# anthonyhu/tumblr-emotions

Hardware: AMD Instinct MI355X
Metric: training samples/sec (224x224 img + 32-tok text, batch 256) (higher is better)
Workload: dtype f32; 1 GPU; joint train step (fwd+bwd+all-reduce+Adam): Inception-v1 224x224x3 + 300-d embedding + LSTM-512, T=32, V=10000, 15 classes, batch 256 per GPU, reference freeze (<=Mixed_5b conv weights frozen, all BN betas trainable), dropout 0.8, BN train mode; global_batch=256, per_gpu_batch=256, parallelism=dp1, launch=eager

## Files before the change

include/ds_kernels.h:

```cpp
#ifndef DS_KERNELS_H
#define DS_KERNELS_H

#include <stddef.h>
#include <stdint.h>

#ifdef __cplusplus
extern "C" {
#endif

#define DS_OK 0
#define DS_ERR_ARG (-1)
#define DS_ERR_LAUNCH (-2)
#define DS_ERR_WORKSPACE (-3)

#define DS_DTYPE_F32 0
#define DS_DTYPE_BF16 1

#define DS_EPI_BIAS 1
#define DS_EPI_RELU 2
#define DS_EPI_ACCUM 4
#define DS_EPI_STATS 8
#define DS_EPI_MASK 16
#define DS_EPI_BNSUMS 32
#define DS_EPI_BN_RELU 64

int ds_version(void);
const char *ds_last_error(void);

typedef struct ds_conv_desc {
    int32_t N, H, W;
    int32_t Cin;
    int32_t ldx;
    int32_t KH, KW, stride;
    int32_t pad_t, pad_l;
    int32_t OH, OW;
    int32_t Cout;
    int32_t ldz;
    int64_t w_tap_stride;
    int32_t w_n_stride;
    int32_t w_k_stride;
    int32_t flip;
    int32_t fold_cin;
    int32_t flags;
    int32_t ldmask;
    int32_t splits;
    int64_t z_split_stride;
    int32_t tile_nt;
    int32_t grid_x;
    int32_t dtype;
    int32_t x_dtype;
    int32_t partials;
    const float *norm_rstd;
    const float *norm_shift;
    const float *mask_rstd;
    const float *mask_shift;
    const struct ds_bn_bwd_on_load *bnb;
    int32_t mask_dtype;
    int32_t z_dtype;
    uint8_t *pool_argmax;
    const struct ds_bn_finalize_in_launch *fin;
} ds_conv_desc;

typedef struct ds_bn_finalize_in_launch {
    const float *beta;
    float *mean, *rstd, *shift;
    float *moving_mean, *moving_var;
    uint32_t *ticket;
    int64_t count;
    float eps, decay;
} ds_bn_finalize_in_launch;

typedef struct ds_bn_bwd_on_load {
    const float *mean, *rstd, *shift;
    const float *coef;
    int32_t nseg;
    int32_t c_end[3];
    int32_t ld[3];
    const float *dy[3];
} ds_bn_bwd_on_load;

#ifdef DS_TUNING
int ds_debug_conv_set_tile(int mt, int nt);
int ds_debug_conv_set_path(int path);
int ds_debug_conv_set_wide(int mode);
int ds_debug_conv_wino_allow_ablation(int on);
int ds_debug_conv_wino4_set_nb(int nb);
int ds_debug_conv_bf16_set_max_nb(int nb);
#endif
int ds_conv_igemm_partials(const ds_conv_desc *d);
int ds_conv_igemm_bnsums_supported(const ds_conv_desc *d);
int ds_conv_igemm_norm_supported(const ds_conv_desc *d);
int ds_conv_igemm_bnb_supported(const ds_conv_desc *d);
int ds_conv_igemm_pool3_supported(const ds_conv_desc *d);
int ds_conv_igemm_finalize_tickets(const ds_conv_desc *d);
int ds_conv_igemm(const ds_conv_desc *d, const float *x, const float *w, float *z, const float *bias,
                  const float *mask, float *stats, const float *pivot, void *stream);

size_t ds_weights_bf16_bytes(int32_t Cin, int32_t Cout, int32_t taps, int32_t dgrad);
int ds_weights_to_bf16(const float *w, void *wb, int32_t Cin, int32_t Cout, int32_t taps, int32_t dgrad, void *stream);
int ds_conv_bf16_supported(const ds_conv_desc *d);
int ds_conv_bf16_partials(const ds_conv_desc *d);
int ds_conv_bf16(const ds_conv_desc *d, const void *x, const void *wb, float *z, const void *mask, float *stats,
                 const float *pivot, void *stream);

size_t ds_weights_f32x3_bytes(int32_t Cin, int32_t Cout, int32_t taps, int32_t dgrad);
int ds_weights_to_f32x3(const float *w, void *wb, int32_t Cin, int32_t Cout, int32_t taps, int32_t dgrad, void *stream);
int ds_conv_f32x3_supported(const ds_conv_desc *d);
int ds_conv_f32x3_partials(const ds_conv_desc *d);
int ds_conv_f32x3(const ds_conv_desc *d, const float *x, const void *wb, float *z, const float *mask, float *stats,
                  const float *pivot, void *stream);

#define DS_FP8_E4M3 0
#define DS_FP8_E5M2 1
#define DS_AMAX_FLOATS 512
int ds_absmax(const void *x, int64_t n, int32_t x_dtype, float *amax, void *stream);
size_t ds_weights_fp8_bytes(int32_t Cin, int32_t Cout, int32_t taps, int32_t dgrad);
int ds_weights_to_fp8(const float *w, void *wq, float *wscale, int32_t Cin, int32_t Cout, int32_t taps, int32_t dgrad,
                      void *stream);
int ds_conv_fp8_supported(const ds_conv_desc *d);
int ds_conv_fp8_partials(const ds_conv_desc *d);
int ds_conv_fp8(const ds_conv_desc *d, const void *x, const float *x_amax, int32_t a_format, const void *wq,
                const float *wscale, float *z, const void *mask, float *stats, const float *pivot, void *stream);

int ds_conv_stem_partials(int32_t N, int32_t OH, int32_t OW);
int ds_conv_stem(const float *x, const float *w, float *z, float *stats, const float *pivot, int32_t N, int32_t H,
                 int32_t W, int32_t cin_store, int32_t Cout, int32_t ldz, void *stream);
int ds_conv_stem_pool_supported(int32_t H, int32_t W);
int ds_conv_stem_pool_partials(int32_t N, int32_t OH, int32_t OW);
int ds_conv_stem_pool(const float *x, const float *w, float *zmax, float *stats, const float *pivot, int32_t N, int32_t H,
                      int32_t W, int32_t cin_store, int32_t Cout, int32_t ldz, void *stream);
int ds_conv_stem_pool_bf16(const float *x, const float *w, float *zmax, float *stats, const float *pivot, int32_t N, int32_t H,
                           int32_t W, int32_t cin_store, int32_t Cout, int32_t ldz, void *stream);
int ds_conv_stem_dgrad_supported(int32_t H, int32_t W);
int ds_conv_stem_dgrad(const float *dz, const float *w, float *dx, int32_t N, int32_t H, int32_t W, int32_t cin_store,
                       int32_t ldx, void *stream);
int ds_conv_stem_bf16_partials(int32_t N, int32_t OH, int32_t OW);
int ds_conv_stem_bf16(const float *x, const float *w, float *z, float *stats, const float *pivot, int32_t N, int32_t H, int32_t W,
                      int32_t cin_store, int32_t Cout, int32_t ldz, void *stream);

int ds_wino_transform_weights(const float *w, float *u, int32_t Cin, int32_t Cout, int32_t dgrad, void *stream);
int ds_conv_wino_partials(int32_t N, int32_t H, int32_t W);
int ds_conv_wino(const float *x, const float *u, float *z, float *stats, const float *pivot, const float *ymask,
                 int32_t N, int32_t H, int32_t W, int32_t Cin, int32_t ldx, int32_t Cout, int32_t ldz, int32_t flags,
                 void *stream);

int ds_conv_wino4_supported(int32_t H, int32_t W, int32_t Cin, int32_t Cout);
int ds_conv_wino4_prefer(int32_t N, int32_t H, int32_t W, int32_t Cin, int32_t Cout);
int ds_wino4_transform_weights(const float *w, float *u, int32_t Cin, int32_t Cout, int32_t dgrad, void *stream);
int ds_conv_wino4_partials(int32_t N, int32_t H, int32_t W);
int ds_conv_wino4(const float *x, const float *u, float *z, float *stats, const float *pivot, const float *ymask,
                  int32_t N, int32_t H, int32_t W, int32_t Cin, int32_t ldx, int32_t Cout, int32_t ldz, int32_t flags,
                  void *stream);
int ds_conv_wino4_splitk_choose(int32_t N, int32_t H, int32_t W, int32_t Cin, int32_t Cout);
int ds_conv_wino4_splitk_partials(int32_t N, int32_t H, int32_t W);
size_t ds_conv_wino4_splitk_workspace(int32_t N, int32_t H, int32_t W, int32_t Cout, int32_t splits);
int ds_conv_wino4_splitk(const float *x, const float *u, float *z, float *stats, const float *pivot, const float *ymask,
                         int32_t y_dtype, int32_t N, int32_t H, int32_t W, int32_t Cin, int32_t ldx, int32_t Cout, int32_t ldz,
                         int32_t flags, int32_t splits, void *ws, size_t ws_bytes, void *stream);
int ds_wino4_transform_weights_bf16x2(const float *w, void *u2, int32_t Cin, int32_t Cout, int32_t dgrad, void *stream);
int ds_conv_wino4_bf16x2(const float *x, const void *u2, float *z, float *stats, const float *pivot, const void *ymask,
                         int32_t y_dtype , int32_t N,
                         int32_t H, int32_t W, int32_t Cin, int32_t ldx, int32_t Cout, int32_t ldz, int32_t flags, void *stream);
int ds_conv_wino4_bf16x2_x16(const void *x16, const void *u2, float *z, float *stats, const float *pivot, const void *ymask,
                             int32_t y_dtype, int32_t N, int32_t H, int32_t W, int32_t Cin, int32_t ldx, int32_t Cout, int32_t ldz,
                             int32_t flags, void *stream);

#define DS_CONV_FWD 0
#define DS_CONV_DGRAD 1
#define DS_ARITH_F32 0
#define DS_ARITH_BF16 1
#define DS_ARITH_FP8 2
#define DS_ARITH_F32X3 3
#define DS_FAM_IGEMM 0
#define DS_FAM_WINO2 1
#define DS_FAM_WINO4 2
#define DS_FAM_STEM 3
#define DS_FAM_BF16D 4
#define DS_FAM_FP8D 5
#define DS_FAM_F32X3 6
#define DS_FAM_WINO4H 7
#define DS_FAM_STEM_POOL 8
#define DS_FAM_STEM_DGRAD 9
#define DS_PLAN_NO_WINO 1u
#define DS_PLAN_NO_WINO4 2u
#define DS_PLAN_NO_STEM_DIRECT 4u
#define DS_PLAN_NO_BF16_DIRECT 8u
#define DS_PLAN_ACT16 16u
#define DS_PLAN_FP8_EVERYWHERE 64u
#define DS_PLAN_FP8_WIDE_RULE 128u
#define DS_PLAN_NO_WINO4H 256u
#define DS_PLAN_STEM_POOL 512u
#define DS_PLAN_NO_SPLITK 1024u
#define DS_PLAN_PACKED_RGB 32u
typedef struct ds_conv_layer_plan {
    ds_conv_desc d;
    int32_t family;
    int32_t role, arith;
    int32_t partials;
    int32_t w_cin, w_cout, k;
    int32_t a_format;
    int32_t x16_ok;
    int64_t w_bytes;
    int64_t wscale_floats;
    double alg_flops;
    int32_t splitk;
    int32_t reserved0;
    int64_t ws_bytes;
} ds_conv_layer_plan;
typedef struct ds_conv_io {
    const float *bias;
    const float *mask;
    float *stats;
    const float *pivot;
    const float *x_amax;
    const float *wscale;
    const ds_bn_finalize_in_launch *fin;
    void *ws;
    size_t ws_bytes;
    const float *scale;
    const float *shift;
} ds_conv_io;
int ds_conv_plan(ds_conv_layer_plan *plan, int32_t role, int32_t arith, uint32_t options, int32_t N, int32_t H, int32_t W,
                 int32_t w_cin, int32_t w_cout, int32_t k, int32_t stride, int32_t ldx, int32_t ldz, int32_t flags);
int ds_conv_plan_set_flags(ds_conv_layer_plan *plan, int32_t flags);
int ds_conv_plan_enable_bnsums(ds_conv_layer_plan *plan, int32_t ldy);
int ds_conv_plan_norm_supported(const ds_conv_layer_plan *plan);
int ds_conv_plan_bnb_supported(const ds_conv_layer_plan *plan);
int ds_conv_plan_enable_pool3(ds_conv_layer_plan *plan, uint8_t *argmax);
int ds_conv_plan_enable_bn_relu(ds_conv_layer_plan *plan);
int ds_conv_plan_finalize_tickets(const ds_conv_layer_plan *plan);
int ds_conv_prepare_weights(const ds_conv_layer_plan *plan, const float *w_hwio, void *w_prepared, float *wscale,
                            void *stream);
int ds_conv_run(const ds_conv_layer_plan *plan, const void *x, const void *w, float *z, const ds_conv_io *io, void *stream);

size_t ds_conv_wgrad_workspace(const ds_conv_desc *d);
int ds_conv_wgrad(const ds_conv_desc *d, const float *x, const float *dz, int32_t lddz, float *dw,
                  void *ws, size_t ws_bytes, void *stream);

int ds_bn_finalize(const float *stats, int32_t P, int64_t count, int32_t C, const float *beta, const float *pivot,
                   float eps, float decay, float *mean, float *rstd, float *shift, float *moving_mean,
                   float *moving_var, void *stream);

int ds_bn_finalize_centered(const float *stats, int32_t P, int64_t count, int32_t C, const float *beta, const float *pivot,
                            float eps, float decay, float *mean, float *rstd, float *shift, float *moving_mean,
                            float *moving_var, float *mean_c, float *shift_c, void *stream);
typedef struct ds_bn_finalize_job {
    const float *stats;
    int32_t P, C;
    int64_t count;
    const float *beta;
    const float *pivot;
    float *mean, *rstd, *shift;
    float *moving_mean, *moving_var;
} ds_bn_finalize_job;
int ds_bn_finalize_multi(const ds_bn_finalize_job *jobs, int32_t njobs, float eps, float decay, void *stream);

int ds_bn_finalize_apply_relu(const float *stats, int32_t P, int64_t count, int32_t C, const float *beta, const float *pivot,
                              float eps, float decay, float *mean, float *rstd, float *shift, float *moving_mean,
                              float *moving_var, const float *z, int64_t M, const struct ds_segments *dst, uint32_t *ticket,
                              void *stream);

typedef struct ds_segments {
    int32_t nseg;
    int32_t c_begin[4];
    int32_t c_end[4];
    int32_t ld[4];
    void *ptr[4];
    int32_t dtype[4];
    float *amax[4];
    const float *ptr2[4];
} ds_segments;
int ds_bn_apply_relu(const float *z, int64_t M, int32_t C, const float *rstd, const float *shift,
                     const ds_segments *dst, void *stream);
int ds_bn_apply_relu_z16(const void *z16, int64_t M, int32_t C, const float *rstd, const float *shift,
                         const ds_segments *dst, void *stream);
int ds_bn_infer_prepare(const float *beta, const float *moving_mean, const float *moving_var, float eps,
                        int32_t C, float *rstd, float *shift, void *stream);
typedef struct ds_bn_infer_job {
    const float *beta, *moving_mean, *moving_var;
    int32_t C;
    float *rstd, *shift;
} ds_bn_infer_job;
int ds_bn_infer_prepare_multi(const ds_bn_infer_job *jobs, int32_t njobs, float eps, void *stream);

int ds_bn_bwd_partials(int64_t M, int32_t C);
int ds_bn_bwd_reduce(const void *z, int32_t ldz, int32_t z_dtype, const ds_segments *dy, int64_t M, int32_t C,
                     const float *mean, const float *rstd, const float *shift, float *partials, void *stream);
int ds_bn_bwd_finalize(const float *partials, int32_t P, int64_t M, int32_t C, float *dbeta, float *coef,
                       void *stream);
typedef struct ds_bn_sum_segments {
    int32_t nseg;
    int32_t c_begin[4], c_end[4];
    int32_t P[4];
    int32_t kind[4];
    const float *s[4];
    const float *q[4];
    int32_t P2[4];
    const float *s2[4];
    const float *q2[4];
} ds_bn_sum_segments;
int ds_bn_bwd_finalize_segs(const ds_bn_sum_segments *sg, int64_t M, int32_t C, const float *beta, float *dbeta,
                            float *coef, void *stream);
int ds_bn_bwd_finalize_multi(const ds_bn_sum_segments *sg, int64_t M, int32_t C, const float *const *beta,
                             float *const *dbeta, float *coef, void *stream);
int ds_bn_bwd_finalize_apply(const ds_bn_sum_segments *sg, const float *beta, float *dbeta, const float *const *beta_v,
                             float *const *dbeta_v, float *coef, const float *z, int32_t ldz, const ds_segments *dy, int64_t M,
                             int32_t C, const float *mean, const float *rstd, const float *shift, void *dz, int32_t dz_dtype,
                             int32_t lddz, float *amax, uint32_t *ticket, void *stream);
int ds_bn_bwd_apply(const float *z, int32_t ldz, const ds_segments *dy, int64_t M, int32_t C, const float *mean,
                    const float *rstd, const float *shift, const float *coef, float *dz, float *amax, void *stream);
int ds_bn_bwd_apply_cols(const float *z, int32_t ldz, const ds_segments *dy, int64_t M, int32_t ncols, const float *mean,
                         const float *rstd, const float *shift, const float *coef_g, const float *coef_gx, float *dz,
                         void *stream);
int ds_bn_infer_bwd_apply(const float *z, int32_t ldz, const ds_segments *dy, int64_t M, int32_t C, const float *rstd,
                          const float *shift, float *dz, void *stream);
int ds_bn_infer_bwd_partials(int64_t M, int32_t C);
int ds_bn_infer_bwd_apply_sums(const float *z, int32_t ldz, const ds_segments *dy, int64_t M, int32_t C, const float *rstd,
                               const float *shift, float *dz, float *partials, void *stream);
typedef struct ds_bn_sum_job {
    const float *partials;
    int32_t P, C;
    float *dbeta;
} ds_bn_sum_job;
int ds_bn_dbeta_reduce_multi(const ds_bn_sum_job *jobs, int32_t njobs, void *stream);
int ds_bn_bwd_apply_bf16(const float *z, int32_t ldz, const ds_segments *dy, int64_t M, int32_t C, const float *mean,
                         const float *rstd, const float *shift, const float *coef, void *dz16, int32_t lddz, float *amax,
                         void *stream);

int ds_bn_bwd_apply_z16(const void *z16, int32_t ldz, const ds_segments *dy, int64_t M, int32_t C, const float *mean,
                        const float *rstd, const float *shift, const float *coef, void *dz16, int32_t lddz, float *amax,
                        void *stream);

int ds_maxpool_fwd(const void *x, void *y, uint8_t *argmax, int32_t N, int32_t H, int32_t W, int32_t C,
                   int32_t k, int32_t stride, int32_t pad_t, int32_t pad_l, int32_t OH, int32_t OW,
                   int32_t act_dtype, void *stream);
int ds_maxpool_bn_relu_fwd(const float *z, const float *rstd, const float *shift, void *y, uint8_t *argmax,
                           int32_t N, int32_t H, int32_t W, int32_t C, int32_t k, int32_t stride, int32_t pad_t,
                           int32_t pad_l, int32_t OH, int32_t OW, int32_t y_dtype, float *amax, void *stream);
int ds_bn_pool_bwd_partials(int32_t N, int32_t OH, int32_t OW, int32_t C);
int ds_bn_pool_bwd_reduce(const float *z, const float *dpool, const uint8_t *argmax, int32_t N, int32_t H, int32_t W,
                          int32_t C, int32_t pad_t, int32_t pad_l, int32_t OH, int32_t OW, const float *mean,
                          const float *rstd, const float *shift, float *partials, void *stream);
int ds_bn_pool_bwd_apply(const float *z, const float *dpool, const uint8_t *argmax, int32_t N, int32_t H, int32_t W,
                         int32_t C, int32_t pad_t, int32_t pad_l, int32_t OH, int32_t OW, const float *mean,
                         const float *rstd, const float *shift, const float *coef, float *dz, void *stream);
int ds_bn_pool_bwd_apply_cols(const float *z, int32_t ldz, float *dz, int32_t lddz, const float *dpool, const uint8_t *argmax,
                              int32_t Cp, int32_t c0, int32_t N, int32_t H, int32_t W, int32_t pad_t, int32_t pad_l, int32_t OH,
                              int32_t OW, int32_t ncols, const float *mean, const float *rstd, const float *shift,
                              const float *coef_g, const float *coef_gx, int32_t k, void *stream);
int ds_bn_pool_infer_bwd_apply(const float *z, const float *dpool, const uint8_t *argmax, int32_t N, int32_t H, int32_t W,
                               int32_t C, int32_t pad_t, int32_t pad_l, int32_t OH, int32_t OW, const float *rstd,
                               const float *shift, float *dz, void *stream);
int ds_bn_pool_infer_bwd_apply_sums(const float *z, const float *dpool, const uint8_t *argmax, int32_t N, int32_t H, int32_t W,
                                    int32_t C, int32_t pad_t, int32_t pad_l, int32_t OH, int32_t OW, const float *rstd,
                                    const float *shift, float *dz, float *partials, void *stream);
int ds_maxpool_bwd(const float *dy, const uint8_t *argmax, float *dx, int32_t accumulate, int32_t N,
                   int32_t H, int32_t W, int32_t C, int32_t k, int32_t stride, int32_t pad_t, int32_t pad_l,
                   int32_t OH, int32_t OW, void *stream);

int ds_maxpool3_bwd_sums_partials(int32_t N, int32_t W, int32_t C);
int ds_maxpool3_bwd_sums(const float *dy, const uint8_t *argmax, float *dx, int32_t accumulate, const void *y,
                         int32_t y_dtype, int32_t N, int32_t H, int32_t W, int32_t C, float *partials, void *stream);

int ds_maxpool3_bwd_dy16(const void *dy16, const uint8_t *argmax, float *dx, int32_t accumulate, const void *y, int32_t y_dtype,
                         int32_t N, int32_t H, int32_t W, int32_t C, float *partials, void *stream);

int ds_avgpool_dropout_fwd(const float *x, int32_t N, int32_t HW, int32_t C, float keep, uint64_t seed,
                           const uint64_t *seed_dev, const float *mask_in, float *mask_out, float *out,
                           void *stream);
int ds_avgpool_dropout_bwd(const float *dout, const float *mask, int32_t N, int32_t HW, int32_t C,
                           float keep, float *dx, void *stream);

int ds_gather_rows(const float *table, const int64_t *ids, float *out, int32_t B, int32_t T, int32_t D,
                   int64_t table_rows, int32_t time_major, void *stream);

int ds_token_dot(const float *dx, const float *x, const int64_t *seq_len, float *out, int32_t B, int32_t T, int32_t D,
                 void *stream);

int ds_embedding_grad(const float *dx, const int64_t *ids, float *dtable, int32_t B, int32_t T, int32_t D,
                      int64_t table_rows, int32_t time_major, void *stream);

int ds_lstm_cell_fwd(float *gates, const float *rec_slabs, int32_t nslabs, int64_t slab_stride,
                     const float *c_prev, const float *h_prev, const int64_t *seq_len, int32_t t, int32_t B,
                     int32_t H, float forget_bias, float *c_out, float *h_out, void *stream);
int ds_lstm_cell_bwd(const float *acts, const float *c_t, const float *c_prev, const float *dh,
                     const float *dh_slabs, int32_t nslabs, int64_t slab_stride, const float *dc,
                     const int64_t *seq_len, int32_t t, int32_t B, int32_t H, float *dgates, float *dc_prev,
                     float *dh_carry, void *stream);

int ds_seq_sort_desc(const int64_t *seq_len, int32_t B, int32_t T, int32_t *perm, int64_t *len_sorted, void *stream);
int ds_permute_rows(const void *src, int64_t lds, void *dst, int64_t ldd, const int32_t *perm, int32_t rows, int32_t cols,
                    int32_t elem_bytes, int32_t gather, void *stream);
#define DS_LSTM_SKIP_MASKED 256
int ds_lstm_seq_supported(int32_t B, int32_t H);
size_t ds_lstm_seq_workspace(int32_t B, int32_t H);
int ds_lstm_seq_fwd(float *gates, const float *wh, int32_t ldw, float *h, float *c, const int64_t *seq_len, int32_t T,
                    int32_t B, int32_t H, float forget_bias, int32_t rows, void *ws, size_t ws_bytes, void *stream);
int ds_lstm_seq_bwd(const float *acts, const float *wh, int32_t ldw, const float *c, const float *dh_last,
                    int32_t ld_dh, const int64_t *seq_len, int32_t T, int32_t B, int32_t H, float *dgates, int32_t rows,
                    void *ws, size_t ws_bytes, void *stream);
int ds_lstm_seq_status(void *ws, int32_t B);
#ifdef DS_TUNING
int ds_debug_lstm_seq_set_profile(void *buf);
int ds_debug_lstm_seq_set_profile_bwd(void *buf);
#endif

int ds_softmax_ce(const float *logits, const int64_t *labels, int32_t B, int32_t C, float grad_scale,
                  const float *grad_scale_dev, float *loss, float *dlogits, void *stream);

int ds_adam_tf(float *theta, const float *g, float *m, float *v, int64_t n, int64_t n_wd, float wd,
               float grad_scale, float lr_t, const float *lr_t_dev, float beta1, float beta2, float eps,
               void *stream);

int ds_grad_accumulate(float *acc, float *g, int64_t n, int32_t mode, void *stream);

int ds_sumsq(const float *x, int64_t n, float *scratch, float *out, void *stream);
int ds_colsum(const float *x, int64_t M, int32_t C, int32_t ld, float *scratch, float *out, void *stream);
int ds_slab_epilogue(const float *slabs, int32_t splits, int64_t slab_stride, int32_t lds, int64_t M, int32_t N, float *out,
                     int32_t ldo, const float *bias, const float *mask, int32_t ldmask, int32_t flags, void *stream);
int ds_copy2d(const float *src, int32_t lds, float *dst, int32_t ldd, int64_t rows, int32_t cols,
              void *stream);
int ds_pad_channels(const float *src, int32_t cs, float *dst, int32_t cd, int64_t pixels, void *stream);
int ds_fill(float *dst, int64_t n, float value, void *stream);

typedef struct ds_preprocess_desc {
    int64_t offset;
    int32_t height, width;
    float scale_y, scale_x;
} ds_preprocess_desc;
int ds_preprocess_eval(const uint8_t *bytes, int64_t nbytes, const ds_preprocess_desc *desc, int32_t batch, const float *lut,
                       float *out, int32_t out_h, int32_t out_w, void *stream);

#define DS_PREPROCESS_FLIP 1u
#define DS_PREPROCESS_SATURATION_FIRST 2u
typedef struct ds_preprocess_train_desc {
    int64_t offset;
    int32_t height, width;
    float scale_y, scale_x;
    float delta;
    float factor;
    uint32_t flags;
    uint32_t reserved;
} ds_preprocess_train_desc;
int ds_preprocess_train(const uint8_t *bytes, int64_t nbytes, const ds_preprocess_train_desc *desc, int32_t batch,
                        const float *lut, float *out, int32_t out_h, int32_t out_w, void *stream);

#define DS_JPEG_UNSUPPORTED 1
#define DS_JPEG_MORE 2
#define DS_JPEG_444 0
#define DS_JPEG_422 1
#define DS_JPEG_420 2
#define DS_JPEG_GREY 3
typedef struct ds_jpeg_info {
    int32_t width, height;
    int32_t components;
    int32_t sampling;
    int32_t restart_interval;
    int32_t supported;
    int64_t coef_count;
    int64_t coef_bytes;
    uint8_t quant[3][64];
} ds_jpeg_info;
int ds_jpeg_probe(const uint8_t *bytes, int64_t n, ds_jpeg_info *info);
int ds_jpeg_entropy_decode(const uint8_t *bytes, int64_t n, const ds_jpeg_info *info, int16_t *coef, int64_t capacity);

typedef struct ds_jpeg_desc {
    int64_t coef_offset;
    int64_t out_offset;
    int32_t width, height;
    int32_t sampling;
    int32_t y0, x0, crop_h, crop_w;
    int32_t reserved;
    uint8_t quant[3][64];
} ds_jpeg_desc;
int ds_jpeg_reconstruct_host(const int16_t *coef, int64_t ncoef, const ds_jpeg_desc *desc, int32_t batch,
                             uint8_t *out_bytes, int64_t nbytes);
int ds_jpeg_reconstruct(const int16_t *coef, int64_t ncoef, const ds_jpeg_desc *desc, int32_t batch, uint8_t *out_bytes,
                        int64_t nbytes, void *scratch, int64_t scratch_bytes, void *stream);

typedef struct ds_example_fields {
    int64_t image_offset, image_length;
    int64_t seq_len, label, post_id, day;
    int32_t text_len;
    int32_t reserved;
} ds_example_fields;
int ds_example_parse(const uint8_t *rec, int64_t n, int64_t *text, int32_t text_capacity, ds_example_fields *fields);
int ds_jpeg_record_decode(const uint8_t *rec, int64_t n, int64_t *text, int32_t text_capacity, ds_example_fields *fields,
                          ds_jpeg_info *info, int16_t *coef, int64_t capacity, int32_t *jpeg_status);

typedef struct ds_jpeg_huff {
    uint8_t counts[16];
    uint8_t values[256];
} ds_jpeg_huff;
typedef struct ds_jpeg_scan_info {
    int64_t scan_begin;
    int64_t cut_count;
    ds_jpeg_huff dc[3], ac[3];
} ds_jpeg_scan_info;
int ds_jpeg_scan(const uint8_t *bytes, int64_t n, ds_jpeg_info *info, ds_jpeg_scan_info *scan, int64_t *cuts, int64_t capacity);
int ds_jpeg_record_scan(const uint8_t *rec, int64_t n, int64_t *text, int32_t text_capacity, ds_example_fields *fields,
                        ds_jpeg_info *info, ds_jpeg_scan_info *scan, int64_t *cuts, int64_t capacity, int32_t *jpeg_status);
int ds_jpeg_restart_transcode(const uint8_t *bytes, int64_t n, int32_t interval_mcus, uint8_t *out, int64_t capacity,
                              int64_t *out_n);

typedef struct ds_jpeg_scan_desc {
    int64_t coef_offset;
    int32_t width, height;
    int32_t sampling;
    int32_t first_segment;
    int32_t segments;
    int32_t reserved;
    uint8_t quant[3][64];
    ds_jpeg_huff dc[3], ac[3];
} ds_jpeg_scan_desc;
typedef struct ds_jpeg_segment {
    int64_t begin, end;
    int32_t first_mcu, mcus;
} ds_jpeg_segment;
#define DS_JPEG_E_CODE 1
#define DS_JPEG_E_RUN 2
#define DS_JPEG_E_RANGE 4
#define DS_JPEG_E_COLUMN 8
#define DS_JPEG_E_SEGMENT 16
#define DS_JPEG_E_TABLE 32
int ds_jpeg_entropy_decode_segments_host(const uint8_t *scan, int64_t nscan, const ds_jpeg_scan_desc *images, int32_t nimages,
                                         const ds_jpeg_segment *segs, int64_t nsegs, int16_t *coef, int64_t ncoef,
                                         int32_t *status);
int ds_jpeg_entropy_decode_device(const uint8_t *scan, int64_t nscan, const ds_jpeg_scan_desc *images, int32_t nimages,
                                  const ds_jpeg_segment *segs, int64_t nsegs, int16_t *coef, int64_t ncoef, int32_t *status,
                                  void *stream);

typedef struct ds_gather_desc {
    int64_t src_offset;
    int64_t out_offset;
    int32_t src;
    int32_t pitch;
    int32_t y0, x0;
    int32_t height, width;
} ds_gather_desc;
int ds_ragged_gather(const uint8_t *arena, int64_t narena, const uint8_t *spill, int64_t nspill, const ds_gather_desc *desc,
                     int32_t batch, uint8_t *out, int64_t nout, void *stream);
int ds_ragged_gather_host(const uint8_t *arena, int64_t narena, const uint8_t *spill, int64_t nspill,
                          const ds_gather_desc *desc, int32_t batch, uint8_t *out, int64_t nout);

int ds_eval_metrics_workspace(int32_t B, int32_t C);
int ds_eval_metrics_update(const float *logits, int32_t ldl, const int64_t *labels, int32_t B, int32_t C, int64_t *counts,
                           double *loss_sum, void *scratch, void *stream);

#ifdef __cplusplus
}
#endif
#endif
```

tumblr_emotions_amd/_lib.py:

```python
import ctypes as C
import os

_HERE = os.path.dirname(os.path.abspath(__file__))
LIB_PATH = os.environ.get("DS_LIB") or os.path.join(_HERE, "libds_kernels.so")

def tuning_env(name, default=None):
    return os.environ.get(name, default) if os.environ.get("DS_LIB") else default


DS_EPI_BIAS, DS_EPI_RELU, DS_EPI_ACCUM, DS_EPI_STATS, DS_EPI_MASK, DS_EPI_BNSUMS = 1, 2, 4, 8, 16, 32
DS_EPI_BN_RELU = 64
DS_DTYPE_F32, DS_DTYPE_BF16 = 0, 1
DS_FP8_E4M3, DS_FP8_E5M2 = 0, 1
DS_CONV_FWD, DS_CONV_DGRAD = 0, 1
DS_LSTM_SKIP_MASKED = 256
DS_ARITH_F32, DS_ARITH_BF16, DS_ARITH_FP8, DS_ARITH_F32X3 = 0, 1, 2, 3
DS_FAM_IGEMM, DS_FAM_WINO2, DS_FAM_WINO4, DS_FAM_STEM, DS_FAM_BF16D, DS_FAM_FP8D, DS_FAM_F32X3, DS_FAM_WINO4H, DS_FAM_STEM_POOL = range(9)
DS_FAM_STEM_DGRAD = 9
DS_PLAN_NO_WINO, DS_PLAN_NO_WINO4, DS_PLAN_NO_STEM_DIRECT, DS_PLAN_NO_BF16_DIRECT, DS_PLAN_ACT16, DS_PLAN_PACKED_RGB = 1, 2, 4, 8, 16, 32
DS_PLAN_FP8_EVERYWHERE, DS_PLAN_FP8_WIDE_RULE, DS_PLAN_NO_WINO4H, DS_PLAN_STEM_POOL = 64, 128, 256, 512
DS_PLAN_NO_SPLITK = 1024
DS_PREPROCESS_FLIP, DS_PREPROCESS_SATURATION_FIRST = 1, 2
DS_JPEG_UNSUPPORTED, DS_JPEG_MORE = 1, 2
DS_JPEG_444, DS_JPEG_422, DS_JPEG_420, DS_JPEG_GREY = 0, 1, 2, 3
DS_JPEG_E_CODE, DS_JPEG_E_RUN, DS_JPEG_E_RANGE, DS_JPEG_E_COLUMN, DS_JPEG_E_SEGMENT, DS_JPEG_E_TABLE = 1, 2, 4, 8, 16, 32


class ConvDesc(C.Structure):
    _fields_ = [
        ("N", C.c_int32), ("H", C.c_int32), ("W", C.c_int32), ("Cin", C.c_int32), ("ldx", C.c_int32),
        ("KH", C.c_int32), ("KW", C.c_int32), ("stride", C.c_int32), ("pad_t", C.c_int32), ("pad_l", C.c_int32),
        ("OH", C.c_int32), ("OW", C.c_int32), ("Cout", C.c_int32), ("ldz", C.c_int32),
        ("w_tap_stride", C.c_int64), ("w_n_stride", C.c_int32), ("w_k_stride", C.c_int32),
        ("flip", C.c_int32), ("fold_cin", C.c_int32), ("flags", C.c_int32), ("ldmask", C.c_int32),
        ("splits", C.c_int32), ("z_split_stride", C.c_int64),
        ("tile_nt", C.c_int32), ("grid_x", C.c_int32), ("dtype", C.c_int32), ("x_dtype", C.c_int32),
        ("partials", C.c_int32),
        ("norm_rstd", C.c_void_p), ("norm_shift", C.c_void_p), ("mask_rstd", C.c_void_p), ("mask_shift", C.c_void_p),
        ("bnb", C.c_void_p), ("mask_dtype", C.c_int32), ("z_dtype", C.c_int32), ("pool_argmax", C.c_void_p), ("fin", C.c_void_p),
    ]


class BnBwdOnLoad(C.Structure):
    _fields_ = [("mean", C.c_void_p), ("rstd", C.c_void_p), ("shift", C.c_void_p), ("coef", C.c_void_p),
                ("nseg", C.c_int32), ("c_end", C.c_int32 * 3), ("ld", C.c_int32 * 3), ("dy", C.c_void_p * 3)]


class BnFinalizeInLaunch(C.Structure):
    _fields_ = [("beta", C.c_void_p), ("mean", C.c_void_p), ("rstd", C.c_void_p), ("shift", C.c_void_p),
                ("moving_mean", C.c_void_p), ("moving_var", C.c_void_p), ("ticket", C.c_void_p), ("count", C.c_int64),
                ("eps", C.c_float), ("decay", C.c_float)]


class LayerPlanStruct(C.Structure):
    _fields_ = [("d", ConvDesc), ("family", C.c_int32), ("role", C.c_int32), ("arith", C.c_int32), ("partials", C.c_int32),
                ("w_cin", C.c_int32), ("w_cout", C.c_int32), ("k", C.c_int32), ("a_format", C.c_int32), ("x16_ok", C.c_int32),
                ("w_bytes", C.c_int64), ("wscale_floats", C.c_int64), ("alg_flops", C.c_double), ("splitk", C.c_int32),
                ("reserved0", C.c_int32), ("ws_bytes", C.c_int64)]


class ConvIO(C.Structure):
    _fields_ = [("bias", C.c_void_p), ("mask", C.c_void_p), ("stats", C.c_void_p), ("pivot", C.c_void_p),
                ("x_amax", C.c_void_p), ("wscale", C.c_void_p), ("fin", C.c_void_p), ("ws", C.c_void_p), ("ws_bytes", C.c_size_t),
                ("scale", C.c_void_p), ("shift", C.c_void_p)]


class Segments(C.Structure):
    _fields_ = [("nseg", C.c_int32), ("c_begin", C.c_int32 * 4), ("c_end", C.c_int32 * 4),
                ("ld", C.c_int32 * 4), ("ptr", C.c_void_p * 4), ("dtype", C.c_int32 * 4),
                ("amax", C.c_void_p * 4), ("ptr2", C.c_void_p * 4)]


class BnFinalizeJob(C.Structure):
    _fields_ = [("stats", C.c_void_p), ("P", C.c_int32), ("C", C.c_int32), ("count", C.c_int64), ("beta", C.c_void_p),
                ("pivot", C.c_void_p), ("mean", C.c_void_p), ("rstd", C.c_void_p), ("shift", C.c_void_p),
                ("moving_mean", C.c_void_p), ("moving_var", C.c_void_p)]


class BnInferJob(C.Structure):
    _fields_ = [("beta", C.c_void_p), ("moving_mean", C.c_void_p), ("moving_var", C.c_void_p), ("C", C.c_int32),
                ("rstd", C.c_void_p), ("shift", C.c_void_p)]


class BnSumJob(C.Structure):
    _fields_ = [("partials", C.c_void_p), ("P", C.c_int32), ("C", C.c_int32), ("dbeta", C.c_void_p)]


class SumSegments(C.Structure):
    _fields_ = [("nseg", C.c_int32), ("c_begin", C.c_int32 * 4), ("c_end", C.c_int32 * 4), ("P", C.c_int32 * 4),
                ("kind", C.c_int32 * 4), ("s", C.c_void_p * 4), ("q", C.c_void_p * 4), ("P2", C.c_int32 * 4),
                ("s2", C.c_void_p * 4), ("q2", C.c_void_p * 4)]


class PreprocessDesc(C.Structure):
    _fields_ = [("offset", C.c_int64), ("height", C.c_int32), ("width", C.c_int32), ("scale_y", C.c_float), ("scale_x", C.c_float)]


class PreprocessTrainDesc(C.Structure):
    _fields_ = [("offset", C.c_int64), ("height", C.c_int32), ("width", C.c_int32), ("scale_y", C.c_float), ("scale_x", C.c_float),
                ("delta", C.c_float), ("factor", C.c_float), ("flags", C.c_uint32), ("reserved", C.c_uint32)]


class JpegInfo(C.Structure):
    _fields_ = [("width", C.c_int32), ("height", C.c_int32), ("components", C.c_int32), ("sampling", C.c_int32),
                ("restart_interval", C.c_int32), ("supported", C.c_int32), ("coef_count", C.c_int64), ("coef_bytes", C.c_int64),
                ("quant", C.c_uint8 * 192)]


class JpegDesc(C.Structure):
    _fields_ = [("coef_offset", C.c_int64), ("out_offset", C.c_int64), ("width", C.c_int32), ("height", C.c_int32),
                ("sampling", C.c_int32), ("y0", C.c_int32), ("x0", C.c_int32), ("crop_h", C.c_int32), ("crop_w", C.c_int32),
                ("reserved", C.c_int32), ("quant", C.c_uint8 * 192)]


class JpegHuff(C.Structure):
    _fields_ = [("counts", C.c_uint8 * 16), ("values", C.c_uint8 * 256)]


class JpegScanInfo(C.Structure):
    _fields_ = [("scan_begin", C.c_int64), ("cut_count", C.c_int64), ("dc", JpegHuff * 3), ("ac", JpegHuff * 3)]


class GatherDesc(C.Structure):
    _fields_ = [("src_offset", C.c_int64), ("out_offset", C.c_int64), ("src", C.c_int32), ("pitch", C.c_int32),
                ("y0", C.c_int32), ("x0", C.c_int32), ("height", C.c_int32), ("width", C.c_int32)]


class ExampleFields(C.Structure):
    _fields_ = [("image_offset", C.c_int64), ("image_length", C.c_int64), ("seq_len", C.c_int64), ("label", C.c_int64),
                ("post_id", C.c_int64), ("day", C.c_int64), ("text_len", C.c_int32), ("reserved", C.c_int32)]


_P = C.c_void_p
_i32, _i64, _f32, _u64 = C.c_int32, C.c_int64, C.c_float, C.c_uint64
_CD = C.POINTER(ConvDesc)
_SG = C.POINTER(Segments)
_SS = C.POINTER(SumSegments)
_LP = C.POINTER(LayerPlanStruct)
_IO = C.POINTER(ConvIO)

SIGNATURES = {
    "ds_version": (C.c_int, []),
    "ds_last_error": (C.c_char_p, []),
    "ds_conv_igemm_partials": (C.c_int, [_CD]),
    "ds_conv_igemm_bnsums_supported": (C.c_int, [_CD]),
    "ds_conv_igemm_norm_supported": (C.c_int, [_CD]),
    "ds_conv_igemm_bnb_supported": (C.c_int, [_CD]),
    "ds_conv_igemm_pool3_supported": (C.c_int, [_CD]),
    "ds_conv_igemm_finalize_tickets": (C.c_int, [_CD]),
    "ds_conv_igemm": (C.c_int, [_CD, _P, _P, _P, _P, _P, _P, _P, _P]),
    "ds_weights_bf16_bytes": (C.c_size_t, [_i32, _i32, _i32, _i32]),
    "ds_weights_to_bf16": (C.c_int, [_P, _P, _i32, _i32, _i32, _i32, _P]),
    "ds_conv_bf16_supported": (C.c_int, [_CD]),
    "ds_conv_bf16_partials": (C.c_int, [_CD]),
    "ds_conv_bf16": (C.c_int, [_CD, _P, _P, _P, _P, _P, _P, _P]),
    "ds_weights_f32x3_bytes": (C.c_size_t, [_i32, _i32, _i32, _i32]),
    "ds_weights_to_f32x3": (C.c_int, [_P, _P, _i32, _i32, _i32, _i32, _P]),
    "ds_conv_f32x3_supported": (C.c_int, [_CD]),
    "ds_conv_f32x3_partials": (C.c_int, [_CD]),
    "ds_conv_f32x3": (C.c_int, [_CD, _P, _P, _P, _P, _P, _P, _P]),
    "ds_absmax": (C.c_int, [_P, _i64, _i32, _P, _P]),
    "ds_weights_fp8_bytes": (C.c_size_t, [_i32, _i32, _i32, _i32]),
    "ds_weights_to_fp8": (C.c_int, [_P, _P, _P, _i32, _i32, _i32, _i32, _P]),
    "ds_conv_fp8_supported": (C.c_int, [_CD]),
    "ds_conv_fp8_partials": (C.c_int, [_CD]),
    "ds_conv_fp8": (C.c_int, [_CD, _P, _P, _i32, _P, _P, _P, _P, _P, _P, _P]),
    "ds_conv_stem_partials": (C.c_int, [_i32, _i32, _i32]),
    "ds_conv_stem_bf16_partials": (C.c_int, [_i32, _i32, _i32]),
    "ds_conv_stem": (C.c_int, [_P, _P, _P, _P, _P, _i32, _i32, _i32, _i32, _i32, _i32, _P]),
    "ds_conv_stem_bf16": (C.c_int, [_P, _P, _P, _P, _P, _i32, _i32, _i32, _i32, _i32, _i32, _P]),
    "ds_conv_stem_pool_supported": (C.c_int, [_i32, _i32]),
    "ds_conv_stem_pool_partials": (C.c_int, [_i32, _i32, _i32]),
    "ds_conv_stem_pool": (C.c_int, [_P, _P, _P, _P, _P, _i32, _i32, _i32, _i32, _i32, _i32, _P]),
    "ds_conv_stem_pool_bf16": (C.c_int, [_P, _P, _P, _P, _P, _i32, _i32, _i32, _i32, _i32, _i32, _P]),
    "ds_conv_stem_dgrad_supported": (C.c_int, [_i32, _i32]),
    "ds_conv_stem_dgrad": (C.c_int, [_P, _P, _P, _i32, _i32, _i32, _i32, _i32, _P]),
    "ds_wino_transform_weights": (C.c_int, [_P, _P, _i32, _i32, _i32, _P]),
    "ds_conv_wino_partials": (C.c_int, [_i32, _i32, _i32]),
    "ds_conv_wino": (C.c_int, [_P, _P, _P, _P, _P, _P, _i32, _i32, _i32, _i32, _i32, _i32, _i32, _i32, _P]),
    "ds_conv_wino4_supported": (C.c_int, [_i32, _i32, _i32, _i32]),
    "ds_conv_wino4_prefer": (C.c_int, [_i32, _i32, _i32, _i32, _i32]),
    "ds_wino4_transform_weights": (C.c_int, [_P, _P, _i32, _i32, _i32, _P]),
    "ds_conv_wino4_partials": (C.c_int, [_i32, _i32, _i32]),
    "ds_conv_wino4_splitk_choose": (C.c_int, [_i32, _i32, _i32, _i32, _i32]),
    "ds_conv_wino4_splitk_partials": (C.c_int, [_i32, _i32, _i32]),
    "ds_conv_wino4_splitk_workspace": (C.c_size_t, [_i32, _i32, _i32, _i32, _i32]),
    "ds_conv_wino4_splitk": (C.c_int, [_P, _P, _P, _P, _P, _P, _i32, _i32, _i32, _i32, _i32, _i32, _i32, _i32, _i32, _i32, _P, C.c_size_t, _P]),
    "ds_conv_wino4": (C.c_int, [_P, _P, _P, _P, _P, _P, _i32, _i32, _i32, _i32, _i32, _i32, _i32, _i32, _P]),
    "ds_conv_wino4_bf16x2": (C.c_int, [_P, _P, _P, _P, _P, _P, _i32, _i32, _i32, _i32, _i32, _i32, _i32, _i32, _i32, _P]),
    "ds_conv_wino4_bf16x2_x16": (C.c_int, [_P, _P, _P, _P, _P, _P, _i32, _i32, _i32, _i32, _i32, _i32, _i32, _i32, _i32, _P]),
    "ds_wino4_transform_weights_bf16x2": (C.c_int, [_P, _P, _i32, _i32, _i32, _P]),
    "ds_conv_plan": (C.c_int, [_LP, _i32, _i32, C.c_uint32] + [_i32] * 10),
    "ds_conv_plan_set_flags": (C.c_int, [_LP, _i32]),
    "ds_conv_plan_enable_bnsums": (C.c_int, [_LP, _i32]),
    "ds_conv_plan_norm_supported": (C.c_int, [_LP]),
    "ds_conv_plan_bnb_supported": (C.c_int, [_LP]),
    "ds_conv_plan_enable_pool3": (C.c_int, [_LP, C.c_void_p]),
    "ds_conv_plan_enable_bn_relu": (C.c_int, [_LP]),
    "ds_conv_plan_finalize_tickets": (C.c_int, [_LP]),
    "ds_conv_prepare_weights": (C.c_int, [_LP, _P, _P, _P, _P]),
    "ds_conv_run": (C.c_int, [_LP, _P, _P, _P, _IO, _P]),
    "ds_conv_wgrad_workspace": (C.c_size_t, [_CD]),
    "ds_conv_wgrad": (C.c_int, [_CD, _P, _P, _i32, _P, _P, C.c_size_t, _P]),
    "ds_bn_finalize": (C.c_int, [_P, _i32, _i64, _i32, _P, _P, _f32, _f32, _P, _P, _P, _P, _P, _P]),
    "ds_bn_finalize_centered": (C.c_int, [_P, _i32, _i64, _i32, _P, _P, _f32, _f32, _P, _P, _P, _P, _P, _P, _P, _P]),
    "ds_bn_apply_relu": (C.c_int, [_P, _i64, _i32, _P, _P, _SG, _P]),
    "ds_bn_apply_relu_z16": (C.c_int, [_P, _i64, _i32, _P, _P, _SG, _P]),
    "ds_bn_bwd_apply_z16": (C.c_int, [_P, _i32, _SG, _i64, _i32, _P, _P, _P, _P, _P, _i32, _P, _P]),
    "ds_bn_infer_prepare": (C.c_int, [_P, _P, _P, _f32, _i32, _P, _P, _P]),
    "ds_bn_infer_prepare_multi": (C.c_int, [_P, _i32, _f32, _P]),
    "ds_bn_bwd_partials": (C.c_int, [_i64, _i32]),
    "ds_bn_bwd_reduce": (C.c_int, [_P, _i32, _i32, _SG, _i64, _i32, _P, _P, _P, _P, _P]),
    "ds_bn_bwd_finalize_segs": (C.c_int, [_SS, _i64, _i32, _P, _P, _P, _P]),
    "ds_bn_bwd_finalize": (C.c_int, [_P, _i32, _i64, _i32, _P, _P, _P]),
    "ds_bn_bwd_finalize_multi": (C.c_int, [_SS, _i64, _i32, _P, _P, _P, _P]),
    "ds_bn_finalize_multi": (C.c_int, [_P, _i32, _f32, _f32, _P]),
    "ds_bn_finalize_apply_relu": (C.c_int, [_P, _i32, _i64, _i32, _P, _P, _f32, _f32, _P, _P, _P, _P, _P, _P, _i64, _SG, _P, _P]),
    "ds_bn_bwd_finalize_apply": (C.c_int, [_SS, _P, _P, _P, _P, _P, _P, _i32, _SG, _i64, _i32, _P, _P, _P, _P, _i32, _i32, _P, _P, _P]),
    "ds_bn_bwd_apply": (C.c_int, [_P, _i32, _SG, _i64, _i32, _P, _P, _P, _P, _P, _P, _P]),
    "ds_bn_bwd_apply_cols": (C.c_int, [_P, _i32, _SG, _i64, _i32, _P, _P, _P, _P, _P, _P, _P]),
    "ds_bn_infer_bwd_apply": (C.c_int, [_P, _i32, _SG, _i64, _i32, _P, _P, _P, _P]),
    "ds_bn_infer_bwd_partials": (C.c_int, [_i64, _i32]),
    "ds_bn_infer_bwd_apply_sums": (C.c_int, [_P, _i32, _SG, _i64, _i32, _P, _P, _P, _P, _P]),
    "ds_bn_dbeta_reduce_multi": (C.c_int, [_P, _i32, _P]),
    "ds_bn_bwd_apply_bf16": (C.c_int, [_P, _i32, _SG, _i64, _i32, _P, _P, _P, _P, _P, _i32, _P, _P]),
    "ds_maxpool_fwd": (C.c_int, [_P, _P, _P] + [_i32] * 11 + [_P]),
    "ds_maxpool_bn_relu_fwd": (C.c_int, [_P, _P, _P, _P, _P] + [_i32] * 11 + [_P, _P]),
    "ds_bn_pool_bwd_partials": (C.c_int, [_i32, _i32, _i32, _i32]),
    "ds_bn_pool_bwd_reduce": (C.c_int, [_P, _P, _P] + [_i32] * 8 + [_P, _P, _P, _P, _P]),
    "ds_bn_pool_bwd_apply": (C.c_int, [_P, _P, _P] + [_i32] * 8 + [_P, _P, _P, _P, _P, _P]),
    "ds_bn_pool_bwd_apply_cols": (C.c_int, [_P, _i32, _P, _i32, _P, _P] + [_i32] * 10 + [_P, _P, _P, _P, _P, _i32, _P]),
    "ds_bn_pool_infer_bwd_apply": (C.c_int, [_P, _P, _P] + [_i32] * 8 + [_P, _P, _P, _P]),
    "ds_bn_pool_infer_bwd_apply_sums": (C.c_int, [_P, _P, _P] + [_i32] * 8 + [_P, _P, _P, _P, _P]),
    "ds_maxpool_bwd": (C.c_int, [_P, _P, _P] + [_i32] * 11 + [_P]),
    "ds_maxpool3_bwd_sums_partials": (C.c_int, [_i32, _i32, _i32]),
    "ds_maxpool3_bwd_sums": (C.c_int, [_P, _P, _P, _i32, _P, _i32, _i32, _i32, _i32, _i32, _P, _P]),
    "ds_maxpool3_bwd_dy16": (C.c_int, [_P, _P, _P, _i32, _P, _i32, _i32, _i32, _i32, _i32, _P, _P]),
    "ds_avgpool_dropout_fwd": (C.c_int, [_P, _i32, _i32, _i32, _f32, _u64, _P, _P, _P, _P, _P]),
    "ds_avgpool_dropout_bwd": (C.c_int, [_P, _P, _i32, _i32, _i32, _f32, _P, _P]),
    "ds_gather_rows": (C.c_int, [_P, _P, _P, _i32, _i32, _i32, _i64, _i32, _P]),
    "ds_token_dot": (C.c_int, [_P, _P, _P, _P, _i32, _i32, _i32, _P]),
    "ds_embedding_grad": (C.c_int, [_P, _P, _P, _i32, _i32, _i32, _i64, _i32, _P]),
    "ds_lstm_cell_fwd": (C.c_int, [_P, _P, _i32, _i64, _P, _P, _P, _i32, _i32, _i32, _f32, _P, _P, _P]),
    "ds_lstm_cell_bwd": (C.c_int, [_P, _P, _P, _P, _P, _i32, _i64, _P, _P, _i32, _i32, _i32, _P, _P, _P, _P]),
    "ds_seq_sort_desc": (C.c_int, [_P, _i32, _i32, _P, _P, _P]),
    "ds_permute_rows": (C.c_int, [_P, _i64, _P, _i64, _P, _i32, _i32, _i32, _i32, _P]),
    "ds_lstm_seq_supported": (C.c_int, [_i32, _i32]),
    "ds_lstm_seq_workspace": (C.c_size_t, [_i32, _i32]),
    "ds_lstm_seq_fwd": (C.c_int, [_P, _P, _i32, _P, _P, _P, _i32, _i32, _i32, _f32, _i32, _P, C.c_size_t, _P]),
    "ds_lstm_seq_bwd": (C.c_int, [_P, _P, _i32, _P, _P, _i32, _P, _i32, _i32, _i32, _P, _i32, _P, C.c_size_t, _P]),
    "ds_lstm_seq_status": (C.c_int, [_P, _i32]),
    "ds_softmax_ce": (C.c_int, [_P, _P, _i32, _i32, _f32, _P, _P, _P, _P]),
    "ds_adam_tf": (C.c_int, [_P, _P, _P, _P, _i64, _i64, _f32, _f32, _f32, _P, _f32, _f32, _f32, _P]),
    "ds_grad_accumulate": (C.c_int, [_P, _P, _i64, _i32, _P]),
    "ds_sumsq": (C.c_int, [_P, _i64, _P, _P, _P]),
    "ds_colsum": (C.c_int, [_P, _i64, _i32, _i32, _P, _P, _P]),
    "ds_slab_epilogue": (C.c_int, [_P, _i32, _i64, _i32, _i64, _i32, _P, _i32, _P, _P, _i32, _i32, _P]),
    "ds_copy2d": (C.c_int, [_P, _i32, _P, _i32, _i64, _i32, _P]),
    "ds_pad_channels": (C.c_int, [_P, _i32, _P, _i32, _i64, _P]),
    "ds_fill": (C.c_int, [_P, _i64, _f32, _P]),
    "ds_preprocess_eval": (C.c_int, [_P, _i64, _P, _i32, _P, _P, _i32, _i32, _P]),
    "ds_preprocess_train": (C.c_int, [_P, _i64, _P, _i32, _P, _P, _i32, _i32, _P]),
    "ds_jpeg_probe": (C.c_int, [_P, _i64, C.POINTER(JpegInfo)]),
    "ds_jpeg_entropy_decode": (C.c_int, [_P, _i64, C.POINTER(JpegInfo), _P, _i64]),
    "ds_jpeg_reconstruct_host": (C.c_int, [_P, _i64, _P, _i32, _P, _i64]),
    "ds_jpeg_reconstruct": (C.c_int, [_P, _i64, _P, _i32, _P, _i64, _P, _i64, _P]),
    "ds_example_parse": (C.c_int, [_P, _i64, _P, _i32, C.POINTER(ExampleFields)]),
    "ds_jpeg_record_decode": (C.c_int, [_P, _i64, _P, _i32, C.POINTER(ExampleFields), C.POINTER(JpegInfo), _P, _i64,
                                        C.POINTER(_i32)]),
    "ds_jpeg_scan": (C.c_int, [_P, _i64, C.POINTER(JpegInfo), C.POINTER(JpegScanInfo), _P, _i64]),
    "ds_jpeg_record_scan": (C.c_int, [_P, _i64, _P, _i32, C.POINTER(ExampleFields), C.POINTER(JpegInfo), C.POINTER(JpegScanInfo),
                                      _P, _i64, C.POINTER(_i32)]),
    "ds_jpeg_restart_transcode": (C.c_int, [_P, _i64, _i32, _P, _i64, C.POINTER(_i64)]),
    "ds_jpeg_entropy_decode_segments_host": (C.c_int, [_P, _i64, _P, _i32, _P, _i64, _P, _i64, _P]),
    "ds_jpeg_entropy_decode_device": (C.c_int, [_P, _i64, _P, _i32, _P, _i64, _P, _i64, _P, _P]),
    "ds_ragged_gather": (C.c_int, [_P, _i64, _P, _i64, _P, _i32, _P, _i64, _P]),
    "ds_ragged_gather_host": (C.c_int, [_P, _i64, _P, _i64, _P, _i32, _P, _i64]),
    "ds_eval_metrics_workspace": (C.c_int, [_i32, _i32]),
    "ds_eval_metrics_update": (C.c_int, [_P, _i32, _P, _i32, _i32, _P, _P, _P, _P]),
}

_lib = None


DEBUG_SIGNATURES = {
    "ds_debug_conv_set_tile": (C.c_int, [C.c_int, C.c_int]),
    "ds_debug_conv_set_path": (C.c_int, [C.c_int]),
    "ds_debug_conv_set_wide": (C.c_int, [C.c_int]),
    "ds_debug_conv_wino_allow_ablation": (C.c_int, [C.c_int]),
    "ds_debug_conv_wino4_set_nb": (C.c_int, [C.c_int]),
    "ds_debug_conv_bf16_set_max_nb": (C.c_int, [C.c_int]),
    "ds_debug_lstm_seq_set_profile": (C.c_int, [_P]),
    "ds_debug_lstm_seq_set_profile_bwd": (C.c_int, [_P]),
}
TUNING_LIB_PATH = os.path.join(_HERE, "libds_kernels_tuning.so")
_tuning = None


def _bind(lib, table):
    for name, (res, args) in table.items():
        fn = getattr(lib, name)
        fn.restype = res
        fn.argtypes = args


def load_tuning():
    global _tuning
    if _tuning is None:
        if not os.path.exists(TUNING_LIB_PATH):
            raise RuntimeError("tumblr_emotions_amd: %s not found -- `make -C tumblr_emotions_amd/csrc` builds it" % TUNING_LIB_PATH)
        lib = C.CDLL(TUNING_LIB_PATH)
        _bind(lib, SIGNATURES)
        _bind(lib, DEBUG_SIGNATURES)
        _tuning = lib
    return _tuning


class tuning_library:

    def __enter__(self):
        global _lib
        self._saved = load()
        _lib = load_tuning()
        return _lib

    def __exit__(self, *exc):
        global _lib
        _lib = self._saved
        return False


def load():
    global _lib
    if _lib is not None:
        return _lib
    if not os.path.exists(LIB_PATH):
        raise RuntimeError(
            "tumblr_emotions_amd: %s not found -- build it with `python -c 'import __graft_entry__ as g; "
            "g.build()'` or `make -C tumblr_emotions_amd/csrc`.  There is no CPU fallback." % LIB_PATH)
    if os.environ.get("DS_LIB"):
        import sys
        sys.stderr.write("tumblr_emotions_amd: DS_LIB overrides the kernel library: %s\n" % LIB_PATH)
    lib = C.CDLL(LIB_PATH)
    _bind(lib, SIGNATURES)
    if hasattr(lib, "ds_debug_conv_set_tile"):
        _bind(lib, DEBUG_SIGNATURES)
    _lib = lib
    return lib


def check(rc, what):
    if rc != 0:
        raise RuntimeError("%s failed (%d): %s" % (what, rc, load().ds_last_error().decode()))
```

tumblr_emotions_amd/csrc/conv_wgrad.hip:

```cpp
#include <stdio.h>
#include <stdlib.h>
#include "ds_common.h"

typedef float f32x16 __attribute__((ext_vector_type(16)));
typedef float f32x4 __attribute__((ext_vector_type(4)));
typedef unsigned int u32x4 __attribute__((ext_vector_type(4)));

namespace {

constexpr int TJ = 128;
constexpr int TP = 16;

struct WgradParams {
    ds_conv_desc d;
    const float *x;
    const float *dz;
    float *out;
    int lddz;
    int M;
    int ci_tiles;
    int pix_per_split;
    int x_vec, z_vec;
    unsigned x_bytes, z_bytes;
    float inv_ohw, inv_ow;
    int slabs;
};

constexpr unsigned kOOB = 0x80000000u;

__device__ __forceinline__ __amdgpu_buffer_rsrc_t make_srd(const void *p, unsigned bytes) {
    return __builtin_amdgcn_make_buffer_rsrc(const_cast<void *>(p), 0, (int)bytes, 0x00020000);
}

__device__ __forceinline__ f32x4 load4(__amdgpu_buffer_rsrc_t r, unsigned off, bool ok, bool vec, int valid) {
    if (vec) return __builtin_bit_cast(f32x4, __builtin_amdgcn_raw_buffer_load_b128(r, ok ? off : kOOB, 0, 0));
    f32x4 v;
#pragma unroll
    for (int j = 0; j < 4; ++j)
        v[j] = __builtin_bit_cast(float, __builtin_amdgcn_raw_buffer_load_b32(r, (ok && j < valid) ? off + 4 * j : kOOB, 0, 0));
    return v;
}

__device__ __forceinline__ int fdiv(int a, int b, float inv) {
    int q = (int)((float)a * inv);
    int r = a - q * b;
    if (r < 0) --q;
    if (r >= b) ++q;
    return q;
}

template <int TIT>
__global__ __launch_bounds__(256) void conv_wgrad_kernel(const WgradParams p) {
    constexpr int LDX = TIT + 4, LDZ = TJ + 4;
    constexpr int WNW = TIT == 128 ? 2 : 4;
    constexpr int CW = TJ / WNW;
    constexpr int BS = CW / 32;
    constexpr int XQ = TIT / 4;
    constexpr int XROWS = 256 / XQ;
    constexpr int XP = TP / XROWS;
    __shared__ __attribute__((aligned(16))) float smem[2 * TP * LDX + 2 * TP * LDZ];
    float *Xs = smem;
    float *Zs = smem + 2 * TP * LDX;
    const ds_conv_desc &d = p.d;
    const int tid = threadIdx.x, lane = tid & 63;
    const int wave = __builtin_amdgcn_readfirstlane(tid >> 6);
    const int wm = TIT == 128 ? wave >> 1 : 0, wn = TIT == 128 ? wave & 1 : wave;
    const int li = lane & 31, lk = lane >> 5;
    const int tap = blockIdx.x / p.ci_tiles;
    const int i0 = (blockIdx.x % p.ci_tiles) * TIT;
    const int j0 = blockIdx.y * TJ;
    const int split = blockIdx.z;
    const int dh = tap / d.KW, dw = tap % d.KW;
    const int ohw = d.OH * d.OW;
    const int m_begin = split * p.pix_per_split;
    int m_end = m_begin + p.pix_per_split;
    if (m_end > p.M) m_end = p.M;

    int it_valid = (d.Cin - (i0 + wm * 64) + 31) / 32;
    it_valid = it_valid < 0 ? 0 : (it_valid > 2 ? 2 : it_valid);
    int jt_valid = (d.Cout - (j0 + wn * CW) + 31) / 32;
    jt_valid = jt_valid < 0 ? 0 : (jt_valid > BS ? BS : jt_valid);

    f32x16 acc[2][BS];
#pragma unroll
    for (int a = 0; a < 2; ++a)
#pragma unroll
        for (int b = 0; b < BS; ++b)
#pragma unroll
            for (int r = 0; r < 16; ++r) acc[a][b][r] = 0.f;

    const int xrow = tid / XQ, xc4 = (tid % XQ) * 4;
    const int zrow = tid >> 5, zc4 = (tid & 31) * 4;
    f32x4 rx[XP], rz[2];
    const __amdgpu_buffer_rsrc_t srd_x = make_srd(p.x, p.x_bytes);
    const __amdgpu_buffer_rsrc_t srd_z = make_srd(p.dz, p.z_bytes);
    const int cx = i0 + xc4, cz = j0 + zc4;
    const bool small = p.M < (1 << 24);

    auto load_tile = [&](int mt0) {
#pragma unroll
        for (int i = 0; i < XP; ++i) {
            const int m = mt0 + xrow + XROWS * i;
            const bool rv = m < m_end;
            const int mm = rv ? m : 0;
            const int n = small ? fdiv(mm, ohw, p.inv_ohw) : mm / ohw;
            const int r = mm - n * ohw;
            const int oh = small ? fdiv(r, d.OW, p.inv_ow) : r / d.OW;
            const int ow = r - oh * d.OW;
            const int ih = oh * d.stride - d.pad_t + dh, iw = ow * d.stride - d.pad_l + dw;
            const int iwc = d.fold_cin > 0 ? iw + cx / d.fold_cin : iw;
            const bool okx = rv && (unsigned)ih < (unsigned)d.H && (unsigned)iwc < (unsigned)d.W && cx < d.Cin;
            const unsigned offx = (unsigned)(((n * d.H + ih) * d.W + iw) * d.ldx + cx);
            rx[i] = load4(srd_x, offx * 4u, okx, p.x_vec, d.Cin - cx);
        }
#pragma unroll
        for (int i = 0; i < 2; ++i) {
            const int m = mt0 + zrow + 8 * i;
            const bool okz = m < m_end && cz < d.Cout;
            const unsigned offz = (unsigned)(m < m_end ? m : 0) * (unsigned)p.lddz + (unsigned)cz;
            rz[i] = load4(srd_z, offz * 4u, okz, p.z_vec, d.Cout - cz);
        }
    };
    auto store_tile = [&](int buf) {
#pragma unroll
        for (int i = 0; i < XP; ++i)
            *reinterpret_cast<f32x4 *>(Xs + (buf * TP + xrow + XROWS * i) * LDX + xc4) = rx[i];
#pragma unroll
        for (int i = 0; i < 2; ++i)
            *reinterpret_cast<f32x4 *>(Zs + (buf * TP + zrow + 8 * i) * LDZ + zc4) = rz[i];
    };
    auto compute = [&](int buf) {
        const float *xs = Xs + buf * TP * LDX + wm * 64 + li;
        const float *zs = Zs + buf * TP * LDZ + wn * CW + li;
#pragma unroll
        for (int s = 0; s < TP / 2; ++s) {
            const int row = 2 * s + lk;
            float af[2], bf[BS];
            af[0] = xs[row * LDX];
            af[1] = xs[row * LDX + 32];
#pragma unroll
            for (int b = 0; b < BS; ++b) bf[b] = zs[row * LDZ + 32 * b];
#pragma unroll
            for (int a = 0; a < 2; ++a)
#pragma unroll
                for (int b = 0; b < BS; ++b)
                    if (a < it_valid && b < jt_valid)
                        acc[a][b] = __builtin_amdgcn_mfma_f32_32x32x2f32(af[a], bf[b], acc[a][b], 0, 0, 0);
        }
    };

    const int KT = (m_end - m_begin + TP - 1) / TP;
    if (KT > 0) {
        load_tile(m_begin);
        store_tile(0);
        __syncthreads();
        for (int kt = 0; kt < KT; ++kt) {
            const int cur = kt & 1;
            if (kt + 1 < KT) load_tile(m_begin + (kt + 1) * TP);
            compute(cur);
            if (kt + 1 < KT) store_tile(cur ^ 1);
            __syncthreads();
        }
    }

    float *out = p.out + (int64_t)split * (d.KH * d.KW) * d.Cin * d.Cout + (int64_t)tap * d.Cin * d.Cout;
#pragma unroll
    for (int a = 0; a < 2; ++a)
#pragma unroll
        for (int b = 0; b < BS; ++b) {
            const int col = j0 + wn * CW + b * 32 + li;
#pragma unroll
            for (int r = 0; r < 16; ++r) {
                const int row = i0 + wm * 64 + a * 32 + (r & 3) + 8 * (r >> 2) + 4 * lk;
                if (row < d.Cin && col < d.Cout) out[(int64_t)row * d.Cout + col] = acc[a][b][r];
            }
        }
}


#ifndef DS_WG_U
#define DS_WG_U 4
#endif
template <int W>
__device__ __forceinline__ f32x4 loadw(__amdgpu_buffer_rsrc_t r, unsigned off) {
    f32x4 v = {0.f, 0.f, 0.f, 0.f};
    if constexpr (W == 4) {
        v = __builtin_bit_cast(f32x4, __builtin_amdgcn_raw_buffer_load_b128(r, off, 0, 0));
    } else if constexpr (W == 2) {
        typedef unsigned int u32x2 __attribute__((ext_vector_type(2)));
        typedef float f32x2 __attribute__((ext_vector_type(2)));
        const f32x2 t = __builtin_bit_cast(f32x2, __builtin_amdgcn_raw_buffer_load_b64(r, off, 0, 0));
        v[0] = t[0]; v[1] = t[1];
    } else {
        v[0] = __builtin_bit_cast(float, __builtin_amdgcn_raw_buffer_load_b32(r, off, 0, 0));
    }
    return v;
}

template <int AI, int BJ>
__global__ __launch_bounds__(256, (AI * BJ > 8) ? 1 : 2) void wgrad_direct_kernel(const WgradParams p) {
    constexpr int NACC = AI * BJ, U = DS_WG_U;
    __shared__ __attribute__((aligned(16))) float red[2 * NACC * 16 * 64];
    const ds_conv_desc &d = p.d;
    const int tid = threadIdx.x, lane = tid & 63;
    const int wave = __builtin_amdgcn_readfirstlane(tid >> 6);
    const int li = lane & 31, lk = lane >> 5;
    const int co_tiles = (d.Cout + 32 * BJ - 1) / (32 * BJ);
    const int split = (int)(blockIdx.x % (unsigned)p.slabs);
    int bid = (int)(blockIdx.x / (unsigned)p.slabs);
    const int jt = bid % co_tiles; bid /= co_tiles;
    const int itile = bid % p.ci_tiles;
    const int tap = bid / p.ci_tiles;
    const int dh = tap / d.KW, dw = tap % d.KW;
    const int ci0 = itile * 32 * AI, co0 = jt * 32 * BJ;
    const int ci = ci0 + AI * li, co = co0 + BJ * li;
    const bool ci_ok = ci < d.Cin, co_ok = co < d.Cout;
    const __amdgpu_buffer_rsrc_t srd_x = make_srd(p.x, p.x_bytes);
    const __amdgpu_buffer_rsrc_t srd_z = make_srd(p.dz, p.z_bytes);

    const int m_begin = split * p.pix_per_split;
    int m_end = m_begin + p.pix_per_split;
    if (m_end > p.M) m_end = p.M;
    int q = (m_end - m_begin + 3) / 4;
    q = (q + 1) & ~1;
    const int wb = m_begin + wave * q;
    int we = wb + q;
    if (we > m_end) we = m_end;
    const int steps = we > wb ? (we - wb + 1) / 2 : 0;

    int m = wb + lk;
    const int ohw = d.OH * d.OW;
    int oh = 0, ow = 0;
    unsigned offx, offz;
    {
        const int mm = m < p.M ? m : 0;
        const int n = mm / ohw;
        const int r = mm - n * ohw;
        oh = r / d.OW;
        ow = r - oh * d.OW;
        const int ih = oh * d.stride - d.pad_t + dh, iw = ow * d.stride - d.pad_l + dw;
        offx = ((unsigned)((n * d.H + ih) * d.W + iw) * (unsigned)d.ldx + (unsigned)ci) * 4u;
        offz = ((unsigned)mm * (unsigned)p.lddz + (unsigned)co) * 4u;
    }
    const unsigned ldx4 = (unsigned)d.ldx * 4u;
    const unsigned step_x = 2u * (unsigned)d.stride * ldx4;
    const unsigned row_x = (unsigned)((d.W - d.OW) * d.stride) * ldx4;
    const unsigned img_x = (unsigned)((d.H - d.OH * d.stride) * d.W) * ldx4;
    const unsigned step_z = 2u * (unsigned)p.lddz * 4u;
    auto lo_of = [](int pad, int tap, int stride) { const int v = pad - tap; return v <= 0 ? 0 : (v + stride - 1) / stride; };
    auto hi_of = [](int pad, int tap, int stride, int ext, int oext) {
        const int v = ext - 1 + pad - tap;
        const int h = v < 0 ? -1 : v / stride;
        return h > oext - 1 ? oext - 1 : h;
    };
    const int lo_h = lo_of(d.pad_t, dh, d.stride), lo_w = lo_of(d.pad_l, dw, d.stride);
    const unsigned span_h = (unsigned)(hi_of(d.pad_t, dh, d.stride, d.H, d.OH) - lo_h);
    const unsigned span_w = (unsigned)(hi_of(d.pad_l, dw, d.stride, d.W, d.OW) - lo_w);
    const int OWc = d.OW, OHc = d.OH;
    auto offsets = [&](unsigned &ox, unsigned &oz) {
        const bool mv = m < we;
        const bool in = (unsigned)(oh - lo_h) <= span_h && (unsigned)(ow - lo_w) <= span_w;
        oz = (mv && co_ok) ? offz : kOOB;
        ox = (mv && ci_ok && in) ? offx : kOOB;
        m += 2;
        offz += step_z;
        offx += step_x;
        ow += 2;
#pragma unroll
        for (int rep = 0; rep < 2; ++rep) {
            if (rep == 1 && OWc > 1) break;
            const bool wrap = ow >= OWc;
            ow = wrap ? ow - OWc : ow;
            oh += wrap ? 1 : 0;
            offx += wrap ? row_x : 0u;
            const bool wrap2 = oh >= OHc;
            oh = wrap2 ? oh - OHc : oh;
            offx += wrap2 ? img_x : 0u;
        }
    };

    f32x16 acc[AI][BJ];
#pragma unroll
    for (int a = 0; a < AI; ++a)
#pragma unroll
        for (int b = 0; b < BJ; ++b)
#pragma unroll
            for (int r = 0; r < 16; ++r) acc[a][b][r] = 0.f;

    f32x4 xa[U], zb[U];
#pragma unroll
    for (int u = 0; u < U; ++u) {
        unsigned ox, oz;
        offsets(ox, oz);
        xa[u] = loadw<AI>(srd_x, ox);
        zb[u] = loadw<BJ>(srd_z, oz);
    }
    for (int s = 0; s < steps; s += U) {
#pragma unroll
        for (int u = 0; u < U; ++u) {
            const f32x4 a4 = xa[u], b4 = zb[u];
            unsigned ox, oz;
            offsets(ox, oz);
            xa[u] = loadw<AI>(srd_x, ox);
            zb[u] = loadw<BJ>(srd_z, oz);
#pragma unroll
            for (int a = 0; a < AI; ++a)
#pragma unroll
                for (int b = 0; b < BJ; ++b)
                    acc[a][b] = __builtin_amdgcn_mfma_f32_32x32x2f32(a4[a], b4[b], acc[a][b], 0, 0, 0);
        }
    }

    auto put = [&](int slot) {
#pragma unroll
        for (int a = 0; a < AI; ++a)
#pragma unroll
            for (int b = 0; b < BJ; ++b)
#pragma unroll
                for (int r4 = 0; r4 < 4; ++r4) {
                    f32x4 v = {acc[a][b][4 * r4], acc[a][b][4 * r4 + 1], acc[a][b][4 * r4 + 2], acc[a][b][4 * r4 + 3]};
                    *reinterpret_cast<f32x4 *>(red + ((slot * NACC + a * BJ + b) * 4 + r4) * 256 + lane * 4) = v;
                }
    };
    auto get = [&](int slot) {
#pragma unroll
        for (int a = 0; a < AI; ++a)
#pragma unroll
            for (int b = 0; b < BJ; ++b)
#pragma unroll
                for (int r4 = 0; r4 < 4; ++r4) {
                    const f32x4 v = *reinterpret_cast<const f32x4 *>(red + ((slot * NACC + a * BJ + b) * 4 + r4) * 256 + lane * 4);
#pragma unroll
                    for (int e = 0; e < 4; ++e) acc[a][b][4 * r4 + e] += v[e];
                }
    };
    if (wave >= 2) put(wave - 2);
    __syncthreads();
    if (wave < 2) get(wave);
    __syncthreads();
    if (wave == 1) put(0);
    __syncthreads();
    if (wave != 0) return;
    get(0);

    float *out = p.out + (int64_t)split * (d.KH * d.KW) * d.Cin * d.Cout + (int64_t)tap * d.Cin * d.Cout;
    if (!co_ok) return;
#pragma unroll
    for (int a = 0; a < AI; ++a)
#pragma unroll
        for (int r = 0; r < 16; ++r) {
            const int row = ci0 + AI * ((r & 3) + 8 * (r >> 2) + 4 * lk) + a;
            if (row < d.Cin) {
                float *o = out + (int64_t)row * d.Cout + co;
                if constexpr (BJ == 4) {
                    *reinterpret_cast<f32x4 *>(o) = f32x4{acc[a][0][r], acc[a][1][r], acc[a][2][r], acc[a][3][r]};
                } else if constexpr (BJ == 2) {
                    typedef float f32x2 __attribute__((ext_vector_type(2)));
                    *reinterpret_cast<f32x2 *>(o) = f32x2{acc[a][0][r], acc[a][1][r]};
                } else {
                    *o = acc[a][0][r];
                }
            }
        }
}

__global__ __launch_bounds__(256) void splitk_reduce_kernel(const float *ws, float *dw, int64_t n, int splits) {
    for (int64_t i = (int64_t)blockIdx.x * 256 + threadIdx.x; i < n; i += (int64_t)gridDim.x * 256) {
        float s = 0.f;
        for (int k = 0; k < splits; ++k) s += ws[(int64_t)k * n + i];
        dw[i] = s;
    }
}

int pick_ti(const ds_conv_desc *d) {
    const int p128 = (d->Cin + 127) / 128 * 128, p64 = (d->Cin + 63) / 64 * 64;
    return (p128 - p64) * 5 >= p128 ? 64 : 128;
}

int pick_splits(const ds_conv_desc *d, int64_t M) {
    const int ti = pick_ti(d);
    const int tiles = d->KH * d->KW * ((d->Cin + ti - 1) / ti) * ((d->Cout + TJ - 1) / TJ);
    static int occ = 0, minpix = 0;
    if (!occ) {
        const char *e = ds::tune_env("DS_WGRAD_OCC");
        occ = e ? atoi(e) : 3;
        e = ds::tune_env("DS_WGRAD_MINPIX");
        minpix = e ? atoi(e) : 64;
    }
    int splits = (occ * ds::kCUs + tiles - 1) / tiles;
    const int max_splits = (int)((M + minpix - 1) / minpix);
    if (splits > max_splits) splits = max_splits;
    if (splits < 1) splits = 1;
    return splits;
}

struct WgradPlan {
    int direct;
    int ai, bj;
    int splits;
};

int max_width(int C, int ld, uintptr_t ptr) {
    for (int w = 4; w > 1; w >>= 1)
        if (C % w == 0 && ld % w == 0 && (ptr & (4 * w - 1)) == 0) return w;
    return 1;
}

bool direct_ok(const ds_conv_desc *d, int64_t M) {
    static int mode = -1;
    if (mode < 0) {
        const char *e = ds::tune_env("DS_WGRAD_DIRECT");
        mode = e ? atoi(e) : 1;
    }
    return mode && d->fold_cin == 0 && M >= 512;
}

WgradPlan plan_direct(const ds_conv_desc *d, int64_t M, int wx, int wz, int only_ai = 0, int only_bj = 0) {
    WgradPlan best = {};
    double best_cost = 1e30;
    static const int kSlabs[] = {1, 2, 4, 8, 16, 24, 32, 40, 48, 56, 64};
    const double wbytes = (double)d->KH * d->KW * d->Cin * d->Cout * 4.0;
    for (int ai = 1; ai <= wx; ai *= 2)
        for (int bj = 1; bj <= wz; bj *= 2) {
            if ((only_ai && ai != only_ai) || (only_bj && bj != only_bj)) continue;
            const int nacc = ai * bj;
            const int occ = nacc > 8 ? 1 : (nacc > 4 ? 2 : 3);
            const int tiles = d->KH * d->KW * ((d->Cin + 32 * ai - 1) / (32 * ai)) * ((d->Cout + 32 * bj - 1) / (32 * bj));
            for (int slabs : kSlabs) {
                if (slabs > 1 && M / slabs < 256) break;
                const int xcds = slabs >= 8 ? 8 : slabs;
                const double per_xcd = (double)tiles * slabs / 8.0;
                const double slots = 32.0 * occ;
                double rounds = (double)(int64_t)(per_xcd / slots);
                if (rounds * slots < per_xcd) rounds += 1.0;
                const double steps = (double)M / slabs / 8.0;
                const double step_cycles = nacc * 64.0 > 160.0 ? nacc * 64.0 : 160.0;
                const double t_wg = steps * step_cycles + 1500.0 + nacc * 350.0;
                const double t_red = slabs > 1 ? 6000.0 + slabs * wbytes / 1500.0 : 0.0;
                const double cost = rounds * t_wg + t_red;
                (void)xcds;
                if (cost < best_cost) {
                    best_cost = cost;
                    best.direct = 1; best.ai = ai; best.bj = bj; best.splits = slabs;
                }
            }
        }
    return best;
}

WgradPlan plan_wgrad(const ds_conv_desc *d, int64_t M, const float *x, const float *dz, int lddz, const float *dw,
                     const void *ws) {
    if (direct_ok(d, M)) {
        const uintptr_t zalign = (uintptr_t)dz | (uintptr_t)dw | (uintptr_t)ws;
        const int wx = max_width(d->Cin, d->ldx, (uintptr_t)x), wz = max_width(d->Cout, lddz, zalign);
        WgradPlan pl = plan_direct(d, M, wx, wz);
        if (const char *e = ds::tune_env("DS_WGRAD_FORCE")) {
            int a = 0, b = 0, sl = 0;
            if (sscanf(e, "%d,%d,%d", &a, &b, &sl) == 3) {
                if ((a && a <= wx) || (b && b <= wz)) {
                    const WgradPlan f = plan_direct(d, M, wx, wz, a <= wx ? a : 0, b <= wz ? b : 0);
                    if (f.direct) pl = f;
                }
                if (sl) pl.splits = sl;
            }
        }
        return pl;
    }
    WgradPlan pl = {};
    pl.splits = pick_splits(d, M);
    return pl;
}

}

extern "C" size_t ds_conv_wgrad_workspace(const ds_conv_desc *d) {
    const int64_t M = (int64_t)d->N * d->OH * d->OW;
    int splits = pick_splits(d, M);
    if (direct_ok(d, M)) {
        splits = 1;
        for (int wx = 1; wx <= 4; wx *= 2)
            for (int wz = 1; wz <= 4; wz *= 2) {
                const int sp = plan_direct(d, M, wx, wz).splits;
                splits = sp > splits ? sp : splits;
            }
    }
    if (splits == 1) return 0;
    return (size_t)splits * d->KH * d->KW * d->Cin * d->Cout * sizeof(float);
}

extern "C" int ds_conv_wgrad(const ds_conv_desc *d, const float *x, const float *dz, int32_t lddz, float *dw,
                             void *ws, size_t ws_bytes, void *stream) {
    DS_REQUIRE(d && x && dz && dw, "ds_conv_wgrad: null argument");
    const int64_t M = (int64_t)d->N * d->OH * d->OW;
    DS_REQUIRE(M < (1ll << 31), "ds_conv_wgrad: M too large");
    DS_REQUIRE(d->fold_cin == 0 || (d->KW == 1 && d->ldx == d->fold_cin && d->fold_cin % 4 == 0 && d->Cin % d->fold_cin == 0),
               "ds_conv_wgrad: fold_cin needs KW=1, ldx==fold_cin, fold_cin %% 4 == 0");
    const WgradPlan pl = plan_wgrad(d, M, x, dz, lddz, dw, ws);
    if (ds::tune_env("DS_WGRAD_DEBUG"))
        fprintf(stderr, "wgrad M=%lld Cin=%d Cout=%d k=%d: direct=%d ai=%d bj=%d slabs=%d\n", (long long)M, d->Cin, d->Cout, d->KH,
                pl.direct, pl.ai, pl.bj, pl.splits);
    const int splits = pl.splits;
    const size_t need = splits == 1 ? 0 : (size_t)splits * d->KH * d->KW * d->Cin * d->Cout * sizeof(float);
    if (need > 0 && (ws == nullptr || ws_bytes < need)) {
        ds::set_error("ds_conv_wgrad: workspace %zu bytes < required %zu", ws_bytes, need);
        return DS_ERR_WORKSPACE;
    }
    WgradParams p;
    p.d = *d;
    p.x = x; p.dz = dz; p.lddz = lddz;
    p.out = splits == 1 ? dw : (float *)ws;
    p.M = (int)M;
    const int64_t x_elems = ((int64_t)d->N * d->H * d->W - 1) * d->ldx + d->Cin;
    const int64_t z_elems = (M - 1) * lddz + d->Cout;
    DS_REQUIRE(x_elems * 4 < (1ll << 31) && z_elems * 4 < (1ll << 31), "ds_conv_wgrad: operand larger than 2 GiB (split the batch)");
    p.x_bytes = (unsigned)(x_elems * 4);
    p.z_bytes = (unsigned)(z_elems * 4);
    p.inv_ohw = 1.0f / (float)(d->OH * d->OW);
    p.inv_ow = 1.0f / (float)d->OW;
    p.x_vec = (d->ldx % 4 == 0) && (d->Cin % 4 == 0) && (((uintptr_t)x & 15) == 0);
    p.z_vec = (lddz % 4 == 0) && (d->Cout % 4 == 0) && (((uintptr_t)dz & 15) == 0);
    hipStream_t s = (hipStream_t)stream;
    int pps = (int)((M + splits - 1) / splits);
    if (pl.direct) {
        p.ci_tiles = (d->Cin + 32 * pl.ai - 1) / (32 * pl.ai);
        p.pix_per_split = (pps + 7) / 8 * 8;
        const int co_tiles = (d->Cout + 32 * pl.bj - 1) / (32 * pl.bj);
        p.slabs = splits;
        const dim3 grid((unsigned)(d->KH * d->KW * p.ci_tiles * co_tiles * splits));
#define DS_WG(A, B) if (pl.ai == A && pl.bj == B) hipLaunchKernelGGL((wgrad_direct_kernel<A, B>), grid, dim3(256), 0, s, p);
        DS_WG(4, 4) DS_WG(4, 2) DS_WG(4, 1) DS_WG(2, 4) DS_WG(2, 2) DS_WG(2, 1) DS_WG(1, 4) DS_WG(1, 2) DS_WG(1, 1)
#undef DS_WG
    } else {
        const int ti = pick_ti(d);
        p.ci_tiles = (d->Cin + ti - 1) / ti;
        p.pix_per_split = ((pps + TP - 1) / TP) * TP;
        dim3 grid(d->KH * d->KW * p.ci_tiles, (d->Cout + TJ - 1) / TJ, splits);
        if (ti == 64) hipLaunchKernelGGL(conv_wgrad_kernel<64>, grid, dim3(256), 0, s, p);
        else hipLaunchKernelGGL(conv_wgrad_kernel<128>, grid, dim3(256), 0, s, p);
    }
    if (splits > 1) {
        const int64_t n = (int64_t)d->KH * d->KW * d->Cin * d->Cout;
        hipLaunchKernelGGL(splitk_reduce_kernel, dim3(ds::stream_grid(n, 256)), dim3(256), 0, s,
                           (const float *)ws, dw, n, splits);
    }
    return ds::check_launch("ds_conv_wgrad");
}
```

tumblr_emotions_amd/csrc/text_misc.hip:

```cpp
#include <stdlib.h>
#include "ds_common.h"

namespace {

template <int VEC, bool NT = true, bool OUTORDER = false>
__global__ __launch_bounds__(256) void gather_rows_kernel(const float *table, const int64_t *ids, float *out, int B,
                                                          int T, int D, int64_t rows, int time_major, int rpw) {
    typedef float vec_t __attribute__((ext_vector_type(VEC)));
    const int lane = threadIdx.x & 63;
    const int64_t wave = ((int64_t)blockIdx.x * 256 + threadIdx.x) >> 6;
    const int64_t total = (int64_t)B * T;
    int64_t r = wave * rpw;
    const int64_t r1 = r + rpw < total ? r + rpw : total;
    if (r >= r1) return;
    const int DV = D / VEC;
    int b, t;
    if (OUTORDER) { t = (int)(r / B); b = (int)(r - (int64_t)t * B); }
    else { b = (int)(r / T); t = (int)(r - (int64_t)b * T); }
    constexpr int U = 4;
    if (VEC == 4 && DV <= 128) {
        const float *srcA[U], *srcB[U];
        float *dstA[U], *dstB[U];
        bool okA[U], okB[U];
        vec_t a0[U], a1[U], b0[U], b1[U];
// ... 10 lines not shown
            }
#pragma unroll
            for (int u = 0; u < U; ++u) {
                v0[u] = vec_t(0.f);
                v1[u] = vec_t(0.f);
                if (lane < DV && ok[u]) v0[u] = *reinterpret_cast<const vec_t *>(src[u] + lane * VEC);
                if (64 + lane < DV && ok[u]) v1[u] = *reinterpret_cast<const vec_t *>(src[u] + (64 + lane) * VEC);
            }
        };
        auto put = [&](float *(&dst)[U], vec_t (&v0)[U], vec_t (&v1)[U]) {
#pragma unroll
            for (int u = 0; u < U; ++u) {
                if (!dst[u]) continue;
                if (lane < DV) {
                    if (NT) __builtin_nontemporal_store(v0[u], reinterpret_cast<vec_t *>(dst[u] + lane * VEC));
                    else *reinterpret_cast<vec_t *>(dst[u] + lane * VEC) = v0[u];
                }
                if (64 + lane < DV) {
                    if (NT) __builtin_nontemporal_store(v1[u], reinterpret_cast<vec_t *>(dst[u] + (64 + lane) * VEC));
                    else *reinterpret_cast<vec_t *>(dst[u] + (64 + lane) * VEC) = v1[u];
                }
            }
        };
        fetch(r, srcA, dstA, okA, a0, a1);
        for (; r < r1; r += 2 * U) {
            if (r + U < r1) fetch(r + U, srcB, dstB, okB, b0, b1);
            put(dstA, a0, a1);
            if (r + U >= r1) break;
            if (r + 2 * U < r1) fetch(r + 2 * U, srcA, dstA, okA, a0, a1);
            put(dstB, b0, b1);
        }
        return;
    }
    for (; r < r1; r += U) {
        const float *src[U];
        float *dst[U];
        bool ok[U];
#pragma unroll
        for (int u = 0; u < U; ++u) {
            const bool in = r + u < r1;
            const int64_t id = in ? ids[OUTORDER ? (int64_t)b * T + t : r + u] : -1;
            ok[u] = id >= 0 && id < rows;
            src[u] = table + (ok[u] ? id : 0) * D;
            dst[u] = in ? out + (OUTORDER ? r + u : (time_major ? (int64_t)t * B + b : r + u)) * D : nullptr;
            if (OUTORDER) { if (++b == B) { b = 0; ++t; } }
            else if (++t == T) { t = 0; ++b; }
        }
        for (int v0 = 0; v0 < DV; v0 += 64) {
            const int v = v0 + lane;
            vec_t val[U];
#pragma unroll
            for (int u = 0; u < U; ++u) {
                val[u] = vec_t(0.f);
                if (v < DV && ok[u]) val[u] = *reinterpret_cast<const vec_t *>(src[u] + v * VEC);
            }
#pragma unroll
            for (int u = 0; u < U; ++u)
                if (v < DV && dst[u]) {
                    if (NT) __builtin_nontemporal_store(val[u], reinterpret_cast<vec_t *>(dst[u] + v * VEC));
                    else *reinterpret_cast<vec_t *>(dst[u] + v * VEC) = val[u];
                }
        }
    }
}

template <int NQ>
__global__ __launch_bounds__(256) void embedding_grad_kernel(const float *dx, const int64_t *ids, float *dtable, int B,
                                                             int T, int D, int64_t rows, int time_major) {
    const int lane = threadIdx.x & 63;
    const int64_t v = (int64_t)blockIdx.x * 4 + (threadIdx.x >> 6);
    if (v >= rows) return;
    float acc[NQ];
#pragma unroll
    for (int q = 0; q < NQ; ++q) acc[q] = 0.f;
    const int BT = B * T;
    for (int base = 0; base < BT; base += 64) {
        const int pos = base + lane;
        const int64_t id = pos < BT ? ids[pos] : -1;
        unsigned long long mask = __ballot(id == v);
        while (mask) {
            const int j = __ffsll((long long)mask) - 1;
            mask &= mask - 1;
            const int p = base + j;
            const int b = p / T, t = p - b * T;
            const float *src = dx + (time_major ? (int64_t)t * B + b : (int64_t)p) * D;
#pragma unroll
            for (int q = 0; q < NQ; ++q) {
                const int c = lane + 64 * q;
                if (c < D) acc[q] += src[c];
            }
        }
    }
#pragma unroll
    for (int q = 0; q < NQ; ++q) {
        const int c = lane + 64 * q;
        if (c < D) dtable[v * D + c] = acc[q];
    }
}

__device__ __forceinline__ float sigmoidf_(float x) { return 1.f / (1.f + __expf(-x)); }

__global__ __launch_bounds__(256) void lstm_cell_fwd_kernel(float *gates, const float *rec, int nslabs,
                                                            int64_t slab_stride, const float *c_prev,
                                                            const float *h_prev, const int64_t *seq_len, int t, int B,
                                                            int H, float forget_bias, float *c_out, float *h_out) {
    const int64_t total = (int64_t)B * H;
    for (int64_t i = (int64_t)blockIdx.x * 256 + threadIdx.x; i < total; i += (int64_t)gridDim.x * 256) {
        const int b = (int)(i / H), h = (int)(i - (int64_t)b * H);
        float *g = gates + (int64_t)b * 4 * H + h;
        float pi = g[0], pj = g[H], pf = g[2 * H], po = g[3 * H];
        for (int s = 0; s < nslabs; ++s) {
            const float *r = rec + s * slab_stride + (int64_t)b * 4 * H + h;
            pi += r[0]; pj += r[H]; pf += r[2 * H]; po += r[3 * H];
        }
        const float si = sigmoidf_(pi);
        const float tj = tanhf(pj);
        const float sf = sigmoidf_(pf + forget_bias);
        const float so = sigmoidf_(po);
        const float cp = c_prev[i], hp = h_prev[i];
        const float cn = cp * sf + si * tj;
        const float hn = tanhf(cn) * so;
        const bool live = (int64_t)t < seq_len[b];
        g[0] = si;
        g[H] = tj;
        g[2 * H] = sf;
        g[3 * H] = so;
        c_out[i] = live ? cn : cp;
        h_out[i] = live ? hn : hp;
    }
}

__global__ __launch_bounds__(256) void lstm_cell_bwd_kernel(const float *acts, const float *c_t, const float *c_prev,
                                                            const float *dh, const float *dh_slabs, int nslabs,
                                                            int64_t slab_stride, const float *dc,
                                                            const int64_t *seq_len, int t, int B, int H,
                                                            float *dgates, float *dc_prev, float *dh_carry) {
    const int64_t total = (int64_t)B * H;
    for (int64_t i = (int64_t)blockIdx.x * 256 + threadIdx.x; i < total; i += (int64_t)gridDim.x * 256) {
        const int b = (int)(i / H), h = (int)(i - (int64_t)b * H);
        const float *a = acts + (int64_t)b * 4 * H + h;
        float *dg = dgates + (int64_t)b * 4 * H + h;
        const bool live = (int64_t)t < seq_len[b];
        float dhv = dh[i];
        for (int s = 0; s < nslabs; ++s) dhv += dh_slabs[s * slab_stride + i];
        const float dcv = dc[i];
        if (live) {
            const float si = a[0], tj = a[H], sf = a[2 * H], so = a[3 * H];
            const float tc = tanhf(c_t[i]);
            const float dct = dcv + dhv * so * (1.f - tc * tc);
            dg[0] = dct * tj * si * (1.f - si);
            dg[H] = dct * si * (1.f - tj * tj);
            dg[2 * H] = dct * c_prev[i] * sf * (1.f - sf);
            dg[3 * H] = dhv * tc * so * (1.f - so);
            dc_prev[i] = dct * sf;
            dh_carry[i] = 0.f;
        } else {
            dg[0] = 0.f;
            dg[H] = 0.f;
            dg[2 * H] = 0.f;
            dg[3 * H] = 0.f;
            dc_prev[i] = dcv;
            dh_carry[i] = dhv;
        }
    }
}

__global__ __launch_bounds__(256) void softmax_ce_kernel(const float *logits, const int64_t *labels, int B, int C,
                                                         float grad_scale, const float *grad_scale_dev,
                                                         float *loss, float *dlogits) {
    __shared__ float red[256];
    if (grad_scale_dev) grad_scale *= grad_scale_dev[0];
    float acc = 0.f;
    for (int b = threadIdx.x; b < B; b += 256) {
        const float *z = logits + (int64_t)b * C;
        float m = -INFINITY;
        for (int c = 0; c < C; ++c) m = fmaxf(m, z[c]);
        float s = 0.f;
        for (int c = 0; c < C; ++c) s += expf(z[c] - m);
        const int64_t yl = labels[b];
        const bool yok = yl >= 0 && yl < C;
        const int y = yok ? (int)yl : -1;
        acc += yok ? (m + logf(s)) - z[y] : NAN;
        if (dlogits) {
            const float k = grad_scale / (float)B, inv = 1.f / s;
            for (int c = 0; c < C; ++c)
                dlogits[(int64_t)b * C + c] = (expf(z[c] - m) * inv - (c == y ? 1.f : 0.f)) * k;
        }
    }
    red[threadIdx.x] = acc;
    __syncthreads();
    for (int o = 128; o > 0; o >>= 1) {
        if (threadIdx.x < o) red[threadIdx.x] += red[threadIdx.x + o];
        __syncthreads();
    }
    if (threadIdx.x == 0 && loss) loss[0] = red[0] / (float)B;
}

__global__ __launch_bounds__(256) void adam_tf_kernel(float *theta, const float *g, float *m, float *v, int64_t n,
                                                      int64_t n_wd, float wd, float grad_scale, float lr_t,
                                                      const float *lr_t_dev, float b1, float b2, float eps) {
    if (lr_t_dev) lr_t = lr_t_dev[0];
    for (int64_t i = (int64_t)blockIdx.x * 256 + threadIdx.x; i < n; i += (int64_t)gridDim.x * 256) {
        const float w = theta[i];
        float gi = g[i] * grad_scale;
        if (i < n_wd) gi += wd * w;
        const float mi = b1 * m[i] + (1.f - b1) * gi;
        const float vi = b2 * v[i] + (1.f - b2) * gi * gi;
        m[i] = mi;
        v[i] = vi;
        theta[i] = w - lr_t * mi / (sqrtf(vi) + eps);
    }
}

constexpr int kAccumVecPerBlock = 256 * 4;

template <int MODE>
__global__ __launch_bounds__(256) void grad_accumulate_kernel(float4 *acc, float4 *g, int64_t n4) {
    for (int64_t i = (int64_t)blockIdx.x * 256 + threadIdx.x; i < n4; i += (int64_t)gridDim.x * 256) {
        const float4 b = g[i];
        if (MODE == 0) {
            acc[i] = b;
        } else {
            const float4 a = acc[i];
            const float4 s = make_float4(a.x + b.x, a.y + b.y, a.z + b.z, a.w + b.w);
            if (MODE == 1) acc[i] = s;
            else g[i] = s;
        }
    }
}

constexpr int kSumsqBlocks = 256;

__global__ __launch_bounds__(256) void sumsq_stage1(const float *x, int64_t n, float *partials) {
    __shared__ float red[256];
    float acc = 0.f;
    for (int64_t i = (int64_t)blockIdx.x * 256 + threadIdx.x; i < n; i += (int64_t)gridDim.x * 256) acc += x[i] * x[i];
    red[threadIdx.x] = acc;
    __syncthreads();
    for (int o = 128; o > 0; o >>= 1) {
        if (threadIdx.x < o) red[threadIdx.x] += red[threadIdx.x + o];
        __syncthreads();
    }
    if (threadIdx.x == 0) partials[blockIdx.x] = red[0];
}

__global__ __launch_bounds__(256) void sum_stage2(const float *partials, int n, float *out) {
    __shared__ double red[256];
    double acc = 0.0;
    for (int i = threadIdx.x; i < n; i += 256) acc += (double)partials[i];
    red[threadIdx.x] = acc;
    __syncthreads();
    for (int o = 128; o > 0; o >>= 1) {
        if (threadIdx.x < o) red[threadIdx.x] += red[threadIdx.x + o];
        __syncthreads();
    }
    if (threadIdx.x == 0) out[0] = (float)red[0];
}

__global__ __launch_bounds__(256) void colsum_stage1(const float *x, int64_t M, int C, int ld, int rows_per_split,
                                                     float *partials) {
    __shared__ float red[4][64];
    const int cl = threadIdx.x & 63, rl = threadIdx.x >> 6;
    const int c = blockIdx.x * 64 + cl;
    const int64_t r0 = (int64_t)blockIdx.y * rows_per_split;
    int64_t r1 = r0 + rows_per_split;
    if (r1 > M) r1 = M;
    float acc = 0.f;
    if (c < C)
        for (int64_t r = r0 + rl; r < r1; r += 4) acc += x[r * ld + c];
    red[rl][cl] = acc;
    __syncthreads();
    if (rl == 0 && c < C) partials[(int64_t)blockIdx.y * C + c] = red[0][cl] + red[1][cl] + red[2][cl] + red[3][cl];
}

__global__ __launch_bounds__(256) void colsum_small_kernel(const float *x, int64_t M, int C, int ld, int rows_per_split,
                                                           int RS, float *out) {
    __shared__ float red[4][64];
    const int cl = threadIdx.x & 63, rl = threadIdx.x >> 6;
    const int c = blockIdx.x * 64 + cl;
    double total = 0.0;
    for (int s = 0; s < RS; ++s) {
        const int64_t r0 = (int64_t)s * rows_per_split;
        int64_t r1 = r0 + rows_per_split;
        if (r1 > M) r1 = M;
        float acc = 0.f;
        if (c < C)
            for (int64_t r = r0 + rl; r < r1; r += 4) acc += x[r * ld + c];
        __syncthreads();
        red[rl][cl] = acc;
        __syncthreads();
        if (rl == 0) total += (double)(red[0][cl] + red[1][cl] + red[2][cl] + red[3][cl]);
    }
    if (rl == 0 && c < C) out[c] = (float)total;
}

__global__ __launch_bounds__(256) void colsum_stage2(const float *partials, int RS, int C, float *out) {
    const int c = blockIdx.x * 256 + threadIdx.x;
    if (c >= C) return;
    double acc = 0.0;
    for (int s = 0; s < RS; ++s) acc += (double)partials[(int64_t)s * C + c];
    out[c] = (float)acc;
}

__global__ __launch_bounds__(256) void copy2d_kernel(const float *src, int lds, float *dst, int ldd, int64_t rows,
                                                     int cols) {
    const int64_t total = rows * cols;
    for (int64_t i = (int64_t)blockIdx.x * 256 + threadIdx.x; i < total; i += (int64_t)gridDim.x * 256) {
        const int64_t r = i / cols;
        const int c = (int)(i - r * cols);
        dst[r * ldd + c] = src[r * lds + c];
    }
}

__global__ __launch_bounds__(256) void pad_channels_kernel(const float *src, int cs, float *dst, int cd,
                                                           int64_t pixels) {
    const int64_t total = pixels * cd;
    for (int64_t i = (int64_t)blockIdx.x * 256 + threadIdx.x; i < total; i += (int64_t)gridDim.x * 256) {
        const int64_t p = i / cd;
        const int c = (int)(i - p * cd);
        dst[i] = c < cs ? src[p * cs + c] : 0.f;
    }
}

__global__ __launch_bounds__(256) void fill_kernel(float *dst, int64_t n, float value) {
    for (int64_t i = (int64_t)blockIdx.x * 256 + threadIdx.x; i < n; i += (int64_t)gridDim.x * 256) dst[i] = value;
}

template <int VEC>
__global__ __launch_bounds__(256) void token_dot_kernel(const float *dx, const float *x, const int64_t *seq_len, float *out,
                                                        int B, int T, int D) {
    const int lane = threadIdx.x & 63;
    const int64_t row = (int64_t)blockIdx.x * 4 + (threadIdx.x >> 6);
    if (row >= (int64_t)T * B) return;
    const int t = (int)(row / B), b = (int)(row - (int64_t)t * B);
    float acc = 0.f;
    if ((int64_t)t < seq_len[b]) {
        const float *a = dx + row * D, *e = x + row * D;
        if (VEC == 4) {
            for (int d = lane * 4; d < D; d += 256) {
                const float4 u = *reinterpret_cast<const float4 *>(a + d), v = *reinterpret_cast<const float4 *>(e + d);
                acc = __builtin_fmaf(u.x, v.x, acc);
                acc = __builtin_fmaf(u.y, v.y, acc);
                acc = __builtin_fmaf(u.z, v.z, acc);
                acc = __builtin_fmaf(u.w, v.w, acc);
            }
        } else {
            for (int d = lane; d < D; d += 64) acc = __builtin_fmaf(a[d], e[d], acc);
        }
        acc = ds::wave_sum(acc);
    }
    if (lane == 0) out[(int64_t)b * T + t] = acc;
}

}

extern "C" int ds_gather_rows(const float *table, const int64_t *ids, float *out, int32_t B, int32_t T, int32_t D,
                              int64_t table_rows, int32_t time_major, void *stream) {
    DS_REQUIRE(table && ids && out && B > 0 && T > 0 && D > 0 && table_rows > 0, "ds_gather_rows: bad argument");
    hipStream_t s = (hipStream_t)stream;
    const bool a16 = (((uintptr_t)table | (uintptr_t)out) & 15) == 0, a8 = (((uintptr_t)table | (uintptr_t)out) & 7) == 0;
    const int64_t total = (int64_t)B * T;
    int rpw = (int)((total + (int64_t)ds::kCUs * 32 * 4 - 1) / ((int64_t)ds::kCUs * 32 * 4));
    rpw = rpw < 4 ? 4 : (rpw > 16 ? 16 : rpw);
    const int64_t waves = (total + rpw - 1) / rpw;
    const dim3 grid((unsigned)((waves + 3) / 4));
    static int plain = -1;
    if (plain < 0) {
        const char *e = ds::tune_env("DS_GATHER_PLAIN_STORES");
        plain = e ? atoi(e) : 0;
    }
    static int outorder = -1;
    if (outorder < 0) {
        const char *e = ds::tune_env("DS_GATHER_OUTORDER");
        outorder = e ? atoi(e) : 1;
    }
    if (D % 4 == 0 && a16 && !plain && time_major && outorder == 1) {
        hipLaunchKernelGGL((gather_rows_kernel<4, true, true>), grid, dim3(256), 0, s, table, ids, out, B, T, D, table_rows, time_major, rpw);
    } else if (D % 4 == 0 && a16 && time_major && outorder == 2) {
        hipLaunchKernelGGL((gather_rows_kernel<4, false, true>), grid, dim3(256), 0, s, table, ids, out, B, T, D, table_rows, time_major, rpw);
    } else if (D % 4 == 0 && a16 && plain) {
        hipLaunchKernelGGL((gather_rows_kernel<4, false>), grid, dim3(256), 0, s, table, ids, out, B, T, D, table_rows, time_major, rpw);
    } else if (D % 4 == 0 && a16) {
        hipLaunchKernelGGL(gather_rows_kernel<4>, grid, dim3(256), 0, s, table, ids, out, B, T, D, table_rows, time_major, rpw);
    } else if (D % 2 == 0 && a8) {
        hipLaunchKernelGGL(gather_rows_kernel<2>, grid, dim3(256), 0, s, table, ids, out, B, T, D, table_rows, time_major, rpw);
    } else {
        hipLaunchKernelGGL(gather_rows_kernel<1>, grid, dim3(256), 0, s, table, ids, out, B, T, D, table_rows, time_major, rpw);
    }
    return ds::check_launch("ds_gather_rows");
}

extern "C" int ds_token_dot(const float *dx, const float *x, const int64_t *seq_len, float *out, int32_t B, int32_t T,
                            int32_t D, void *stream) {
    DS_REQUIRE(dx && x && seq_len && out && B > 0 && T > 0 && D > 0, "ds_token_dot: bad argument");
    const int64_t rows = (int64_t)B * T;
    const dim3 grid((unsigned)((rows + 3) / 4));
    if (D % 4 == 0 && ((((uintptr_t)dx) | ((uintptr_t)x)) & 15) == 0)
        hipLaunchKernelGGL(token_dot_kernel<4>, grid, dim3(256), 0, (hipStream_t)stream, dx, x, seq_len, out, B, T, D);
    else
        hipLaunchKernelGGL(token_dot_kernel<1>, grid, dim3(256), 0, (hipStream_t)stream, dx, x, seq_len, out, B, T, D);
    return ds::check_launch("ds_token_dot");
}

extern "C" int ds_embedding_grad(const float *dx, const int64_t *ids, float *dtable, int32_t B, int32_t T, int32_t D,
                                 int64_t table_rows, int32_t time_major, void *stream) {
    DS_REQUIRE(dx && ids && dtable && B > 0 && T > 0 && D > 0 && D <= 512 && table_rows > 0,
               "ds_embedding_grad: bad argument (D <= 512)");
    const dim3 grid((unsigned)((table_rows + 3) / 4)), block(256);
    hipStream_t s = (hipStream_t)stream;
    if (D <= 64) hipLaunchKernelGGL(embedding_grad_kernel<1>, grid, block, 0, s, dx, ids, dtable, B, T, D, table_rows, time_major);
    else if (D <= 128) hipLaunchKernelGGL(embedding_grad_kernel<2>, grid, block, 0, s, dx, ids, dtable, B, T, D, table_rows, time_major);
    else if (D <= 320) hipLaunchKernelGGL(embedding_grad_kernel<5>, grid, block, 0, s, dx, ids, dtable, B, T, D, table_rows, time_major);
    else hipLaunchKernelGGL(embedding_grad_kernel<8>, grid, block, 0, s, dx, ids, dtable, B, T, D, table_rows, time_major);
    return ds::check_launch("ds_embedding_grad");
}

extern "C" int ds_lstm_cell_fwd(float *gates, const float *rec_slabs, int32_t nslabs, int64_t slab_stride,
                                const float *c_prev, const float *h_prev, const int64_t *seq_len, int32_t t, int32_t B,
                                int32_t H, float forget_bias, float *c_out, float *h_out, void *stream) {
    DS_REQUIRE(gates && c_prev && h_prev && seq_len && c_out && h_out && B > 0 && H > 0 && nslabs >= 0 &&
                   (nslabs == 0 || rec_slabs),
               "ds_lstm_cell_fwd: bad argument");
    hipLaunchKernelGGL(lstm_cell_fwd_kernel, dim3(ds::stream_grid((int64_t)B * H, 256)), dim3(256), 0,
                       (hipStream_t)stream, gates, rec_slabs, nslabs, slab_stride, c_prev, h_prev, seq_len, t, B, H,
                       forget_bias, c_out, h_out);
    return ds::check_launch("ds_lstm_cell_fwd");
}

extern "C" int ds_lstm_cell_bwd(const float *acts, const float *c_t, const float *c_prev, const float *dh,
                                const float *dh_slabs, int32_t nslabs, int64_t slab_stride, const float *dc,
                                const int64_t *seq_len, int32_t t, int32_t B, int32_t H, float *dgates,
                                float *dc_prev, float *dh_carry, void *stream) {
    DS_REQUIRE(acts && c_t && c_prev && dh && dc && seq_len && dgates && dc_prev && dh_carry && nslabs >= 0 &&
                   (nslabs == 0 || dh_slabs),
               "ds_lstm_cell_bwd: bad argument");
    hipLaunchKernelGGL(lstm_cell_bwd_kernel, dim3(ds::stream_grid((int64_t)B * H, 256)), dim3(256), 0,
                       (hipStream_t)stream, acts, c_t, c_prev, dh, dh_slabs, nslabs, slab_stride, dc, seq_len, t, B,
                       H, dgates, dc_prev, dh_carry);
    return ds::check_launch("ds_lstm_cell_bwd");
}

extern "C" int ds_softmax_ce(const float *logits, const int64_t *labels, int32_t B, int32_t C, float grad_scale,
                             const float *grad_scale_dev, float *loss, float *dlogits, void *stream) {
    DS_REQUIRE(logits && labels && B > 0 && C > 0, "ds_softmax_ce: bad argument");
    hipLaunchKernelGGL(softmax_ce_kernel, dim3(1), dim3(256), 0, (hipStream_t)stream, logits, labels, B, C, grad_scale,
                       grad_scale_dev, loss, dlogits);
    return ds::check_launch("ds_softmax_ce");
}

extern "C" int ds_adam_tf(float *theta, const float *g, float *m, float *v, int64_t n, int64_t n_wd, float wd,
                          float grad_scale, float lr_t, const float *lr_t_dev, float beta1, float beta2, float eps,
                          void *stream) {
    DS_REQUIRE(theta && g && m && v && n > 0 && n_wd >= 0 && n_wd <= n, "ds_adam_tf: bad argument");
    hipLaunchKernelGGL(adam_tf_kernel, dim3(ds::stream_grid(n, 256)), dim3(256), 0, (hipStream_t)stream, theta, g, m, v,
                       n, n_wd, wd, grad_scale, lr_t, lr_t_dev, beta1, beta2, eps);
    return ds::check_launch("ds_adam_tf");
}

extern "C" int ds_grad_accumulate(float *acc, float *g, int64_t n, int32_t mode, void *stream) {
    DS_REQUIRE(acc && g, "ds_grad_accumulate: null pointer");
    DS_REQUIRE(n > 0 && n % 4 == 0, "ds_grad_accumulate: n must be a positive multiple of 4 (got %lld)", (long long)n);
    DS_REQUIRE(mode >= 0 && mode <= 2, "ds_grad_accumulate: mode must be 0 (first), 1 (middle) or 2 (last), not %d", (int)mode);
    DS_REQUIRE(((uintptr_t)acc | (uintptr_t)g) % 16 == 0, "ds_grad_accumulate: acc and g must be 16-byte aligned");
    const int64_t n4 = n / 4;
    const dim3 grid(ds::stream_grid(n4, kAccumVecPerBlock)), block(256);
    float4 *a4 = reinterpret_cast<float4 *>(acc), *g4 = reinterpret_cast<float4 *>(g);
    if (mode == 0) hipLaunchKernelGGL(grad_accumulate_kernel<0>, grid, block, 0, (hipStream_t)stream, a4, g4, n4);
    else if (mode == 1) hipLaunchKernelGGL(grad_accumulate_kernel<1>, grid, block, 0, (hipStream_t)stream, a4, g4, n4);
    else hipLaunchKernelGGL(grad_accumulate_kernel<2>, grid, block, 0, (hipStream_t)stream, a4, g4, n4);
    return ds::check_launch("ds_grad_accumulate");
}

extern "C" int ds_sumsq(const float *x, int64_t n, float *scratch, float *out, void *stream) {
    DS_REQUIRE(x && scratch && out && n > 0, "ds_sumsq: bad argument");
    int blocks = ds::stream_grid(n, 256 * 8);
    if (blocks > kSumsqBlocks) blocks = kSumsqBlocks;
    hipLaunchKernelGGL(sumsq_stage1, dim3(blocks), dim3(256), 0, (hipStream_t)stream, x, n, scratch);
    hipLaunchKernelGGL(sum_stage2, dim3(1), dim3(256), 0, (hipStream_t)stream, scratch, blocks, out);
    return ds::check_launch("ds_sumsq");
}

__global__ __launch_bounds__(256) void seq_sort_desc_kernel(const int64_t *seq_len, int B, int T, int *perm, int64_t *len_sorted) {
    extern __shared__ int lens[];
    for (int i = threadIdx.x; i < B; i += 256) {
        const int64_t l = seq_len[i];
        lens[i] = (int)(l < 0 ? 0 : (l > T ? T : l));
    }
    __syncthreads();
    for (int i = threadIdx.x; i < B; i += 256) {
        const int li = lens[i];
        int rank = 0;
        for (int j = 0; j < B; ++j) {
            const int lj = lens[j];
            rank += (lj > li || (lj == li && j < i)) ? 1 : 0;
        }
        perm[rank] = i;
        len_sorted[rank] = li;
    }
}

template <typename E>
__global__ __launch_bounds__(256) void permute_rows_kernel(const E *src, int64_t lds, E *dst, int64_t ldd, const int *perm,
                                                           int rows, int cols, int gather) {
    const int64_t total = (int64_t)rows * cols;
    for (int64_t i = (int64_t)blockIdx.x * 256 + threadIdx.x; i < total; i += (int64_t)gridDim.x * 256) {
        const int r = (int)(i / cols), c = (int)(i - (int64_t)r * cols);
        const int pr = perm[r];
        if (gather) dst[(int64_t)r * ldd + c] = src[(int64_t)pr * lds + c];
        else dst[(int64_t)pr * ldd + c] = src[(int64_t)r * lds + c];
    }
}

extern "C" int ds_seq_sort_desc(const int64_t *seq_len, int32_t B, int32_t T, int32_t *perm, int64_t *len_sorted, void *stream) {
    DS_REQUIRE(seq_len && perm && len_sorted && B > 0 && B <= 4096 && T > 0, "ds_seq_sort_desc: bad argument (1 <= B <= 4096)");
    hipLaunchKernelGGL(seq_sort_desc_kernel, dim3(1), dim3(256), (size_t)B * sizeof(int), (hipStream_t)stream, seq_len, B, T, perm,
                       len_sorted);
    return ds::check_launch("ds_seq_sort_desc");
}

extern "C" int ds_permute_rows(const void *src, int64_t lds, void *dst, int64_t ldd, const int32_t *perm, int32_t rows, int32_t cols,
                               int32_t elem_bytes, int32_t gather, void *stream) {
    DS_REQUIRE(src && dst && perm && rows > 0 && cols > 0 && lds >= cols && ldd >= cols && (elem_bytes == 4 || elem_bytes == 8),
               "ds_permute_rows: bad argument (elem_bytes 4 or 8)");
    const int grid = ds::stream_grid((int64_t)rows * cols, 256);
    if (elem_bytes == 4)
        hipLaunchKernelGGL(permute_rows_kernel<float>, dim3(grid), dim3(256), 0, (hipStream_t)stream, (const float *)src, lds,
                           (float *)dst, ldd, perm, rows, cols, gather);
    else
        hipLaunchKernelGGL(permute_rows_kernel<int64_t>, dim3(grid), dim3(256), 0, (hipStream_t)stream, (const int64_t *)src, lds,
                           (int64_t *)dst, ldd, perm, rows, cols, gather);
    return ds::check_launch("ds_permute_rows");
}

extern "C" int ds_colsum(const float *x, int64_t M, int32_t C, int32_t ld, float *scratch, float *out, void *stream) {
    DS_REQUIRE(x && scratch && out && M > 0 && C > 0 && ld >= C, "ds_colsum: bad argument");
    int RS = (int)((M + 63) / 64);
    if (RS > 64) RS = 64;
    const int rps = (int)((M + RS - 1) / RS);
    if (RS <= 8) {
        hipLaunchKernelGGL(colsum_small_kernel, dim3((C + 63) / 64), dim3(256), 0, (hipStream_t)stream, x, M, C, ld, rps, RS, out);
        return ds::check_launch("ds_colsum");
    }
    hipLaunchKernelGGL(colsum_stage1, dim3((C + 63) / 64, RS), dim3(256), 0, (hipStream_t)stream, x, M, C, ld, rps,
                       scratch);
    hipLaunchKernelGGL(colsum_stage2, dim3((C + 255) / 256), dim3(256), 0, (hipStream_t)stream, scratch, RS, C, out);
    return ds::check_launch("ds_colsum");
}

__global__ __launch_bounds__(256) void slab_epilogue_kernel(const float *slabs, int splits, int64_t slab_stride, int lds,
                                                            int64_t M, int N, float *out, int ldo, const float *bias,
                                                            const float *mask, int ldmask, int flags) {
    const int64_t total = M * N;
    for (int64_t i = (int64_t)blockIdx.x * 256 + threadIdx.x; i < total; i += (int64_t)gridDim.x * 256) {
        const int64_t m = i / N;
        const int n = (int)(i - m * N);
        float v = 0.f;
        for (int k = 0; k < splits; ++k) v += slabs[(int64_t)k * slab_stride + m * lds + n];
        if (flags & DS_EPI_BIAS) v += bias[n];
        const int64_t o = m * ldo + n;
        if (flags & DS_EPI_ACCUM) v += out[o];
        if (flags & DS_EPI_MASK) v = mask[m * ldmask + n] > 0.f ? v : 0.f;
        if (flags & DS_EPI_RELU) v = fmaxf(v, 0.f);
        out[o] = v;
    }
}

extern "C" int ds_slab_epilogue(const float *slabs, int32_t splits, int64_t slab_stride, int32_t lds, int64_t M, int32_t N,
                                float *out, int32_t ldo, const float *bias, const float *mask, int32_t ldmask, int32_t flags,
                                void *stream) {
    DS_REQUIRE(slabs && out && splits >= 1 && M > 0 && N > 0 && lds >= N && ldo >= N, "ds_slab_epilogue: bad argument");
    DS_REQUIRE((flags & ~(DS_EPI_BIAS | DS_EPI_ACCUM | DS_EPI_MASK | DS_EPI_RELU)) == 0 && (!(flags & DS_EPI_BIAS) || bias) &&
                   (!(flags & DS_EPI_MASK) || (mask && ldmask >= N)),
               "ds_slab_epilogue: flags are BIAS / ACCUM / MASK / RELU (with their operands)");
    hipLaunchKernelGGL(slab_epilogue_kernel, dim3(ds::stream_grid(M * N, 256)), dim3(256), 0, (hipStream_t)stream, slabs, splits,
                       slab_stride, lds, M, N, out, ldo, bias, mask, ldmask, flags);
    return ds::check_launch("ds_slab_epilogue");
}

extern "C" int ds_copy2d(const float *src, int32_t lds, float *dst, int32_t ldd, int64_t rows, int32_t cols,
                         void *stream) {
    DS_REQUIRE(src && dst && rows > 0 && cols > 0, "ds_copy2d: bad argument");
    hipLaunchKernelGGL(copy2d_kernel, dim3(ds::stream_grid(rows * cols, 256)), dim3(256), 0, (hipStream_t)stream, src,
                       lds, dst, ldd, rows, cols);
    return ds::check_launch("ds_copy2d");
}

extern "C" int ds_pad_channels(const float *src, int32_t cs, float *dst, int32_t cd, int64_t pixels, void *stream) {
    DS_REQUIRE(src && dst && cs > 0 && cd >= cs && pixels > 0, "ds_pad_channels: bad argument");
    hipLaunchKernelGGL(pad_channels_kernel, dim3(ds::stream_grid(pixels * cd, 256)), dim3(256), 0, (hipStream_t)stream,
                       src, cs, dst, cd, pixels);
    return ds::check_launch("ds_pad_channels");
}

extern "C" int ds_fill(float *dst, int64_t n, float value, void *stream) {
    DS_REQUIRE(dst && n > 0, "ds_fill: bad argument");
    hipLaunchKernelGGL(fill_kernel, dim3(ds::stream_grid(n, 256)), dim3(256), 0, (hipStream_t)stream, dst, n, value);
    return ds::check_launch("ds_fill");
}
```

tumblr_emotions_amd/engine_text.py:

```python
import ctypes as C

import torch

from . import _lib, ops
from .ops import WgradPlan, gemm_plan, head_gemm_plan, DS_EPI_ACCUM, DS_EPI_BIAS, DS_EPI_MASK, DS_EPI_RELU

FORGET_BIAS = 1.0


def _vp(addr):
    return C.c_void_p(addr)


def _gemm_wgrad(M, K, N, lda, lddz):
    return WgradPlan(M, 1, 1, K, lda, 1, 1, 1, N, lddz, pad_t=0, pad_l=0, OH=1, OW=1)


class TextTowerEngine:
    KERNEL = "Text/rnn/basic_lstm_cell/kernel"
    BIAS = "Text/rnn/basic_lstm_cell/bias"
    EMB = "Text/W_embedding"

    def __init__(self, store, vocab_rows, embed_dim, rnn_size, post_size, device="cuda", trainable_embedding=False):
        self.store, self.V, self.D, self.H, self.T = store, vocab_rows, embed_dim, rnn_size, post_size
        self.device = torch.device(device)
        self.trainable_embedding = trainable_embedding
        store.declare(self.EMB, (vocab_rows, embed_dim), trainable_embedding, bucket=1)
        store.declare(self.KERNEL, (embed_dim + rnn_size, 4 * rnn_size), True, bucket=1)
        store.declare(self.BIAS, (4 * rnn_size,), True, bucket=1)
        self.B = None
        self.reducer = None
        self.persistent = True
        self.seq_rows = 1
        self.sort_by_length = _lib.tuning_env("DS_LSTM_SORT", "1") != "0" 

    def alloc(self, B):
        if self.B == B:
            return
        dev, T, D, H = self.device, self.T, self.D, self.H
        self.B = B
        self.alloc_gen = getattr(self, "alloc_gen", 0) + 1
        self.use_seq = self.persistent and ops.lstm_seq_supported(B, H)
        self.sorted = bool(self.use_seq and self.sort_by_length)
        if self.sorted:
            self.perm = torch.empty(B, dtype=torch.int32, device=dev)
            self.len_sorted = torch.empty(B, dtype=torch.int64, device=dev)
            self.texts_sorted = torch.empty(B, T, dtype=torch.int64, device=dev)
            self.h_last = torch.empty(B, H, device=dev)
            self.dh_sorted = torch.empty(B, H, device=dev)
        self.seq_ws = torch.zeros(max(ops.lstm_seq_workspace(B, H) // 4, 4), dtype=torch.int32, device=dev)
        self.x = torch.empty(T * B, D, device=dev)
        self.gates = torch.empty(T, B, 4 * H, device=dev)
        self.dgates = torch.empty(T, B, 4 * H, device=dev)
        self.h = torch.zeros(T + 1, B, H, device=dev)
        self.c = torch.zeros(T + 1, B, H, device=dev)
        self.dh = [torch.empty(B, H, device=dev), torch.empty(B, H, device=dev)]
        self.dc = torch.empty(B, H, device=dev)
        st = self.store
        self.table = st.view(self.EMB)
        kptr = st.ptr(self.KERNEL)
        self.wx, self.wh = _vp(kptr), _vp(kptr + 4 * D * 4 * H)
        self.bias = _vp(st.ptr(self.BIAS))
        gk = st.grad_ptr(self.KERNEL)
        self.gwx, self.gwh = _vp(gk), _vp(gk + 4 * D * 4 * H)
        self.gbias = st.grad_view(self.BIAS)
        self.xproj = gemm_plan(T * B, D, 4 * H, D, 4 * H, 4 * H, flags=DS_EPI_BIAS)
        def nsplit(m, n, k):
            blocks = -(-m // 128) * -(-n // 32)
            return int(max(1, min(512 // max(blocks, 1), (k // 16) // 4)))
        self.sf, self.sb = nsplit(B, 4 * H, H), nsplit(B, H, 4 * H)
        self.rec_slabs = torch.empty(self.sf, B, 4 * H, device=dev)
        self.dh_slabs = torch.empty(self.sb, B, H, device=dev)
        self.rec = gemm_plan(B, H, 4 * H, H, 4 * H, 4 * H, splits=self.sf, z_split_stride=B * 4 * H)
        self.rec_dgrad = gemm_plan(B, 4 * H, H, 4 * H, H, 4 * H, transposed_w=True, splits=self.sb,
                                   z_split_stride=B * H)
        self.wgrad_x = _gemm_wgrad(T * B, D, 4 * H, D, 4 * H)
        self.wgrad_h = _gemm_wgrad(T * B, H, 4 * H, H, 4 * H)
        self.ws_bytes = max(self.wgrad_x.ws_bytes, self.wgrad_h.ws_bytes)
        self.ws = torch.empty(max(self.ws_bytes // 4, 4), device=dev)
        self.colsum_scratch = torch.empty(64 * 4 * H, device=dev)
        self.dx = None
        if self.trainable_embedding:
            self._ensure_dx()
            self.gtable = st.grad_view(self.EMB)

    def _ensure_dx(self):
        if self.dx is None:
            B, T, D, H = self.B, self.T, self.D, self.H
            self.dx = torch.empty(T * B, D, device=self.device)
            self.x_dgrad = gemm_plan(T * B, 4 * H, D, 4 * H, D, 4 * H, transposed_w=True)
            self.tok = torch.empty(B, T, device=self.device)

    def forward(self, texts, seq_lens, scale=None):
        B, T, H = texts.shape[0], self.T, self.H
        assert texts.shape[1] == T and texts.dtype == torch.int64 and seq_lens.dtype == torch.int64
        self.alloc(B)
        if self.sorted:
            if not seq_lens.is_contiguous() or not texts.is_contiguous():
                seq_lens, texts = seq_lens.contiguous(), texts.contiguous()
            ops.seq_sort_desc(seq_lens, B, T, self.perm, self.len_sorted)
            ops.permute_rows(texts, self.texts_sorted, self.perm, B, T, gather=True)
            seq_lens, texts = self.len_sorted, self.texts_sorted
        self.seq_lens, self.texts = seq_lens, texts
        ops.gather_rows(self.table, texts, self.x, B, T, self.D, time_major=True)
        if scale is not None:
            if tuple(scale.shape) != (B,) or scale.dtype != torch.float32:
                raise ValueError("scale must be a float32 [%d] tensor" % B)
            if self.sorted:
                scale = scale[self.perm.long()]
            self.x.view(T, B, self.D).mul_(scale.view(1, B, 1))
        self.xproj.run(ops._p(self.x), self.wx, ops._p(self.gates), bias=self.bias)
        if self.use_seq:
            rows = self.seq_rows | (_lib.DS_LSTM_SKIP_MASKED if self.sorted else 0)
            ops.lstm_seq_fwd(self.gates, self.wh, 4 * H, self.h, self.c, seq_lens, T, B, H, FORGET_BIAS, self.seq_ws, rows=rows)
            if self.sorted:
                ops.permute_rows(self.h[T], self.h_last, self.perm, B, H, gather=False)
                return self.h_last
            return self.h[T]
        slab = B * 4 * H
        for t in range(T):
            ns = 0
            if t > 0:
                self.rec.run(ops._p(self.h[t]), self.wh, ops._p(self.rec_slabs))
                ns = self.sf
            ops.lstm_cell_fwd(self.gates[t], self.c[t], self.h[t], seq_lens, t, B, H, FORGET_BIAS, self.c[t + 1],
                              self.h[t + 1], self.rec_slabs, ns, slab)
        return self.h[T]

    def check_status(self):
        if self.B is not None and self.use_seq:
            ops.lstm_seq_status(self.seq_ws, self.B)

    def backward(self, dh_last):
        self._bptt(dh_last)
        self._weight_grads()

    def input_backward(self, dh_last):
        B, T, D, H = self.B, self.T, self.D, self.H
        self._bptt(dh_last)
        self._ensure_dx()
        self.x_dgrad.run(ops._p(self.dgates), self.wx, ops._p(self.dx))
        ops.token_dot(self.dx, self.x, self.seq_lens, self.tok, B, T, D)
        live = torch.arange(T, device=self.device).view(1, T) < self.seq_lens.view(B, 1)
        dwords = torch.where(live.unsqueeze(-1), self.dx.view(T, B, D).permute(1, 0, 2), self.dx.new_zeros(()))
        scores = self.tok
        if self.sorted:
            order = torch.empty_like(self.perm, dtype=torch.int64)
            order[self.perm.long()] = torch.arange(B, device=self.device)
            dwords, scores = dwords[order], scores[order]
        return dwords.contiguous(), scores.clone()

    def _bptt(self, dh_last):
        B, T, H = self.B, self.T, self.H
        if self.use_seq:
            rows = self.seq_rows
            if self.sorted:
                ops.permute_rows(dh_last, self.dh_sorted, self.perm, B, H, gather=True)
                dh_last, rows = self.dh_sorted, rows | _lib.DS_LSTM_SKIP_MASKED
            ops.lstm_seq_bwd(self.gates, self.wh, 4 * H, self.c, dh_last, dh_last.stride(0), self.seq_lens, T, B, H,
                             self.dgates, self.seq_ws, rows=rows)
            return
        dh, dh2 = self.dh
        ops.copy2d(dh_last, dh_last.stride(0), dh, H, B, H)
        ops.fill(self.dc, B * H, 0.0)
        ns = 0
        for t in range(T - 1, -1, -1):
            ops.lstm_cell_bwd(self.gates[t], self.c[t + 1], self.c[t], dh, self.dc, self.seq_lens, t, B, H,
                              self.dgates[t], self.dc, dh2, self.dh_slabs, ns, B * H)
            if t > 0:
                self.rec_dgrad.run(ops._p(self.dgates[t]), self.wh, ops._p(self.dh_slabs))
                ns = self.sb
            dh, dh2 = dh2, dh

    def _weight_grads(self):
        B, T, H = self.B, self.T, self.H
        dg = ops._p(self.dgates)
        self.wgrad_x.run(ops._p(self.x), dg, self.gwx, ops._p(self.ws), self.ws_bytes)
        self.wgrad_h.run(ops._p(self.h), dg, self.gwh, ops._p(self.ws), self.ws_bytes)
        ops.colsum(self.dgates, T * B, 4 * H, 4 * H, self.colsum_scratch, self.gbias)
        if self.trainable_embedding:
            self.x_dgrad.run(dg, self.wx, ops._p(self.dx))
            ops.embedding_grad(self.dx, self.texts, self.gtable, B, T, self.D, time_major=True)
        if self.reducer is not None:
            self.reducer.stage_done("text")


class JointHeadEngine:

    def __init__(self, store, im_size, tx_size, fc_size, nb_emotions, device="cuda"):
        self.store, self.im, self.tx, self.fc, self.nc = store, im_size, tx_size, fc_size, nb_emotions
        self.device = torch.device(device)
        store.declare("W_fc", (im_size + tx_size, fc_size), True, bucket=1)
        store.declare("b_fc", (fc_size,), True, bucket=1)
        store.declare("W_softmax", (fc_size, nb_emotions), True, bucket=1)
        store.declare("b_softmax", (nb_emotions,), True, bucket=1)
        self.B = None
        self.reducer = None

    def alloc(self, B):
        if self.B == B:
            return
        dev, im, tx, fc, nc = self.device, self.im, self.tx, self.fc, self.nc
        self.B = B
        self.alloc_gen = getattr(self, "alloc_gen", 0) + 1
        self.dense = torch.empty(B, fc, device=dev)
        self.ddense = torch.empty(B, fc, device=dev)
        self.logits = torch.empty(B, nc, device=dev)
        self.d_im = torch.empty(B, im, device=dev)
        self.d_tx = torch.empty(B, tx, device=dev)
        st = self.store
        w = st.ptr("W_fc")
        self.w_im, self.w_tx = _vp(w), _vp(w + 4 * im * fc)
        gw = st.grad_ptr("W_fc")
        self.gw_im, self.gw_tx = _vp(gw), _vp(gw + 4 * im * fc)
        self.b_fc, self.gb_fc = _vp(st.ptr("b_fc")), st.grad_view("b_fc")
        self.w_sm, self.gw_sm = _vp(st.ptr("W_softmax")), _vp(st.grad_ptr("W_softmax"))
        self.b_sm, self.gb_sm = _vp(st.ptr("b_softmax")), st.grad_view("b_softmax")
        self.fc_im = None
        self.ws_bytes = 0
        self.colsum_scratch = torch.empty(64 * max(fc, nc), device=dev)

    def _plans(self, ld_im, ld_tx):
        B, im, tx, fc, nc = self.B, self.im, self.tx, self.fc, self.nc
        self.fc_im = head_gemm_plan(B, im, fc, ld_im, fc, fc, device=self.device)
        self.fc_tx = head_gemm_plan(B, tx, fc, ld_tx, fc, fc, flags=DS_EPI_ACCUM | DS_EPI_BIAS | DS_EPI_RELU, device=self.device)
        self.sm = head_gemm_plan(B, fc, nc, fc, nc, nc, flags=DS_EPI_BIAS, device=self.device)
        self.sm_dgrad = head_gemm_plan(B, nc, fc, nc, fc, nc, transposed_w=True, flags=DS_EPI_MASK, ldmask=fc, device=self.device)
        self.sm_wgrad = _gemm_wgrad(B, fc, nc, fc, nc)
        self.im_dgrad = head_gemm_plan(B, fc, im, fc, im, fc, transposed_w=True, device=self.device)
        self.tx_dgrad = head_gemm_plan(B, fc, tx, fc, tx, fc, transposed_w=True, device=self.device)
        self.im_wgrad = _gemm_wgrad(B, im, fc, ld_im, fc)
        self.tx_wgrad = _gemm_wgrad(B, tx, fc, ld_tx, fc)
        self.ws_bytes = max(p.ws_bytes for p in (self.sm_wgrad, self.im_wgrad, self.tx_wgrad))
        self.ws = torch.empty(max(self.ws_bytes // 4, 4), device=self.device)
        self._lds = (ld_im, ld_tx)

    def forward(self, im_feat, tx_feat):
        B = im_feat.shape[0]
        self.alloc(B)
        lds = (im_feat.stride(0), tx_feat.stride(0))
        if self.fc_im is None or self._lds != lds:
            self._plans(*lds)
        self.im_feat, self.tx_feat = im_feat, tx_feat
        self.fc_im.run(ops._p(im_feat), self.w_im, ops._p(self.dense))
        self.fc_tx.run(ops._p(tx_feat), self.w_tx, ops._p(self.dense), bias=self.b_fc)
        self.sm.run(ops._p(self.dense), self.w_sm, ops._p(self.logits), bias=self.b_sm)
        return self.logits

    def backward(self, dlogits):
        B, fc, nc = self.B, self.fc, self.nc
        dl, ws = ops._p(dlogits), ops._p(self.ws)
        self.sm_wgrad.run(ops._p(self.dense), dl, self.gw_sm, ws, self.ws_bytes)
        ops.colsum(dlogits, B, nc, nc, self.colsum_scratch, self.gb_sm)
        self.sm_dgrad.run(dl, self.w_sm, ops._p(self.ddense), mask=ops._p(self.dense))
        dd = ops._p(self.ddense)
        self.im_wgrad.run(ops._p(self.im_feat), dd, self.gw_im, ws, self.ws_bytes)
        self.tx_wgrad.run(ops._p(self.tx_feat), dd, self.gw_tx, ws, self.ws_bytes)
        ops.colsum(self.ddense, B, fc, fc, self.colsum_scratch, self.gb_fc)
        self.im_dgrad.run(dd, self.w_im, ops._p(self.d_im))
        self.tx_dgrad.run(dd, self.w_tx, ops._p(self.d_tx))
        if self.reducer is not None:
            self.reducer.stage_done("head")
        return self.d_im, self.d_tx

    def input_backward(self, dlogits, with_text=False):
        self.sm_dgrad.run(ops._p(dlogits), self.w_sm, ops._p(self.ddense), mask=ops._p(self.dense))
        self.im_dgrad.run(ops._p(self.ddense), self.w_im, ops._p(self.d_im))
        if with_text:
            self.tx_dgrad.run(ops._p(self.ddense), self.w_tx, ops._p(self.d_tx))
            return self.d_im, self.d_tx
        return self.d_im


class TextHeadEngine:

    def __init__(self, store, rnn_size, nb_emotions, device="cuda"):
        self.store, self.H, self.nc = store, rnn_size, nb_emotions
        self.device = torch.device(device)
        store.declare("W_softmax", (rnn_size, nb_emotions), True, bucket=1)
        store.declare("b_softmax", (nb_emotions,), True, bucket=1)
        self.B = None
        self.reducer = None

    def alloc(self, B):
        if self.B == B:
            return
        dev, H, nc = self.device, self.H, self.nc
        self.B = B
        self.alloc_gen = getattr(self, "alloc_gen", 0) + 1
        self.logits = torch.empty(B, nc, device=dev)
        self.d_tx = torch.empty(B, H, device=dev)
        st = self.store
        self.w_sm, self.gw_sm = _vp(st.ptr("W_softmax")), _vp(st.grad_ptr("W_softmax"))
        self.b_sm, self.gb_sm = _vp(st.ptr("b_softmax")), st.grad_view("b_softmax")
        self.sm = head_gemm_plan(B, H, nc, H, nc, nc, flags=DS_EPI_BIAS, device=self.device)
        self.sm_dgrad = head_gemm_plan(B, nc, H, nc, H, nc, transposed_w=True, device=self.device)
        self.sm_wgrad = _gemm_wgrad(B, H, nc, H, nc)
        self.ws_bytes = self.sm_wgrad.ws_bytes
        self.ws = torch.empty(max(self.ws_bytes // 4, 4), device=dev)
        self.colsum_scratch = torch.empty(64 * max(nc, 4), device=dev)

    def forward(self, tx_feat):
        self.alloc(tx_feat.shape[0])
        assert tx_feat.stride(0) == self.H
        self.tx_feat = tx_feat
        self.sm.run(ops._p(tx_feat), self.w_sm, ops._p(self.logits), bias=self.b_sm)
        return self.logits

    def backward(self, dlogits):
        dl = ops._p(dlogits)
        self.sm_wgrad.run(ops._p(self.tx_feat), dl, self.gw_sm, ops._p(self.ws), self.ws_bytes)
        ops.colsum(dlogits, self.B, self.nc, self.nc, self.colsum_scratch, self.gb_sm)
        self.sm_dgrad.run(dl, self.w_sm, ops._p(self.d_tx))
        if self.reducer is not None:
            self.reducer.stage_done("head")
        return self.d_tx

    def input_backward(self, dlogits):
        self.sm_dgrad.run(ops._p(dlogits), self.w_sm, ops._p(self.d_tx))
        return self.d_tx
```

tumblr_emotions_amd/ops.py:

```python
import ctypes as C
import os

import torch

from . import _lib
from ._lib import (ConvDesc, Segments, SumSegments, DS_EPI_ACCUM, DS_EPI_BIAS, DS_EPI_BNSUMS, DS_EPI_MASK, DS_EPI_RELU,
                   DS_EPI_STATS, DS_EPI_BN_RELU,
                   DS_DTYPE_BF16, DS_DTYPE_F32, DS_FP8_E4M3, DS_FP8_E5M2, DS_CONV_FWD, DS_CONV_DGRAD, DS_ARITH_F32, DS_ARITH_BF16,
                   DS_ARITH_FP8, DS_ARITH_F32X3, DS_FAM_IGEMM, DS_FAM_WINO2, DS_FAM_WINO4, DS_FAM_STEM, DS_FAM_BF16D, DS_FAM_FP8D,
                   DS_FAM_F32X3, DS_FAM_WINO4H, DS_FAM_STEM_POOL, DS_FAM_STEM_DGRAD, DS_PLAN_STEM_POOL, DS_PLAN_NO_SPLITK, DS_PLAN_NO_WINO4H, DS_PLAN_NO_WINO, DS_PLAN_NO_WINO4, DS_PLAN_NO_STEM_DIRECT, DS_PLAN_NO_BF16_DIRECT, DS_PLAN_ACT16,
                   DS_PLAN_PACKED_RGB, DS_PLAN_FP8_EVERYWHERE, DS_PLAN_FP8_WIDE_RULE)


_raw_stream = getattr(torch._C, "_cuda_getCurrentRawStream", None)


def _stream():
    if _raw_stream is not None:
        return C.c_void_p(_raw_stream(torch.cuda.current_device()))
    return C.c_void_p(torch.cuda.current_stream().cuda_stream)


def _p(t):
    if t is None:
# ... 204 lines not shown
            self.u = torch.empty(self.p.w_bytes, dtype=torch.uint8, device=device)
        if self.p.wscale_floats:
            self.wscale = torch.zeros(self.p.wscale_floats, device=device)
            self.io.wscale = self.wscale.data_ptr()

    def set_workspace(self, t):
        assert t.numel() * t.element_size() >= self.ws_bytes
        self._ws = t
        self.io.ws, self.io.ws_bytes = t.data_ptr(), t.numel() * t.element_size()

    def prepare(self, w_hwio):
        if self.u is not None:
            _lib.check(_lib.load().ds_conv_prepare_weights(self._ref, w_hwio, _p(self.u), _p(self.wscale), _stream()),
                       "ds_conv_prepare_weights")

    def enable_bnsums(self, ldy):
        return int(_lib.load().ds_conv_plan_enable_bnsums(self._ref, ldy))

    def norm_supported(self):
        return bool(_lib.load().ds_conv_plan_norm_supported(self._ref))

    def enable_pool3(self, argmax):
        if not _lib.load().ds_conv_plan_enable_pool3(self._ref, _p(argmax)):
            return False
        self.pool_argmax = argmax
        return True

    def copy(self):
        q = object.__new__(LayerPlan)
        q.p = _lib.LayerPlanStruct()
        C.memmove(C.byref(q.p), self._ref, C.sizeof(q.p))
        q._ref = C.byref(q.p)
        q.d, q.family, q.M, q.alg_flops = q.p.d, q.p.family, self.M, self.alg_flops
        q.u, q.wscale, q._ws = self.u, self.wscale, self._ws
        q.io = _lib.ConvIO()
        q.io.ws, q.io.ws_bytes = self.io.ws, self.io.ws_bytes
        q.ws_bytes, q.splitk = self.ws_bytes, self.splitk
        q._run, q._io_ref = self._run, C.byref(q.io)
        q.pool_argmax = getattr(self, "pool_argmax", None)
        return q

    def bn_relu_variant(self, ldz=None):
        q = self.copy()
        q.p.d.flags, q.p.d.partials, q.p.partials = 0, 0, 0
        if ldz is not None:
            q.p.d.ldz = ldz
        if not _lib.load().ds_conv_plan_enable_bn_relu(q._ref):
            return None
        return q

    def run_bn_relu(self, x, w_hwio, y, scale, shift):
        t = CONV_TIMER
        if t is not None:
            t.begin()
        self.io.scale, self.io.shift = scale, shift
        _lib.check(self._run(self._ref, x, w_hwio if self.u is None else self.u.data_ptr(), y, self._io_ref, _stream()),
                   "ds_conv_run")
        if t is not None:
            t.end(self)

    def finalize_tickets(self):
        return int(_lib.load().ds_conv_plan_finalize_tickets(self._ref))

    def enable_bn_backward_on_load(self, mean, rstd, shift, coef, parts):
        if not _lib.load().ds_conv_plan_bnb_supported(self._ref) or len(parts) > 3:
            return False
        if any(c0 % 16 for (c0, _, _, _) in parts):
            return False
        b = _lib.BnBwdOnLoad()
        b.mean, b.rstd, b.shift, b.coef = mean.data_ptr(), rstd.data_ptr(), shift.data_ptr(), coef.data_ptr()
        b.nseg = len(parts)
        for i, (c0, c1, ptr, ld) in enumerate(parts):
            assert c0 == (parts[i - 1][1] if i else 0)
            b.c_end[i], b.ld[i], b.dy[i] = c1, ld, ptr
        self.bnb = b
        self.d.bnb = C.addressof(b)
        return True

    def run(self, x, w_hwio, z, stats=None, pivot=None, mask=None, bias=None, x_amax=None, fin=None):
        t = CONV_TIMER
        if t is not None:
            t.begin()
        io = self.io
        io.stats, io.pivot, io.mask, io.bias, io.x_amax, io.fin = stats, pivot, mask, bias, x_amax, fin
        _lib.check(self._run(self._ref, x, w_hwio if self.u is None else self.u.data_ptr(), z, self._io_ref, _stream()),
                   "ds_conv_run")
        if t is not None:
            t.end(self)


def conv_norm_supported(plan):
    return bool(_lib.load().ds_conv_igemm_norm_supported(C.byref(plan.d)))


def wino4_supported(H, W, Cin, Cout):
    return bool(_lib.load().ds_conv_wino4_supported(H, W, Cin, Cout))


def wino4_prefer(N, H, W, Cin, Cout):
    return bool(_lib.load().ds_conv_wino4_prefer(N, H, W, Cin, Cout))


def wino_transform_weights(w_ptr, u, Cin, Cout, dgrad, f4=False):
    lib = _lib.load()
    if f4:
        _lib.check(lib.ds_wino4_transform_weights(w_ptr, _p(u), Cin, Cout, int(dgrad), _stream()), "ds_wino4_transform_weights")
    else:
        _lib.check(lib.ds_wino_transform_weights(w_ptr, _p(u), Cin, Cout, int(dgrad), _stream()), "ds_wino_transform_weights")


class StemPlan:

    def __init__(self, N, H, W, cin_store, Cout, ldz, bf16=False):
        self.args = (N, H, W, cin_store, Cout, ldz)
        self.bf16 = bf16
        self.flags = DS_EPI_STATS
        OH, OW = (H + 1) // 2, (W + 1) // 2
        self.M = N * OH * OW
        self.partials = (_lib.load().ds_conv_stem_bf16_partials if bf16 else _lib.load().ds_conv_stem_partials)(N, OH, OW)
        self.alg_flops = 2.0 * self.M * Cout * 147

    def run(self, x, w, z, stats=None, pivot=None):
        t = CONV_TIMER
        if t is not None:
            t.begin()
        N, H, W, cs, Cout, ldz = self.args
        f = _lib.load().ds_conv_stem_bf16 if self.bf16 else _lib.load().ds_conv_stem
        _lib.check(f(x, w, z, stats, pivot, N, H, W, cs, Cout, ldz, _stream()), "ds_conv_stem")
        if t is not None:
            t.end(self)


class Bf16Plan:

    def __init__(self, N, H, W, Cin, ldx, k, stride, Cout, ldz, flags=0, pad_t=None, pad_l=None, OH=None, OW=None):
        d = ConvDesc()
        d.dtype = DS_DTYPE_BF16
        d.N, d.H, d.W, d.Cin, d.ldx = N, H, W, Cin, ldx
        d.KH, d.KW, d.stride = k, k, stride
        if OH is None:
            OH, pt = same_pad(H, k, stride)
            OW, pl = same_pad(W, k, stride)
            pad_t = pt if pad_t is None else pad_t
            pad_l = pl if pad_l is None else pad_l
        d.pad_t, d.pad_l, d.OH, d.OW = pad_t, pad_l, OH, OW
        d.Cout, d.ldz, d.flags, d.splits = Cout, ldz, flags, 1
        self.d = d
        lib = _lib.load()
        if not lib.ds_conv_bf16_supported(C.byref(d)):
            raise ValueError("ds_conv_bf16 does not take this geometry")
        self.M = N * OH * OW
        self.partials = lib.ds_conv_bf16_partials(C.byref(d)) if flags & DS_EPI_STATS else 0
        self.alg_flops = 2.0 * self.M * Cout * k * k * Cin

    def set_ldx(self, ldx):
        self.d.ldx = ldx

    @property
    def flags(self):
        return self.d.flags

    @flags.setter
    def flags(self, v):
        self.d.flags = v

    def run(self, x, wb, z, stats=None, pivot=None, mask=None):
        t = CONV_TIMER
        if t is not None:
            t.begin()
        _lib.check(_lib.load().ds_conv_bf16(C.byref(self.d), x, wb, z, mask, stats, pivot, _stream()), "ds_conv_bf16")
        if t is not None:
            t.end(self)


class Fp8Plan(Bf16Plan):

    def __init__(self, N, H, W, Cin, ldx, k, stride, Cout, ldz, flags=0, a_format=DS_FP8_E4M3, **kw):
        super().__init__(N, H, W, Cin, ldx, k, stride, Cout, ldz, flags=flags, **kw)
        lib = _lib.load()
        if not lib.ds_conv_fp8_supported(C.byref(self.d)):
            raise ValueError("ds_conv_fp8 does not take this geometry")
        self.a_format = a_format
        self.partials = lib.ds_conv_fp8_partials(C.byref(self.d)) if flags & DS_EPI_STATS else 0

    def run(self, x, wq, z, stats=None, pivot=None, x_amax=None, wscale=None, mask=None):
        t = CONV_TIMER
        if t is not None:
            t.begin()
        _lib.check(_lib.load().ds_conv_fp8(C.byref(self.d), x, x_amax, self.a_format, wq, wscale, z, mask, stats, pivot,
                                           _stream()), "ds_conv_fp8")
        if t is not None:
            t.end(self)


AMAX_FLOATS = 512
WSCALE_FLOATS = 4 + AMAX_FLOATS


def amax_value(record):
    return float(record.view(-1)[:AMAX_FLOATS:32].max().item())


def absmax(x, n, out, x_dtype=DS_DTYPE_F32):
    if not isinstance(x, C.c_void_p):
        x_dtype = act_dtype(x)
        x = _p(x)
    _lib.check(_lib.load().ds_absmax(x, n, x_dtype, _p(out), _stream()), "ds_absmax")


def weights_fp8_bytes(Cin, Cout, taps, dgrad):
    return int(_lib.load().ds_weights_fp8_bytes(Cin, Cout, taps, int(dgrad)))


def weights_to_fp8(w_ptr, wq, wscale, Cin, Cout, taps, dgrad):
    _lib.check(_lib.load().ds_weights_to_fp8(w_ptr, _p(wq), _p(wscale), Cin, Cout, taps, int(dgrad), _stream()),
               "ds_weights_to_fp8")


def weights_bf16_bytes(Cin, Cout, taps, dgrad):
    return int(_lib.load().ds_weights_bf16_bytes(Cin, Cout, taps, int(dgrad)))


def weights_to_bf16(w_ptr, wb, Cin, Cout, taps, dgrad):
    _lib.check(_lib.load().ds_weights_to_bf16(w_ptr, _p(wb), Cin, Cout, taps, int(dgrad), _stream()),
               "ds_weights_to_bf16")


class F32x3Plan:
    f4 = False

    def __init__(self, N, H, W, Cin, ldx, k, stride, Cout, ldz, flags=0, pad_t=None, pad_l=None, OH=None, OW=None):
        d = ConvDesc()
        d.dtype = DS_DTYPE_F32
        d.N, d.H, d.W, d.Cin, d.ldx = N, H, W, Cin, ldx
        d.KH, d.KW, d.stride = k, k, stride
        if OH is None:
            OH, pt = same_pad(H, k, stride)
            OW, pl = same_pad(W, k, stride)
            pad_t = pt if pad_t is None else pad_t
            pad_l = pl if pad_l is None else pad_l
        d.pad_t, d.pad_l, d.OH, d.OW = pad_t, pad_l, OH, OW
        d.Cout, d.ldz, d.flags, d.splits = Cout, ldz, flags, 1
        self.d = d
        lib = _lib.load()
        if not lib.ds_conv_f32x3_supported(C.byref(d)):
            raise ValueError("ds_conv_f32x3 does not take this geometry")
        self.M = N * OH * OW
        self.partials = lib.ds_conv_f32x3_partials(C.byref(d)) if flags & DS_EPI_STATS else 0
        self.partials_for_sums = lib.ds_conv_f32x3_partials(C.byref(d))
        self.alg_flops = 2.0 * self.M * Cout * k * k * Cin

    def set_ldx(self, ldx):
        self.d.ldx = ldx

    def set_ldz(self, ldz):
        self.d.ldz = ldz

    @property
    def flags(self):
        return self.d.flags

    @flags.setter
    def flags(self, v):
        self.d.flags = v

    def run(self, x, wb, z, stats=None, pivot=None, mask=None):
        t = CONV_TIMER
        if t is not None:
            t.begin()
        _lib.check(_lib.load().ds_conv_f32x3(C.byref(self.d), x, wb, z, mask, stats, pivot, _stream()), "ds_conv_f32x3")
        if t is not None:
            t.end(self)


def weights_f32x3_bytes(Cin, Cout, taps, dgrad):
    return int(_lib.load().ds_weights_f32x3_bytes(Cin, Cout, taps, int(dgrad)))


def weights_to_f32x3(w_ptr, wb, Cin, Cout, taps, dgrad):
    _lib.check(_lib.load().ds_weights_to_f32x3(w_ptr, _p(wb), Cin, Cout, taps, int(dgrad), _stream()), "ds_weights_to_f32x3")


class WgradPlan:

    def __init__(self, N, H, W, Cin, ldx, KH, KW, stride, Cout, lddz, pad_t=None, pad_l=None, OH=None, OW=None,
                 fold_cin=0):
        d = ConvDesc()
        d.fold_cin = fold_cin
        d.N, d.H, d.W, d.Cin, d.ldx = N, H, W, Cin, ldx
        d.KH, d.KW, d.stride = KH, KW, stride
        if OH is None:
            OH, pad_t = same_pad(H, KH, stride)
            OW, pad_l = same_pad(W, KW if not fold_cin else Cin // fold_cin, stride)
        d.pad_t, d.pad_l, d.OH, d.OW = pad_t, pad_l, OH, OW
        d.Cout, d.ldz = Cout, Cout
        self.d = d
        self.lddz = lddz
        self.ws_bytes = int(_lib.load().ds_conv_wgrad_workspace(C.byref(d)))

    def run(self, x, dz, dw, ws, ws_bytes):
        _lib.check(_lib.load().ds_conv_wgrad(C.byref(self.d), x, dz, self.lddz, dw, ws, ws_bytes, _stream()),
                   "ds_conv_wgrad")


def bn_finalize(stats, P, count, C_, beta, eps, decay, mean, rstd, shift, mm, mv, pivot=None):
    _lib.check(_lib.load().ds_bn_finalize(_p(stats), P, count, C_, _p(beta), _p(pivot), eps, decay, _p(mean),
                                          _p(rstd), _p(shift), _p(mm), _p(mv), _stream()), "ds_bn_finalize")


def bn_finalize_centered(stats, P, count, C_, beta, eps, decay, mean, rstd, shift, mm, mv, pivot, mean_c, shift_c):
    _lib.check(_lib.load().ds_bn_finalize_centered(_p(stats), P, count, C_, _p(beta), _p(pivot), eps, decay, _p(mean), _p(rstd),
                                                   _p(shift), _p(mm), _p(mv), _p(mean_c), _p(shift_c), _stream()),
               "ds_bn_finalize_centered")


def bn_apply_relu(z, M, C_, rstd, shift, segs):
    if z.dtype == torch.bfloat16:
        _lib.check(_lib.load().ds_bn_apply_relu_z16(_p(z), M, C_, _p(rstd), _p(shift), C.byref(segs), _stream()),
                   "ds_bn_apply_relu_z16")
        return
    _lib.check(_lib.load().ds_bn_apply_relu(_p(z), M, C_, _p(rstd), _p(shift), C.byref(segs), _stream()),
               "ds_bn_apply_relu")


def bn_infer_prepare(beta, mm, mv, eps, C_, rstd, shift):
    _lib.check(_lib.load().ds_bn_infer_prepare(_p(beta), _p(mm), _p(mv), eps, C_, _p(rstd), _p(shift), _stream()),
               "ds_bn_infer_prepare")


class BnInferJobs:

    def __init__(self, jobs):
        self.n = len(jobs)
        self.arr = (_lib.BnInferJob * self.n)()
        self._keep = jobs
        for a, (beta, mm, mv, C_, rstd, shift) in zip(self.arr, jobs):
            a.beta, a.moving_mean, a.moving_var, a.C = _p(beta), _p(mm), _p(mv), C_
            a.rstd, a.shift = _p(rstd), _p(shift)

    def run(self, eps):
        _lib.check(_lib.load().ds_bn_infer_prepare_multi(C.cast(self.arr, C.c_void_p), self.n, eps, _stream()),
                   "ds_bn_infer_prepare_multi")


def bn_bwd_partials(M, C_):
    return _lib.load().ds_bn_bwd_partials(M, C_)


def bn_bwd_reduce(z, segs, M, C_, mean, rstd, shift, partials, ldz=None, z_dtype=DS_DTYPE_F32):
    ptr = lambda t: t if isinstance(t, C.c_void_p) else _p(t)
    if not isinstance(z, C.c_void_p):
        z_dtype = act_dtype(z)
    _lib.check(_lib.load().ds_bn_bwd_reduce(ptr(z), C_ if ldz is None else ldz, z_dtype, C.byref(segs), M, C_, ptr(mean),
                                            ptr(rstd), ptr(shift), ptr(partials), _stream()), "ds_bn_bwd_reduce")


def bn_bwd_finalize_segs(sum_segs, M, C_, beta, dbeta, coef):
    _lib.check(_lib.load().ds_bn_bwd_finalize_segs(C.byref(sum_segs), M, C_, _p(beta), _p(dbeta), _p(coef), _stream()),
               "ds_bn_bwd_finalize_segs")


class BnFinalizeJobs:

    def __init__(self, jobs):
        self.n = len(jobs)
        self.arr = (_lib.BnFinalizeJob * self.n)()
        self._keep = jobs
        for a, (stats, P, count, C_, beta, pivot, mean, rstd, shift, mm, mv) in zip(self.arr, jobs):
            a.stats, a.P, a.C, a.count = stats.data_ptr(), P, C_, count
            a.beta, a.pivot = beta.data_ptr(), (pivot.data_ptr() if pivot is not None else None)
            a.mean, a.rstd, a.shift = mean.data_ptr(), rstd.data_ptr(), shift.data_ptr()
            a.moving_mean = mm.data_ptr() if mm is not None else None
            a.moving_var = mv.data_ptr() if mv is not None else None

    def run(self, eps, decay):
        _lib.check(_lib.load().ds_bn_finalize_multi(C.cast(self.arr, C.c_void_p), self.n, eps, decay, _stream()),
                   "ds_bn_finalize_multi")


def bn_bwd_finalize_multi(sum_segs, M, C_, betas, dbetas, coef):
    n = sum_segs.nseg
    b = (C.c_void_p * 4)(*[t.data_ptr() for t in betas[:n]])
    d = (C.c_void_p * 4)(*[(t.data_ptr() if t is not None else None) for t in dbetas[:n]])
    _lib.check(_lib.load().ds_bn_bwd_finalize_multi(C.byref(sum_segs), M, C_, C.cast(b, C.c_void_p), C.cast(d, C.c_void_p),
                                                    _p(coef), _stream()), "ds_bn_bwd_finalize_multi")


def bn_finalize_apply_relu(stats, P, count, C_, beta, eps, decay, mean, rstd, shift, mm, mv, pivot, z, M, segs, ticket):
    _lib.check(_lib.load().ds_bn_finalize_apply_relu(_p(stats), P, count, C_, _p(beta), _p(pivot), eps, decay, _p(mean), _p(rstd),
                                                     _p(shift), _p(mm), _p(mv), _p(z), M, C.byref(segs), _p(ticket), _stream()),
               "ds_bn_finalize_apply_relu")


def bn_bwd_finalize_apply(sum_segs, M, C_, beta, dbeta, coef, z, segs, mean, rstd, shift, dz, ticket, amax=None, ldz=0,
                          betas=None, dbetas=None):
    bv = dv = None
    if betas is not None:
        n = sum_segs.nseg
        bv = C.cast((C.c_void_p * 4)(*[t.data_ptr() for t in betas[:n]]), C.c_void_p)
        dv = C.cast((C.c_void_p * 4)(*[(t.data_ptr() if t is not None else None) for t in dbetas[:n]]), C.c_void_p)
    out16 = dz.dtype == torch.bfloat16
    _lib.check(_lib.load().ds_bn_bwd_finalize_apply(C.byref(sum_segs), _p(beta), _p(dbeta), bv, dv, _p(coef), _p(z), ldz or C_,
                                                    C.byref(segs), M, C_, _p(mean), _p(rstd), _p(shift), _p(dz),
                                                    DS_DTYPE_BF16 if out16 else DS_DTYPE_F32, dz.stride(0) if out16 else 0,
                                                    _p(amax), _p(ticket), _stream()), "ds_bn_bwd_finalize_apply")


def bn_bwd_finalize(partials, P, M, C_, dbeta, coef):
    _lib.check(_lib.load().ds_bn_bwd_finalize(_p(partials), P, M, C_, _p(dbeta), _p(coef), _stream()),
               "ds_bn_bwd_finalize")


def bn_bwd_apply(z, segs, M, C_, mean, rstd, shift, coef, dz, amax=None, ldz=0):
    if z.dtype == torch.bfloat16:
        assert dz.dtype == torch.bfloat16
        _lib.check(_lib.load().ds_bn_bwd_apply_z16(_p(z), ldz or C_, C.byref(segs), M, C_, _p(mean), _p(rstd), _p(shift),
                                                   _p(coef), _p(dz), dz.stride(0), _p(amax), _stream()), "ds_bn_bwd_apply_z16")
        return
    if dz.dtype == torch.bfloat16:
        _lib.check(_lib.load().ds_bn_bwd_apply_bf16(_p(z), ldz or C_, C.byref(segs), M, C_, _p(mean), _p(rstd), _p(shift),
                                                    _p(coef), _p(dz), dz.stride(0), _p(amax), _stream()), "ds_bn_bwd_apply_bf16")
        return
    _lib.check(_lib.load().ds_bn_bwd_apply(_p(z), ldz or C_, C.byref(segs), M, C_, _p(mean), _p(rstd), _p(shift), _p(coef),
                                           _p(dz), _p(amax), _stream()), "ds_bn_bwd_apply")


def bn_bwd_apply_cols(z, segs, M, ncols, mean, rstd, shift, coef_g, coef_gx, dz, ldz):
    _lib.check(_lib.load().ds_bn_bwd_apply_cols(_p(z), ldz, C.byref(segs), M, ncols, _p(mean), _p(rstd), _p(shift), _p(coef_g),
                                                _p(coef_gx), _p(dz), _stream()), "ds_bn_bwd_apply_cols")


def bn_infer_bwd_apply(z, segs, M, C_, rstd, shift, dz, ldz=0):
    ptr = lambda t: t if isinstance(t, C.c_void_p) else _p(t)
    _lib.check(_lib.load().ds_bn_infer_bwd_apply(ptr(z), ldz or C_, C.byref(segs), M, C_, ptr(rstd), ptr(shift), ptr(dz),
                                                 _stream()), "ds_bn_infer_bwd_apply")


def bn_infer_bwd_partials(M, C_):
    return _lib.load().ds_bn_infer_bwd_partials(M, C_)


def bn_infer_bwd_apply_sums(z, segs, M, C_, rstd, shift, dz, partials, ldz=0):
    ptr = lambda t: t if isinstance(t, C.c_void_p) else _p(t)
    _lib.check(_lib.load().ds_bn_infer_bwd_apply_sums(ptr(z), ldz or C_, C.byref(segs), M, C_, ptr(rstd), ptr(shift), ptr(dz),
                                                      ptr(partials), _stream()), "ds_bn_infer_bwd_apply_sums")


class BnSumJobs:

    def __init__(self, jobs):
        self.n = len(jobs)
        self.arr = (_lib.BnSumJob * self.n)()
        self._keep = jobs
        for a, (partials, P, C_, dbeta) in zip(self.arr, jobs):
            a.partials = partials if isinstance(partials, int) else partials.data_ptr()
            a.P, a.C, a.dbeta = P, C_, dbeta.data_ptr()

    def run(self):
        _lib.check(_lib.load().ds_bn_dbeta_reduce_multi(C.cast(self.arr, C.c_void_p), self.n, _stream()),
                   "ds_bn_dbeta_reduce_multi")


def maxpool_fwd(x, y, argmax, N, H, W, C_, k, stride, mode="SAME"):
    if mode == "SAME":
        OH, pt = same_pad(H, k, stride)
        OW, pl = same_pad(W, k, stride)
    else:
        OH, OW, pt, pl = (H - k) // stride + 1, (W - k) // stride + 1, 0, 0
    assert x.dtype == y.dtype
    _lib.check(_lib.load().ds_maxpool_fwd(_p(x), _p(y), _p(argmax), N, H, W, C_, k, stride, pt, pl, OH, OW,
                                          act_dtype(x), _stream()), "ds_maxpool_fwd")
    return OH, OW


def maxpool_bn_relu_fwd(z, rstd, shift, y, argmax, N, H, W, C_, k, stride, amax=None):
    OH, pt = same_pad(H, k, stride)
    OW, pl = same_pad(W, k, stride)
    _lib.check(_lib.load().ds_maxpool_bn_relu_fwd(_p(z), _p(rstd), _p(shift), _p(y), _p(argmax), N, H, W, C_, k, stride,
                                                  pt, pl, OH, OW, act_dtype(y), _p(amax), _stream()),
               "ds_maxpool_bn_relu_fwd")
    return OH, OW


def bn_pool_bwd_partials(N, H, W, C_):
    OH, _ = same_pad(H, 3, 2)
    OW, _ = same_pad(W, 3, 2)
    return _lib.load().ds_bn_pool_bwd_partials(N, OH, OW, C_)


def bn_pool_bwd_reduce(z, dpool, argmax, N, H, W, C_, mean, rstd, shift, partials):
    OH, pt = same_pad(H, 3, 2)
    OW, pl = same_pad(W, 3, 2)
    _lib.check(_lib.load().ds_bn_pool_bwd_reduce(_p(z), _p(dpool), _p(argmax), N, H, W, C_, pt, pl, OH, OW, _p(mean),
                                                 _p(rstd), _p(shift), _p(partials), _stream()), "ds_bn_pool_bwd_reduce")


def bn_pool_bwd_apply(z, dpool, argmax, N, H, W, C_, mean, rstd, shift, coef, dz):
    OH, pt = same_pad(H, 3, 2)
    OW, pl = same_pad(W, 3, 2)
    _lib.check(_lib.load().ds_bn_pool_bwd_apply(_p(z), _p(dpool), _p(argmax), N, H, W, C_, pt, pl, OH, OW, _p(mean),
                                                _p(rstd), _p(shift), _p(coef), _p(dz), _stream()), "ds_bn_pool_bwd_apply")


def bn_pool_bwd_apply_cols(z, ldz, dz, lddz, dpool, argmax, Cp, c0, N, H, W, ncols, mean, rstd, shift, coef_g, coef_gx, k):
    OH, pt = same_pad(H, k, 2)
    OW, pl = same_pad(W, k, 2)
    _lib.check(_lib.load().ds_bn_pool_bwd_apply_cols(_p(z), ldz, _p(dz), lddz, _p(dpool), _p(argmax), Cp, c0, N, H, W, pt, pl,
                                                     OH, OW, ncols, _p(mean), _p(rstd), _p(shift), _p(coef_g), _p(coef_gx), k,
                                                     _stream()), "ds_bn_pool_bwd_apply_cols")


def bn_pool_infer_bwd_apply(z, dpool, argmax, N, H, W, C_, rstd, shift, dz):
    OH, pt = same_pad(H, 3, 2)
    OW, pl = same_pad(W, 3, 2)
    _lib.check(_lib.load().ds_bn_pool_infer_bwd_apply(_p(z), _p(dpool), _p(argmax), N, H, W, C_, pt, pl, OH, OW, _p(rstd),
                                                      _p(shift), _p(dz), _stream()), "ds_bn_pool_infer_bwd_apply")


def bn_pool_infer_bwd_apply_sums(z, dpool, argmax, N, H, W, C_, rstd, shift, dz, partials):
    OH, pt = same_pad(H, 3, 2)
    OW, pl = same_pad(W, 3, 2)
    _lib.check(_lib.load().ds_bn_pool_infer_bwd_apply_sums(_p(z), _p(dpool), _p(argmax), N, H, W, C_, pt, pl, OH, OW, _p(rstd),
                                                           _p(shift), _p(dz), _p(partials), _stream()),
               "ds_bn_pool_infer_bwd_apply_sums")


def maxpool_bwd(dy, argmax, dx, accumulate, N, H, W, C_, k, stride, mode="SAME"):
    if dy.dtype == torch.bfloat16:
        assert k == 3 and stride == 1 and mode == "SAME"
        _lib.check(_lib.load().ds_maxpool3_bwd_dy16(_p(dy), _p(argmax), _p(dx), int(accumulate), None, DS_DTYPE_F32, N, H, W, C_,
                                                    None, _stream()), "ds_maxpool3_bwd_dy16")
        return
    if mode == "SAME":
        OH, pt = same_pad(H, k, stride)
        OW, pl = same_pad(W, k, stride)
    else:
        OH, OW, pt, pl = (H - k) // stride + 1, (W - k) // stride + 1, 0, 0
    _lib.check(_lib.load().ds_maxpool_bwd(_p(dy), _p(argmax), _p(dx), int(accumulate), N, H, W, C_, k, stride, pt,
                                          pl, OH, OW, _stream()), "ds_maxpool_bwd")


def maxpool3_bwd_sums_partials(N, W, C_):
    return _lib.load().ds_maxpool3_bwd_sums_partials(N, W, C_)


def maxpool3_bwd_sums(dy, argmax, dx, accumulate, y, N, H, W, C_, partials):
    if dy.dtype == torch.bfloat16:
        _lib.check(_lib.load().ds_maxpool3_bwd_dy16(_p(dy), _p(argmax), _p(dx), int(accumulate), _p(y), act_dtype(y), N, H, W, C_,
                                                    _p(partials), _stream()), "ds_maxpool3_bwd_dy16")
        return
    _lib.check(_lib.load().ds_maxpool3_bwd_sums(_p(dy), _p(argmax), _p(dx), int(accumulate), _p(y), act_dtype(y), N, H, W, C_,
                                                _p(partials), _stream()), "ds_maxpool3_bwd_sums")


def avgpool_dropout_fwd(x, N, HW, C_, keep, seed, mask_in, mask_out, out, seed_dev=None):
    _lib.check(_lib.load().ds_avgpool_dropout_fwd(_p(x), N, HW, C_, keep, seed, _p(seed_dev), _p(mask_in),
                                                  _p(mask_out), _p(out), _stream()), "ds_avgpool_dropout_fwd")


def avgpool_dropout_bwd(dout, mask, N, HW, C_, keep, dx):
    _lib.check(_lib.load().ds_avgpool_dropout_bwd(_p(dout), _p(mask), N, HW, C_, keep, _p(dx), _stream()),
               "ds_avgpool_dropout_bwd")


def gather_rows(table, ids, out, B, T, D, time_major=True):
    _lib.check(_lib.load().ds_gather_rows(_p(table), _p(ids), _p(out), B, T, D, table.shape[0], int(time_major),
                                          _stream()), "ds_gather_rows")


def embedding_grad(dx, ids, dtable, B, T, D, time_major=True):
    _lib.check(_lib.load().ds_embedding_grad(_p(dx), _p(ids), _p(dtable), B, T, D, dtable.shape[0], int(time_major),
                                             _stream()), "ds_embedding_grad")


def token_dot(dx, x, seq_len, out, B, T, D):
    _lib.check(_lib.load().ds_token_dot(_p(dx), _p(x), _p(seq_len), _p(out), B, T, D, _stream()), "ds_token_dot")


def lstm_cell_fwd(gates, c_prev, h_prev, seq_len, t, B, H, forget_bias, c_out, h_out, rec_slabs=None, nslabs=0,
                  slab_stride=0):
    _lib.check(_lib.load().ds_lstm_cell_fwd(_p(gates), _p(rec_slabs), nslabs, slab_stride, _p(c_prev), _p(h_prev),
                                            _p(seq_len), t, B, H, forget_bias, _p(c_out), _p(h_out), _stream()),
               "ds_lstm_cell_fwd")


def lstm_cell_bwd(acts, c_t, c_prev, dh, dc, seq_len, t, B, H, dgates, dc_prev, dh_carry, dh_slabs=None, nslabs=0,
                  slab_stride=0):
    _lib.check(_lib.load().ds_lstm_cell_bwd(_p(acts), _p(c_t), _p(c_prev), _p(dh), _p(dh_slabs), nslabs, slab_stride,
                                            _p(dc), _p(seq_len), t, B, H, _p(dgates), _p(dc_prev), _p(dh_carry),
                                            _stream()), "ds_lstm_cell_bwd")


def lstm_seq_supported(B, H):
    return bool(_lib.load().ds_lstm_seq_supported(B, H))


def lstm_seq_workspace(B, H):
    return int(_lib.load().ds_lstm_seq_workspace(B, H))


def lstm_seq_fwd(gates, wh_ptr, ldw, h, c, seq_len, T, B, H, forget_bias, ws, rows=1):
    _lib.check(_lib.load().ds_lstm_seq_fwd(_p(gates), wh_ptr, ldw, _p(h), _p(c), _p(seq_len), T, B, H, forget_bias,
                                           int(rows), _p(ws), ws.numel() * ws.element_size(), _stream()),
               "ds_lstm_seq_fwd")


def lstm_seq_bwd(acts, wh_ptr, ldw, c, dh_last, ld_dh, seq_len, T, B, H, dgates, ws, rows=1):
    _lib.check(_lib.load().ds_lstm_seq_bwd(_p(acts), wh_ptr, ldw, _p(c), _p(dh_last), ld_dh, _p(seq_len), T, B, H,
                                           _p(dgates), int(rows), _p(ws), ws.numel() * ws.element_size(), _stream()),
               "ds_lstm_seq_bwd")


def seq_sort_desc(seq_len, B, T, perm, len_sorted):
    _lib.check(_lib.load().ds_seq_sort_desc(_p(seq_len), B, T, _p(perm), _p(len_sorted), _stream()), "ds_seq_sort_desc")


def permute_rows(src, dst, perm, rows, cols, gather=True):
    assert src.element_size() == dst.element_size() and src.element_size() in (4, 8)
    _lib.check(_lib.load().ds_permute_rows(_p(src), src.stride(0), _p(dst), dst.stride(0), _p(perm), rows, cols, src.element_size(),
                                           int(bool(gather)), _stream()), "ds_permute_rows")


def lstm_seq_status(ws, B):
    rc = _lib.load().ds_lstm_seq_status(_p(ws), B)
    if rc != 0:
        which = " and ".join(n for b, n in ((1, "forward"), (2, "backward")) if rc > 0 and rc & b) or "status read"
        raise RuntimeError("ds_lstm_seq: a workgroup hand-off of the %s launch timed out (status %d): the LSTM results "
                           "of this step are invalid (a workgroup of a row group never became resident)" % (which, rc))
    return rc


def softmax_ce(logits, labels, B, C_, grad_scale, grad_scale_dev, loss, dlogits):
    _lib.check(_lib.load().ds_softmax_ce(_p(logits), _p(labels), B, C_, grad_scale, _p(grad_scale_dev), _p(loss),
                                         _p(dlogits), _stream()), "ds_softmax_ce")


def adam_tf(theta, g, m, v, n, n_wd, wd, grad_scale, lr_t, b1, b2, eps, lr_t_dev=None):
    _lib.check(_lib.load().ds_adam_tf(_p(theta), _p(g), _p(m), _p(v), n, n_wd, wd, grad_scale, lr_t, _p(lr_t_dev),
                                      b1, b2, eps, _stream()), "ds_adam_tf")


def grad_accumulate(acc, g, n, mode):
    _lib.check(_lib.load().ds_grad_accumulate(_p(acc), _p(g), n, mode, _stream()), "ds_grad_accumulate")


def sumsq(x, n, scratch, out):
    _lib.check(_lib.load().ds_sumsq(_p(x), n, _p(scratch), _p(out), _stream()), "ds_sumsq")


def colsum(x, M, C_, ld, scratch, out):
    _lib.check(_lib.load().ds_colsum(_p(x), M, C_, ld, _p(scratch), _p(out), _stream()), "ds_colsum")


def copy2d(src, lds, dst, ldd, rows, cols):
    _lib.check(_lib.load().ds_copy2d(_p(src), lds, _p(dst), ldd, rows, cols, _stream()), "ds_copy2d")


def pad_channels(src, cs, dst, cd, pixels):
    _lib.check(_lib.load().ds_pad_channels(_p(src), cs, _p(dst), cd, pixels, _stream()), "ds_pad_channels")


def fill(dst, n, value):
    _lib.check(_lib.load().ds_fill(_p(dst), n, value, _stream()), "ds_fill")


def eval_metrics_workspace(B, C_):
    n = _lib.load().ds_eval_metrics_workspace(B, C_)
    _lib.check(min(n, 0), "ds_eval_metrics_workspace")
    return n


def eval_metrics_update(logits, labels, counts, loss_sum, scratch):
    if logits.dtype != torch.float32 or logits.dim() != 2 or logits.stride(1) != 1:
        raise ValueError("eval_metrics_update: logits must be fp32 [B, C] with unit column stride")
    B, C_ = logits.shape
    if labels.dtype != torch.int64 or labels.shape != (B,) or not labels.is_contiguous():
        raise ValueError("eval_metrics_update: labels must be contiguous int64 [B]")
    if counts.dtype != torch.int64 or counts.numel() != C_ * C_ + C_ + 4 or not counts.is_contiguous():
        raise ValueError("eval_metrics_update: counts must be contiguous int64 [C*C + C + 4]")
    if loss_sum.dtype != torch.float64 or loss_sum.numel() != 1:
        raise ValueError("eval_metrics_update: loss_sum must be one float64")
    need = eval_metrics_workspace(B, C_)
    if scratch.numel() * scratch.element_size() < need or not scratch.is_contiguous():
        raise ValueError("eval_metrics_update: scratch is smaller than eval_metrics_workspace(B, C) = %d bytes" % need)
    _lib.check(_lib.load().ds_eval_metrics_update(_p(logits), logits.stride(0), _p(labels), B, C_, _p(counts), _p(loss_sum),
                                                  _p(scratch), _stream()), "ds_eval_metrics_update")


def preprocess_desc_dtype():
    import numpy as np
    return np.dtype([("offset", np.int64), ("height", np.int32), ("width", np.int32),
                     ("scale_y", np.float32), ("scale_x", np.float32)], align=True)


def preprocess_train_desc_dtype():
    import numpy as np
    return np.dtype([("offset", np.int64), ("height", np.int32), ("width", np.int32),
                     ("scale_y", np.float32), ("scale_x", np.float32), ("delta", np.float32), ("factor", np.float32),
                     ("flags", np.uint32), ("reserved", np.uint32)], align=True)


def _check_descs(desc, nbytes, dtype, what):
    import numpy as np
    desc = np.asarray(desc)
    if desc.dtype != dtype or desc.ndim != 1 or desc.size == 0:
        raise ValueError("%s: descriptors must be a non-empty 1-D array of ops.%s()"
                         % (what, "preprocess_train_desc_dtype" if what == "preprocess_train" else "preprocess_desc_dtype"))
    h, w, off = desc["height"].astype(np.int64), desc["width"].astype(np.int64), desc["offset"]
    bad = (h < 1) | (w < 1) | (off < 0) | (off + h * w * 3 > int(nbytes))
    if bad.any():
        i = int(np.flatnonzero(bad)[0])
        raise ValueError("%s: descriptor %d (offset %d, %d x %d pixels) does not fit the byte buffer of %d bytes"
                         % (what, i, int(off[i]), int(h[i]), int(w[i]), int(nbytes)))
    if not (np.isfinite(desc["scale_y"]).all() and np.isfinite(desc["scale_x"]).all()
            and (desc["scale_y"] > 0).all() and (desc["scale_x"] > 0).all()):
        raise ValueError("%s: scales must be finite and positive" % what)
    return desc


def check_preprocess_descs(desc, nbytes):
    _check_descs(desc, nbytes, preprocess_desc_dtype(), "preprocess_eval")


def check_preprocess_train_descs(desc, nbytes):
    import numpy as np
    desc = _check_descs(desc, nbytes, preprocess_train_desc_dtype(), "preprocess_train")
    if not (np.isfinite(desc["delta"]).all() and np.isfinite(desc["factor"]).all() and (desc["factor"] >= 0).all()):
        raise ValueError("preprocess_train: delta and factor must be finite and factor >= 0")
    known = _lib.DS_PREPROCESS_FLIP | _lib.DS_PREPROCESS_SATURATION_FIRST
    if (desc["flags"] & ~np.uint32(known)).any() or desc["reserved"].any():
        raise ValueError("preprocess_train: unknown flag bits (or a non-zero reserved word)")


_preprocess_lut = {}


def preprocess_lut(device):
    import numpy as np
    dev = torch.device(device)
    key = torch.cuda.current_device() if dev.index is None else dev.index
    if key not in _preprocess_lut:
        lut = np.arange(256, dtype=np.float32) / np.float32(255)
        _preprocess_lut[key] = torch.from_numpy(lut).to(torch.device("cuda", key))
    return _preprocess_lut[key]


def _preprocess(what, check, itemsize, image_bytes, desc, out_h, out_w, desc_dev, out):
    import numpy as np
    if not image_bytes.is_cuda:
        raise RuntimeError("tumblr_emotions_amd kernels need CUDA/HIP tensors; there is no CPU fallback")
    if image_bytes.dtype != torch.uint8 or not image_bytes.is_contiguous():
        raise ValueError("%s: image_bytes must be a contiguous uint8 tensor" % what)
    if out_h < 1 or out_w < 1:
        raise ValueError("%s: out_h and out_w must be positive" % what)
    check(desc, image_bytes.numel())
    B = int(np.asarray(desc).size)
    if desc_dev is None:
        desc_dev = torch.from_numpy(np.ascontiguousarray(desc).view(np.uint8)).to(image_bytes.device)
    if desc_dev.numel() * desc_dev.element_size() < B * itemsize or not desc_dev.is_contiguous():
        raise ValueError("%s: desc_dev is smaller than the descriptor table" % what)
    if out is None:
        out = torch.empty((B, out_h, out_w, 3), dtype=torch.float32, device=image_bytes.device)
    if out.dtype != torch.float32 or not out.is_contiguous() or out.numel() != B * out_h * out_w * 3:
        raise ValueError("%s: out must be a contiguous fp32 [B, out_h, out_w, 3] tensor" % what)
    fn = getattr(_lib.load(), "ds_" + what)
    _lib.check(fn(_p(image_bytes), image_bytes.numel(), _p(desc_dev), B, _p(preprocess_lut(image_bytes.device)),
                  _p(out), out_h, out_w, _stream()), "ds_" + what)
    return out


def preprocess_eval(image_bytes, desc, out_h, out_w, desc_dev=None, out=None):
    return _preprocess("preprocess_eval", check_preprocess_descs, preprocess_desc_dtype().itemsize, image_bytes, desc,
                       out_h, out_w, desc_dev, out)


def preprocess_train(image_bytes, desc, out_h, out_w, desc_dev=None, out=None):
    return _preprocess("preprocess_train", check_preprocess_train_descs, preprocess_train_desc_dtype().itemsize,
                       image_bytes, desc, out_h, out_w, desc_dev, out)


JPEG_TEXT_CAPACITY = 50


def jpeg_desc_dtype():
    import numpy as np
    return np.dtype([("coef_offset", np.int64), ("out_offset", np.int64), ("width", np.int32), ("height", np.int32),
                     ("sampling", np.int32), ("y0", np.int32), ("x0", np.int32), ("crop_h", np.int32), ("crop_w", np.int32),
                     ("reserved", np.int32), ("quant", np.uint8, (3, 64))], align=True)


def jpeg_blocks(height, width, sampling):
    if sampling == _lib.DS_JPEG_GREY:
        return -(-width // 8) * -(-height // 8)
    h, v = (2 if sampling in (_lib.DS_JPEG_422, _lib.DS_JPEG_420) else 1), (2 if sampling == _lib.DS_JPEG_420 else 1)
    return -(-width // (8 * h)) * -(-height // (8 * v)) * (h * v + 2)


def check_jpeg_descs(desc, ncoef, nbytes):
    import numpy as np
    desc = np.asarray(desc)
    if desc.dtype != jpeg_desc_dtype() or desc.ndim != 1 or desc.size == 0:
        raise ValueError("jpeg_reconstruct: descriptors must be a non-empty 1-D array of ops.jpeg_desc_dtype()")
    i64 = lambda k: desc[k].astype(np.int64)
    w, h, s = i64("width"), i64("height"), i64("sampling")
    if ((s < 0) | (s > 3) | (w < 1) | (h < 1) | (w > 65535) | (h > 65535)).any() or desc["reserved"].any():
        raise ValueError("jpeg_reconstruct: bad image size or sampling class")
    y0, x0, ch, cw = i64("y0"), i64("x0"), i64("crop_h"), i64("crop_w")
    if ((y0 < 0) | (x0 < 0) | (ch < 1) | (cw < 1) | (y0 + ch > h) | (x0 + cw > w)).any():
        raise ValueError("jpeg_reconstruct: a crop box leaves its image")
    hs, vs = np.where((s == 1) | (s == 2), 2, 1), np.where(s == 2, 2, 1)
    need = -(-w // (8 * hs)) * -(-h // (8 * vs)) * np.where(s == 3, 1, hs * vs + 2) * 64
    co, oo = desc["coef_offset"], desc["out_offset"]
    if ((co < 0) | (co % 8 != 0) | (co + need > int(ncoef))).any():
        raise ValueError("jpeg_reconstruct: coefficients outside the buffer of %d int16 (or an offset that is no multiple of 8)" % int(ncoef))
    end = oo + ch * cw * 3
    if ((oo < 0) | (oo % 4 != 0) | (end > int(nbytes))).any():
        raise ValueError("jpeg_reconstruct: a crop outside the byte buffer of %d bytes (or an offset that is no multiple of 4)" % int(nbytes))
    order = np.argsort(oo, kind="stable")
    if (end[order][:-1] > oo[order][1:]).any():
        raise ValueError("jpeg_reconstruct: two crops overlap in the byte buffer")
    order = np.argsort(co, kind="stable")
    if ((co + need)[order][:-1] > co[order][1:]).any():
        raise ValueError("jpeg_reconstruct: two images share coefficient storage (their planes share the scratch)")
    return desc


def _host_ptr(a):
    return C.c_void_p(a.ctypes.data)


def jpeg_probe(data):
    info = _lib.JpegInfo()
    rc = _lib.load().ds_jpeg_probe(C.cast(C.c_char_p(data), C.c_void_p), len(data), C.byref(info))
    if rc < 0:
        raise ValueError("ds_jpeg_probe: bad argument")
    return info if rc == 0 and info.supported else None


def jpeg_entropy_decode(data, info):
    import numpy as np
    coef = np.empty(int(info.coef_count), np.int16)
    rc = _lib.load().ds_jpeg_entropy_decode(C.cast(C.c_char_p(data), C.c_void_p), len(data), C.byref(info), _host_ptr(coef), coef.size)
    if rc < 0 or rc == _lib.DS_JPEG_MORE:
        raise ValueError("ds_jpeg_entropy_decode: bad argument (%d)" % rc)
    return coef if rc == 0 else None


def jpeg_quant(info):
    import numpy as np
    return np.frombuffer(bytes(info.quant), np.uint8).reshape(3, 64)


def example_parse(rec):
    import numpy as np
    text = np.zeros(JPEG_TEXT_CAPACITY, np.int64)
    f = _lib.ExampleFields()
    rc = _lib.load().ds_example_parse(C.cast(C.c_char_p(rec), C.c_void_p), len(rec), _host_ptr(text), text.size, C.byref(f))
    if rc < 0:
        raise ValueError("ds_example_parse: bad argument")
    if rc != 0:
        return None
    return f.image_offset, f.image_length, text, f.seq_len, f.label, f.post_id, f.day


def jpeg_record_decode(rec, coef):
    import numpy as np
    text = np.zeros(JPEG_TEXT_CAPACITY, np.int64)
    f, info, status = _lib.ExampleFields(), _lib.JpegInfo(), C.c_int32(0)
    rc = _lib.load().ds_jpeg_record_decode(C.cast(C.c_char_p(rec), C.c_void_p), len(rec), _host_ptr(text), text.size, C.byref(f),
                                           C.byref(info), _host_ptr(coef) if coef.size else None, coef.size, C.byref(status))
    if rc < 0:
        raise ValueError("ds_jpeg_record_decode: bad argument")
    if rc != 0:
        return None
    return status.value, info, (f.image_offset, f.image_length, text, f.seq_len, f.label, f.post_id, f.day)


def jpeg_reconstruct_host(coef, desc, out_bytes):
    import numpy as np
    desc = check_jpeg_descs(desc, coef.size, out_bytes.size)
    if coef.dtype != np.int16 or out_bytes.dtype != np.uint8 or not coef.flags.c_contiguous or not out_bytes.flags.c_contiguous:
        raise ValueError("jpeg_reconstruct_host: coef int16 and out_bytes uint8, both contiguous")
    desc = np.ascontiguousarray(desc)
    rc = _lib.load().ds_jpeg_reconstruct_host(_host_ptr(coef), coef.size, _host_ptr(desc), desc.size, _host_ptr(out_bytes), out_bytes.size)
    if rc != 0:
        raise ValueError("ds_jpeg_reconstruct_host: bad descriptor (%d)" % rc)
    return out_bytes


def jpeg_reconstruct(coef, desc, out_bytes, scratch=None, desc_dev=None):
    import numpy as np
    if not (coef.is_cuda and out_bytes.is_cuda):
        raise RuntimeError("tumblr_emotions_amd kernels need CUDA/HIP tensors; there is no CPU fallback")
    if coef.dtype != torch.int16 or out_bytes.dtype != torch.uint8 or not coef.is_contiguous() or not out_bytes.is_contiguous():
        raise ValueError("jpeg_reconstruct: coef must be a contiguous int16 tensor and out_bytes a contiguous uint8 tensor")
    desc = check_jpeg_descs(desc, coef.numel(), out_bytes.numel())
    B = int(desc.size)
    if desc_dev is None:
        desc_dev = torch.from_numpy(np.ascontiguousarray(desc).view(np.uint8)).to(coef.device)
    if desc_dev.numel() * desc_dev.element_size() < B * jpeg_desc_dtype().itemsize or not desc_dev.is_contiguous():
        raise ValueError("jpeg_reconstruct: desc_dev is smaller than the descriptor table")
    if scratch is None:
        scratch = torch.empty(coef.numel(), dtype=torch.uint8, device=coef.device)
    if scratch.dtype != torch.uint8 or not scratch.is_contiguous() or scratch.numel() < coef.numel():
        raise ValueError("jpeg_reconstruct: scratch must be a contiguous uint8 tensor of at least coef.numel() bytes")
    _lib.check(_lib.load().ds_jpeg_reconstruct(_p(coef), coef.numel(), _p(desc_dev), B, _p(out_bytes), out_bytes.numel(),
                                               _p(scratch), scratch.numel(), _stream()), "ds_jpeg_reconstruct")
    return out_bytes


def jpeg_huff_dtype():
    import numpy as np
    return np.dtype([("counts", np.uint8, (16,)), ("values", np.uint8, (256,))])


def jpeg_scan_desc_dtype():
    import numpy as np
    return np.dtype([("coef_offset", np.int64), ("width", np.int32), ("height", np.int32), ("sampling", np.int32),
                     ("first_segment", np.int32), ("segments", np.int32), ("reserved", np.int32), ("quant", np.uint8, (3, 64)),
                     ("dc", jpeg_huff_dtype(), (3,)), ("ac", jpeg_huff_dtype(), (3,))], align=True)


def jpeg_segment_dtype():
    import numpy as np
    return np.dtype([("begin", np.int64), ("end", np.int64), ("first_mcu", np.int32), ("mcus", np.int32)], align=True)


def jpeg_mcus(height, width, sampling):
    h, v = (2 if sampling in (_lib.DS_JPEG_422, _lib.DS_JPEG_420) else 1), (2 if sampling == _lib.DS_JPEG_420 else 1)
    return -(-width // (8 * h)), -(-height // (8 * v))


def jpeg_scan(data):
    import numpy as np
    info, scan = _lib.JpegInfo(), _lib.JpegScanInfo()
    cuts = np.empty(64, np.int64)
    for _ in range(2):
        rc = _lib.load().ds_jpeg_scan(C.cast(C.c_char_p(data), C.c_void_p), len(data), C.byref(info), C.byref(scan), _host_ptr(cuts), cuts.size)
        if rc != _lib.DS_JPEG_MORE:
            break
        cuts = np.empty(int(scan.cut_count), np.int64)
    if rc < 0:
        raise ValueError("ds_jpeg_scan: bad argument")
    return (info, scan, cuts[:int(scan.cut_count)]) if rc == 0 else None


def jpeg_record_scan(rec, cuts):
    import numpy as np
    text = np.zeros(JPEG_TEXT_CAPACITY, np.int64)
    f, info, scan, status = _lib.ExampleFields(), _lib.JpegInfo(), _lib.JpegScanInfo(), C.c_int32(0)
    rc = _lib.load().ds_jpeg_record_scan(C.cast(C.c_char_p(rec), C.c_void_p), len(rec), _host_ptr(text), text.size, C.byref(f),
                                         C.byref(info), C.byref(scan), _host_ptr(cuts) if cuts.size else None, cuts.size,
                                         C.byref(status))
    if rc < 0:
# ... 203 lines not shown
```

Baseline: 19720 samples/s.

## Skip padded timesteps in LSTM weight-gradient GEMMs and bias column sum

Adds a device kernel that counts live sequences per timestep from the sorted lengths. The LSTM input/recurrent weight-gradient kernels and the bias column sum then reduce only over live (t, b) rows, mapping compacted row indices back to time-major rows. This avoids multiplying and summing the zero dgates of padded positions. The cost is per-row index remapping inside the wgrad load loops, an extra tiny launch, and split sizes that are computed on the device.

```diff
diff --git a/include/ds_kernels.h b/include/ds_kernels.h
--- a/include/ds_kernels.h
+++ b/include/ds_kernels.h
@@ -236,6 +236,8 @@
 size_t ds_conv_wgrad_workspace(const ds_conv_desc *d);
 int ds_conv_wgrad(const ds_conv_desc *d, const float *x, const float *dz, int32_t lddz, float *dw,
                   void *ws, size_t ws_bytes, void *stream);
+int ds_conv_wgrad_live(const ds_conv_desc *d, const float *x, const float *dz, int32_t lddz, float *dw,
+                       void *ws, size_t ws_bytes, int32_t B_rows, const int32_t *counts, void *stream);
 
 int ds_bn_finalize(const float *stats, int32_t P, int64_t count, int32_t C, const float *beta, const float *pivot,
                    float eps, float decay, float *mean, float *rstd, float *shift, float *moving_mean,
@@ -391,6 +393,7 @@
 int ds_seq_sort_desc(const int64_t *seq_len, int32_t B, int32_t T, int32_t *perm, int64_t *len_sorted, void *stream);
 int ds_permute_rows(const void *src, int64_t lds, void *dst, int64_t ldd, const int32_t *perm, int32_t rows, int32_t cols,
                     int32_t elem_bytes, int32_t gather, void *stream);
+int ds_seq_live_counts(const int64_t *len, int32_t B, int32_t T, int32_t *counts, void *stream);
 #define DS_LSTM_SKIP_MASKED 256
 int ds_lstm_seq_supported(int32_t B, int32_t H);
 size_t ds_lstm_seq_workspace(int32_t B, int32_t H);
@@ -416,6 +419,8 @@
 
 int ds_sumsq(const float *x, int64_t n, float *scratch, float *out, void *stream);
 int ds_colsum(const float *x, int64_t M, int32_t C, int32_t ld, float *scratch, float *out, void *stream);
+int ds_colsum_live(const float *x, int64_t M, int32_t C, int32_t ld, int32_t B_rows, const int32_t *counts, float *scratch,
+                   float *out, void *stream);
 int ds_slab_epilogue(const float *slabs, int32_t splits, int64_t slab_stride, int32_t lds, int64_t M, int32_t N, float *out,
                      int32_t ldo, const float *bias, const float *mask, int32_t ldmask, int32_t flags, void *stream);
 int ds_copy2d(const float *src, int32_t lds, float *dst, int32_t ldd, int64_t rows, int32_t cols,
diff --git a/tumblr_emotions_amd/_lib.py b/tumblr_emotions_amd/_lib.py
--- a/tumblr_emotions_amd/_lib.py
+++ b/tumblr_emotions_amd/_lib.py
@@ -202,6 +202,7 @@
     "ds_conv_run": (C.c_int, [_LP, _P, _P, _P, _IO, _P]),
     "ds_conv_wgrad_workspace": (C.c_size_t, [_CD]),
     "ds_conv_wgrad": (C.c_int, [_CD, _P, _P, _i32, _P, _P, C.c_size_t, _P]),
+    "ds_conv_wgrad_live": (C.c_int, [_CD, _P, _P, _i32, _P, _P, C.c_size_t, _i32, _P, _P]),
     "ds_bn_finalize": (C.c_int, [_P, _i32, _i64, _i32, _P, _P, _f32, _f32, _P, _P, _P, _P, _P, _P]),
     "ds_bn_finalize_centered": (C.c_int, [_P, _i32, _i64, _i32, _P, _P, _f32, _f32, _P, _P, _P, _P, _P, _P, _P, _P]),
     "ds_bn_apply_relu": (C.c_int, [_P, _i64, _i32, _P, _P, _SG, _P]),
@@ -244,6 +245,7 @@
     "ds_lstm_cell_fwd": (C.c_int, [_P, _P, _i32, _i64, _P, _P, _P, _i32, _i32, _i32, _f32, _P, _P, _P]),
     "ds_lstm_cell_bwd": (C.c_int, [_P, _P, _P, _P, _P, _i32, _i64, _P, _P, _i32, _i32, _i32, _P, _P, _P, _P]),
     "ds_seq_sort_desc": (C.c_int, [_P, _i32, _i32, _P, _P, _P]),
+    "ds_seq_live_counts": (C.c_int, [_P, _i32, _i32, _P, _P]),
     "ds_permute_rows": (C.c_int, [_P, _i64, _P, _i64, _P, _i32, _i32, _i32, _i32, _P]),
     "ds_lstm_seq_supported": (C.c_int, [_i32, _i32]),
     "ds_lstm_seq_workspace": (C.c_size_t, [_i32, _i32]),
@@ -255,6 +257,7 @@
     "ds_grad_accumulate": (C.c_int, [_P, _P, _i64, _i32, _P]),
     "ds_sumsq": (C.c_int, [_P, _i64, _P, _P, _P]),
     "ds_colsum": (C.c_int, [_P, _i64, _i32, _i32, _P, _P, _P]),
+    "ds_colsum_live": (C.c_int, [_P, _i64, _i32, _i32, _i32, _P, _P, _P, _P]),
     "ds_slab_epilogue": (C.c_int, [_P, _i32, _i64, _i32, _i64, _i32, _P, _i32, _P, _P, _i32, _i32, _P]),
     "ds_copy2d": (C.c_int, [_P, _i32, _P, _i32, _i64, _i32, _P]),
     "ds_pad_channels": (C.c_int, [_P, _i32, _P, _i32, _i64, _P]),
diff --git a/tumblr_emotions_amd/csrc/conv_wgrad.hip b/tumblr_emotions_amd/csrc/conv_wgrad.hip
--- a/tumblr_emotions_amd/csrc/conv_wgrad.hip
+++ b/tumblr_emotions_amd/csrc/conv_wgrad.hip
@@ -24,7 +24,11 @@
     unsigned x_bytes, z_bytes;
     float inv_ohw, inv_ow;
     int slabs;
+    const int *counts;
+    int B_rows, T;
 };
+
+constexpr int kLiveMaxT = 256;
 
 constexpr unsigned kOOB = 0x80000000u;
 
@@ -49,7 +53,7 @@
     return q;
 }
 
-template <int TIT>
+template <int TIT, bool LIVE = false>
 __global__ __launch_bounds__(256) void conv_wgrad_kernel(const WgradParams p) {
     constexpr int LDX = TIT + 4, LDZ = TJ + 4;
     constexpr int WNW = TIT == 128 ? 2 : 4;
@@ -72,9 +76,22 @@
     const int split = blockIdx.z;
     const int dh = tap / d.KW, dw = tap % d.KW;
     const int ohw = d.OH * d.OW;
-    const int m_begin = split * p.pix_per_split;
-    int m_end = m_begin + p.pix_per_split;
-    if (m_end > p.M) m_end = p.M;
+    __shared__ int pre[LIVE ? kLiveMaxT + 1 : 1];
+    int M = p.M, pix_per_split = p.pix_per_split;
+    if constexpr (LIVE) {
+        for (int i = tid; i <= p.T; i += 256) pre[i] = p.counts[p.T + i];
+        M = p.counts[2 * p.T];
+        pix_per_split = ((M + (int)gridDim.z - 1) / (int)gridDim.z + TP - 1) / TP * TP;
+        __syncthreads();
+    }
+    auto row_of = [&](int m) {
+        int t = 0;
+        while (t + 1 < p.T && pre[t + 1] <= m) ++t;
+        return t * p.B_rows + (m - pre[t]);
+    };
+    const int m_begin = split * pix_per_split;
+    int m_end = m_begin + pix_per_split;
+    if (m_end > M) m_end = M;
 
     int it_valid = (d.Cin - (i0 + wm * 64) + 31) / 32;
     it_valid = it_valid < 0 ? 0 : (it_valid > 2 ? 2 : it_valid);
@@ -102,7 +119,8 @@
         for (int i = 0; i < XP; ++i) {
             const int m = mt0 + xrow + XROWS * i;
             const bool rv = m < m_end;
-            const int mm = rv ? m : 0;
+            int mm = rv ? m : 0;
+            if constexpr (LIVE) mm = rv ? row_of(m) : 0;
             const int n = small ? fdiv(mm, ohw, p.inv_ohw) : mm / ohw;
             const int r = mm - n * ohw;
             const int oh = small ? fdiv(r, d.OW, p.inv_ow) : r / d.OW;
@@ -117,7 +135,9 @@
         for (int i = 0; i < 2; ++i) {
             const int m = mt0 + zrow + 8 * i;
             const bool okz = m < m_end && cz < d.Cout;
-            const unsigned offz = (unsigned)(m < m_end ? m : 0) * (unsigned)p.lddz + (unsigned)cz;
+            int mz = m < m_end ? m : 0;
+            if constexpr (LIVE) mz = m < m_end ? row_of(m) : 0;
+            const unsigned offz = (unsigned)mz * (unsigned)p.lddz + (unsigned)cz;
             rz[i] = load4(srd_z, offz * 4u, okz, p.z_vec, d.Cout - cz);
         }
     };
@@ -197,10 +217,11 @@
     return v;
 }
 
-template <int AI, int BJ>
+template <int AI, int BJ, bool LIVE = false>
 __global__ __launch_bounds__(256, (AI * BJ > 8) ? 1 : 2) void wgrad_direct_kernel(const WgradParams p) {
     constexpr int NACC = AI * BJ, U = DS_WG_U;
     __shared__ __attribute__((aligned(16))) float red[2 * NACC * 16 * 64];
+    __shared__ int cnt[LIVE ? kLiveMaxT : 1];
     const ds_conv_desc &d = p.d;
     const int tid = threadIdx.x, lane = tid & 63;
     const int wave = __builtin_amdgcn_readfirstlane(tid >> 6);
@@ -218,9 +239,16 @@
     const __amdgpu_buffer_rsrc_t srd_x = make_srd(p.x, p.x_bytes);
     const __amdgpu_buffer_rsrc_t srd_z = make_srd(p.dz, p.z_bytes);
 
-    const int m_begin = split * p.pix_per_split;
-    int m_end = m_begin + p.pix_per_split;
-    if (m_end > p.M) m_end = p.M;
+    int M = p.M, pix_per_split = p.pix_per_split;
+    if constexpr (LIVE) {
+        for (int i = tid; i < p.T; i += 256) cnt[i] = p.counts[i];
+        M = p.counts[2 * p.T];
+        pix_per_split = ((M + p.slabs - 1) / p.slabs + 7) / 8 * 8;
+        __syncthreads();
+    }
+    const int m_begin = split * pix_per_split;
+    int m_end = m_begin + pix_per_split;
+    if (m_end > M) m_end = M;
     int q = (m_end - m_begin + 3) / 4;
     q = (q + 1) & ~1;
     const int wb = m_begin + wave * q;
@@ -257,8 +285,30 @@
     const unsigned span_h = (unsigned)(hi_of(d.pad_t, dh, d.stride, d.H, d.OH) - lo_h);
     const unsigned span_w = (unsigned)(hi_of(d.pad_l, dw, d.stride, d.W, d.OW) - lo_w);
     const int OWc = d.OW, OHc = d.OH;
+    int lt = 0, lb = m, lnt = 0x7fffffff;
+    if constexpr (LIVE) {
+        lnt = cnt[0];
+        while (lt < p.T && lb >= lnt) {
+            lb -= lnt;
+            ++lt;
+            lnt = lt < p.T ? cnt[lt] : 0x7fffffff;
+        }
+    }
     auto offsets = [&](unsigned &ox, unsigned &oz) {
         const bool mv = m < we;
+        if constexpr (LIVE) {
+            const unsigned row = (unsigned)(lt * p.B_rows + lb);
+            oz = (mv && co_ok) ? (row * (unsigned)p.lddz + (unsigned)co) * 4u : kOOB;
+            ox = (mv && ci_ok) ? (row * (unsigned)d.ldx + (unsigned)ci) * 4u : kOOB;
+            m += 2;
+            lb += 2;
+            while (lb >= lnt) {
+                lb -= lnt;
+                ++lt;
+                lnt = lt < p.T ? cnt[lt] : 0x7fffffff;
+            }
+            return;
+        }
         const bool in = (unsigned)(oh - lo_h) <= span_h && (unsigned)(ow - lo_w) <= span_w;
         oz = (mv && co_ok) ? offz : kOOB;
         ox = (mv && ci_ok && in) ? offx : kOOB;
@@ -471,6 +521,9 @@
     return pl;
 }
 
+int wgrad_launch(const char *who, const ds_conv_desc *d, const float *x, const float *dz, int32_t lddz, float *dw, void *ws,
+                 size_t ws_bytes, int32_t B_rows, const int32_t *counts, void *stream);
+
 }
 
 extern "C" size_t ds_conv_wgrad_workspace(const ds_conv_desc *d) {
@@ -490,7 +543,25 @@
 
 extern "C" int ds_conv_wgrad(const ds_conv_desc *d, const float *x, const float *dz, int32_t lddz, float *dw,
                              void *ws, size_t ws_bytes, void *stream) {
+    return wgrad_launch("ds_conv_wgrad", d, x, dz, lddz, dw, ws, ws_bytes, 0, nullptr, stream);
+}
+
+extern "C" int ds_conv_wgrad_live(const ds_conv_desc *d, const float *x, const float *dz, int32_t lddz, float *dw,
+                                  void *ws, size_t ws_bytes, int32_t B_rows, const int32_t *counts, void *stream) {
+    DS_REQUIRE(d && counts && B_rows > 0, "ds_conv_wgrad_live: null argument or B_rows <= 0");
+    DS_REQUIRE(d->KH == 1 && d->KW == 1 && d->H == 1 && d->W == 1 && d->OH == 1 && d->OW == 1 && d->stride == 1 &&
+               d->pad_t == 0 && d->pad_l == 0 && d->fold_cin == 0,
+               "ds_conv_wgrad_live: GEMM form only (KH = KW = H = W = 1, stride 1, no padding)");
+    DS_REQUIRE(d->N > 0 && d->N % B_rows == 0 && d->N / B_rows <= kLiveMaxT, "ds_conv_wgrad_live: N = T * B_rows with T <= 256");
+    return wgrad_launch("ds_conv_wgrad_live", d, x, dz, lddz, dw, ws, ws_bytes, B_rows, counts, stream);
+}
+
+namespace {
+
+int wgrad_launch(const char *who, const ds_conv_desc *d, const float *x, const float *dz, int32_t lddz, float *dw, void *ws,
+                 size_t ws_bytes, int32_t B_rows, const int32_t *counts, void *stream) {
     DS_REQUIRE(d && x && dz && dw, "ds_conv_wgrad: null argument");
+    const bool live = counts != nullptr;
     const int64_t M = (int64_t)d->N * d->OH * d->OW;
     DS_REQUIRE(M < (1ll << 31), "ds_conv_wgrad: M too large");
     DS_REQUIRE(d->fold_cin == 0 || (d->KW == 1 && d->ldx == d->fold_cin && d->fold_cin % 4 == 0 && d->Cin % d->fold_cin == 0),
@@ -519,15 +590,22 @@
     p.inv_ow = 1.0f / (float)d->OW;
     p.x_vec = (d->ldx % 4 == 0) && (d->Cin % 4 == 0) && (((uintptr_t)x & 15) == 0);
     p.z_vec = (lddz % 4 == 0) && (d->Cout % 4 == 0) && (((uintptr_t)dz & 15) == 0);
+    p.counts = counts;
+    p.B_rows = B_rows;
+    p.T = live ? (int)(M / B_rows) : 0;
+    p.slabs = splits;
     hipStream_t s = (hipStream_t)stream;
     int pps = (int)((M + splits - 1) / splits);
     if (pl.direct) {
         p.ci_tiles = (d->Cin + 32 * pl.ai - 1) / (32 * pl.ai);
         p.pix_per_split = (pps + 7) / 8 * 8;
         const int co_tiles = (d->Cout + 32 * pl.bj - 1) / (32 * pl.bj);
-        p.slabs = splits;
         const dim3 grid((unsigned)(d->KH * d->KW * p.ci_tiles * co_tiles * splits));
-#define DS_WG(A, B) if (pl.ai == A && pl.bj == B) hipLaunchKernelGGL((wgrad_direct_kernel<A, B>), grid, dim3(256), 0, s, p);
+#define DS_WG(A, B)                                                                                              \
+    if (pl.ai == A && pl.bj == B) {                                                                              \
+        if (live) hipLaunchKernelGGL((wgrad_direct_kernel<A, B, true>), grid, dim3(256), 0, s, p);               \
+        else hipLaunchKernelGGL((wgrad_direct_kernel<A, B>), grid, dim3(256), 0, s, p);                          \
+    }
         DS_WG(4, 4) DS_WG(4, 2) DS_WG(4, 1) DS_WG(2, 4) DS_WG(2, 2) DS_WG(2, 1) DS_WG(1, 4) DS_WG(1, 2) DS_WG(1, 1)
 #undef DS_WG
     } else {
@@ -535,7 +613,9 @@
         p.ci_tiles = (d->Cin + ti - 1) / ti;
         p.pix_per_split = ((pps + TP - 1) / TP) * TP;
         dim3 grid(d->KH * d->KW * p.ci_tiles, (d->Cout + TJ - 1) / TJ, splits);
-        if (ti == 64) hipLaunchKernelGGL(conv_wgrad_kernel<64>, grid, dim3(256), 0, s, p);
+        if (live && ti == 64) hipLaunchKernelGGL((conv_wgrad_kernel<64, true>), grid, dim3(256), 0, s, p);
+        else if (live) hipLaunchKernelGGL((conv_wgrad_kernel<128, true>), grid, dim3(256), 0, s, p);
+        else if (ti == 64) hipLaunchKernelGGL(conv_wgrad_kernel<64>, grid, dim3(256), 0, s, p);
         else hipLaunchKernelGGL(conv_wgrad_kernel<128>, grid, dim3(256), 0, s, p);
     }
     if (splits > 1) {
@@ -543,5 +623,7 @@
         hipLaunchKernelGGL(splitk_reduce_kernel, dim3(ds::stream_grid(n, 256)), dim3(256), 0, s,
                            (const float *)ws, dw, n, splits);
     }
-    return ds::check_launch("ds_conv_wgrad");
-}
+    return ds::check_launch(who);
+}
+
+}
diff --git a/tumblr_emotions_amd/csrc/text_misc.hip b/tumblr_emotions_amd/csrc/text_misc.hip
--- a/tumblr_emotions_amd/csrc/text_misc.hip
+++ b/tumblr_emotions_amd/csrc/text_misc.hip
@@ -336,6 +336,88 @@
     out[c] = (float)acc;
 }
 
+constexpr int kLiveMaxT = 256;
+
+__global__ __launch_bounds__(256) void colsum_live_stage1(const float *x, int C, int ld, int B, int T, const int *counts, int RS,
+                                                          float *partials) {
+    __shared__ float red[4][64];
+    __shared__ int cnt[kLiveMaxT];
+    for (int i = threadIdx.x; i < T; i += 256) cnt[i] = counts[i];
+    const int R = counts[2 * T];
+    __syncthreads();
+    const int cl = threadIdx.x & 63, rl = __builtin_amdgcn_readfirstlane(threadIdx.x >> 6);
+    const int c = blockIdx.x * 64 + cl;
+    const int rps = (R + RS - 1) / RS;
+    const int r0 = blockIdx.y * rps;
+    int r1 = r0 + rps;
+    if (r1 > R) r1 = R;
+    int r = r0 + rl, t = 0, b = r0 + rl;
+    int nt = cnt[0];
+    while (t < T && b >= nt) {
+        b -= nt;
+        ++t;
+        nt = t < T ? cnt[t] : 0x7fffffff;
+    }
+    float acc = 0.f;
+    if (c < C)
+        while (r < r1) {
+            float v[4];
+#pragma unroll
+            for (int k = 0; k < 4; ++k) {
+                v[k] = r < r1 ? x[((int64_t)t * B + b) * ld + c] : 0.f;
+                r += 4;
+                b += 4;
+                while (b >= nt) {
+                    b -= nt;
+                    ++t;
+                    nt = t < T ? cnt[t] : 0x7fffffff;
+                }
+            }
+#pragma unroll
+            for (int k = 0; k < 4; ++k) acc += v[k];
+        }
+    red[rl][cl] = acc;
+    __syncthreads();
+    if (rl == 0 && c < C) partials[(int64_t)blockIdx.y * C + c] = red[0][cl] + red[1][cl] + red[2][cl] + red[3][cl];
+}
+
+__global__ __launch_bounds__(64) void colsum_live_stage2(const float *partials, int RS, int C, float *out) {
+    const int c = blockIdx.x * 64 + threadIdx.x;
+    if (c >= C) return;
+    float v[64];
+#pragma unroll
+    for (int s = 0; s < 64; ++s) v[s] = partials[(int64_t)(s < RS ? s : RS - 1) * C + c];
+    double acc = 0.0;
+#pragma unroll
+    for (int s = 0; s < 64; ++s) acc += s < RS ? (double)v[s] : 0.0;
+    out[c] = (float)acc;
+}
+
+__global__ __launch_bounds__(256) void seq_live_counts_kernel(const int64_t *len, int B, int T, int *counts) {
+    __shared__ int n[kLiveMaxT];
+    __shared__ int lens[4096];
+    for (int b = threadIdx.x; b < B; b += 256) {
+        const int64_t l = len[b];
+        lens[b] = (int)(l < 0 ? 0 : (l > T ? T : l));
+    }
+    __syncthreads();
+    for (int t = threadIdx.x; t < T; t += 256) {
+        int k = 0;
+        for (int b = 0; b < B; ++b) k += lens[b] > t ? 1 : 0;
+        n[t] = k;
+        counts[t] = k;
+    }
+    __syncthreads();
+    if (threadIdx.x == 0) {
+        int s = 0;
+        for (int t = 0; t < T; ++t) {
+            counts[T + t] = s;
+            s += n[t];
+        }
+        counts[2 * T] = s;
+    }
+}
+
 __global__ __launch_bounds__(256) void copy2d_kernel(const float *src, int lds, float *dst, int ldd, int64_t rows,
                                                      int cols) {
     const int64_t total = rows * cols;
@@ -581,6 +663,24 @@
     return ds::check_launch("ds_colsum");
 }
 
+extern "C" int ds_seq_live_counts(const int64_t *len, int32_t B, int32_t T, int32_t *counts, void *stream) {
+    DS_REQUIRE(len && counts && B > 0 && B <= 4096 && T > 0 && T <= kLiveMaxT, "ds_seq_live_counts: bad argument (B <= 4096, T <= 256)");
+    hipLaunchKernelGGL(seq_live_counts_kernel, dim3(1), dim3(256), 0, (hipStream_t)stream, len, B, T, counts);
+    return ds::check_launch("ds_seq_live_counts");
+}
+
+extern "C" int ds_colsum_live(const float *x, int64_t M, int32_t C, int32_t ld, int32_t B_rows, const int32_t *counts,
+                              float *scratch, float *out, void *stream) {
+    DS_REQUIRE(x && counts && scratch && out && M > 0 && M < (1ll << 31) && C > 0 && ld >= C && B_rows > 0 && M % B_rows == 0 &&
+               M / B_rows <= kLiveMaxT, "ds_colsum_live: bad argument (M = T * B_rows, T <= 256)");
+    int RS = (int)((M + 63) / 64);
+    if (RS > 64) RS = 64;
+    hipLaunchKernelGGL(colsum_live_stage1, dim3((C + 63) / 64, RS), dim3(256), 0, (hipStream_t)stream, x, C, ld, B_rows,
+                       (int)(M / B_rows), counts, RS, scratch);
+    hipLaunchKernelGGL(colsum_live_stage2, dim3((C + 63) / 64), dim3(64), 0, (hipStream_t)stream, scratch, RS, C, out);
+    return ds::check_launch("ds_colsum_live");
+}
+
 __global__ __launch_bounds__(256) void slab_epilogue_kernel(const float *slabs, int splits, int64_t slab_stride, int lds,
                                                             int64_t M, int N, float *out, int ldo, const float *bias,
                                                             const float *mask, int ldmask, int flags) {
diff --git a/tumblr_emotions_amd/engine_text.py b/tumblr_emotions_amd/engine_text.py
--- a/tumblr_emotions_amd/engine_text.py
+++ b/tumblr_emotions_amd/engine_text.py
@@ -33,6 +33,7 @@
         self.persistent = True
         self.seq_rows = 1
         self.sort_by_length = _lib.tuning_env("DS_LSTM_SORT", "1") != "0" 
+        self.skip_padded_rows = _lib.tuning_env("DS_TEXT_SKIP_PAD", "1") != "0"
 
     def alloc(self, B):
         if self.B == B:
@@ -48,6 +49,9 @@
             self.texts_sorted = torch.empty(B, T, dtype=torch.int64, device=dev)
             self.h_last = torch.empty(B, H, device=dev)
             self.dh_sorted = torch.empty(B, H, device=dev)
+        self.live_rows = self.sorted and T <= 256
+        if self.live_rows:
+            self.live_counts = torch.zeros(2 * T + 1, dtype=torch.int32, device=dev)
         self.seq_ws = torch.zeros(max(ops.lstm_seq_workspace(B, H) // 4, 4), dtype=torch.int32, device=dev)
         self.x = torch.empty(T * B, D, device=dev)
         self.gates = torch.empty(T, B, 4 * H, device=dev)
@@ -99,6 +103,8 @@
             if not seq_lens.is_contiguous() or not texts.is_contiguous():
                 seq_lens, texts = seq_lens.contiguous(), texts.contiguous()
             ops.seq_sort_desc(seq_lens, B, T, self.perm, self.len_sorted)
+            if self.live_rows:
+                ops.seq_live_counts(self.len_sorted, B, T, self.live_counts)
             ops.permute_rows(texts, self.texts_sorted, self.perm, B, T, gather=True)
             seq_lens, texts = self.len_sorted, self.texts_sorted
         self.seq_lens, self.texts = seq_lens, texts
@@ -175,9 +181,14 @@
     def _weight_grads(self):
         B, T, H = self.B, self.T, self.H
         dg = ops._p(self.dgates)
-        self.wgrad_x.run(ops._p(self.x), dg, self.gwx, ops._p(self.ws), self.ws_bytes)
-        self.wgrad_h.run(ops._p(self.h), dg, self.gwh, ops._p(self.ws), self.ws_bytes)
-        ops.colsum(self.dgates, T * B, 4 * H, 4 * H, self.colsum_scratch, self.gbias)
+        if self.live_rows and self.skip_padded_rows:
+            self.wgrad_x.run_live(ops._p(self.x), dg, self.gwx, ops._p(self.ws), self.ws_bytes, B, self.live_counts)
+            self.wgrad_h.run_live(ops._p(self.h), dg, self.gwh, ops._p(self.ws), self.ws_bytes, B, self.live_counts)
+            ops.colsum_live(self.dgates, T * B, 4 * H, 4 * H, B, self.live_counts, self.colsum_scratch, self.gbias)
+        else:
+            self.wgrad_x.run(ops._p(self.x), dg, self.gwx, ops._p(self.ws), self.ws_bytes)
+            self.wgrad_h.run(ops._p(self.h), dg, self.gwh, ops._p(self.ws), self.ws_bytes)
+            ops.colsum(self.dgates, T * B, 4 * H, 4 * H, self.colsum_scratch, self.gbias)
         if self.trainable_embedding:
             self.x_dgrad.run(dg, self.wx, ops._p(self.dx))
             ops.embedding_grad(self.dx, self.texts, self.gtable, B, T, self.D, time_major=True)
diff --git a/tumblr_emotions_amd/ops.py b/tumblr_emotions_amd/ops.py
--- a/tumblr_emotions_amd/ops.py
+++ b/tumblr_emotions_amd/ops.py
@@ -530,6 +530,10 @@
         _lib.check(_lib.load().ds_conv_wgrad(C.byref(self.d), x, dz, self.lddz, dw, ws, ws_bytes, _stream()),
                    "ds_conv_wgrad")
 
+    def run_live(self, x, dz, dw, ws, ws_bytes, B_rows, counts):
+        _lib.check(_lib.load().ds_conv_wgrad_live(C.byref(self.d), x, dz, self.lddz, dw, ws, ws_bytes, B_rows, _p(counts),
+                                                  _stream()), "ds_conv_wgrad_live")
+
 
 def bn_finalize(stats, P, count, C_, beta, eps, decay, mean, rstd, shift, mm, mv, pivot=None):
     _lib.check(_lib.load().ds_bn_finalize(_p(stats), P, count, C_, _p(beta), _p(pivot), eps, decay, _p(mean),
@@ -843,6 +847,11 @@
     _lib.check(_lib.load().ds_seq_sort_desc(_p(seq_len), B, T, _p(perm), _p(len_sorted), _stream()), "ds_seq_sort_desc")
 
 
+def seq_live_counts(lens, B, T, counts):
+    assert counts.dtype == torch.int32 and counts.numel() >= 2 * T + 1
+    _lib.check(_lib.load().ds_seq_live_counts(_p(lens), B, T, _p(counts), _stream()), "ds_seq_live_counts")
+
+
 def permute_rows(src, dst, perm, rows, cols, gather=True):
     assert src.element_size() == dst.element_size() and src.element_size() in (4, 8)
     _lib.check(_lib.load().ds_permute_rows(_p(src), src.stride(0), _p(dst), dst.stride(0), _p(perm), rows, cols, src.element_size(),
@@ -878,6 +887,11 @@
 
 def colsum(x, M, C_, ld, scratch, out):
     _lib.check(_lib.load().ds_colsum(_p(x), M, C_, ld, _p(scratch), _p(out), _stream()), "ds_colsum")
+
+
+def colsum_live(x, M, C_, ld, B_rows, counts, scratch, out):
+    _lib.check(_lib.load().ds_colsum_live(_p(x), M, C_, ld, B_rows, _p(counts), _p(scratch), _p(out), _stream()),
+               "ds_colsum_live")
 
 
 def copy2d(src, lds, dst, ldd, rows, cols):
```

Measured after the change: 19890 samples/s, median of 6. Within noise of the previous version (+0.8%).
